# austinjeng/Shift-GCN

Hardware: AMD Instinct MI355X
Metric: skeleton clips/sec fwd+bwd, NTU (3,300,25,2) bs=64; 1/2/4/8 MI355X (higher is better)
Workload: dtype fp32; 1 GPU; NTU Shift-GCN training step (fwd+CE+bwd+SGD), x=(64,3,300,25,2) per GPU; global_batch=64, per_gpu_batch=64, parallelism=dp1, hipgraph=False, world_size=1, backend=none

## Files before the change

include/shiftgcn.h:

```cpp
#ifndef SHIFTGCN_H_
#define SHIFTGCN_H_

#include <stddef.h>

#ifdef __cplusplus
extern "C" {
#endif

#define SGCN_EINVAL (-22)
#define SGCN_ABI_VERSION 24
#define SGCN_ABI_DIAG_FLAG 0x10000

int sgcn_abi_version(void);


int sgcn_tshift_fwd(const float* in, float* out, const float* xpos, const float* ypos,
                    const float* in_scale, const float* in_shift, float* plane_stats,
                    int B, int C, int H, int W, int stride, int ypos_is_raw, void* stream);

int sgcn_tshift_fwd_pre(const float* z, float* out, const float* xpos, const float* ypos,
                        const float* pre_scale, const float* pre_shift, const float* r,
                        const float* r_scale, const float* r_shift, const float* in_scale,
                        const float* in_shift, int B, int C, int H, int W, int stride,
                        int ypos_is_raw, void* stream);

int sgcn_tshift_fwd_tail(const float* in, float* out, const float* xpos, const float* ypos,
                         const float* post_scale, const float* post_shift, const float* r,
                         const float* r_scale, const float* r_shift, const float* gather_m,
                         float* out_gathered, int B, int C, int H, int W, int stride,
                         int ypos_is_raw, void* stream);

int sgcn_tshift_bwd_bnin(const float* dy, const float* y, const float* s, const float* coef,
                         const float* in, const float* xpos, const float* ypos, float* gin,
                         float* gx, float* gy, void* ws, size_t ws_bytes, int B, int C, int H,
                         int W, int ypos_is_raw, int dy_plane, void* stream);
size_t sgcn_tshift_bwd_ws_bytes(int B, int C);

int sgcn_tshift_pos_finalize(const void* ws, int B, int C, float* gx, float* gy, void* stream);

int sgcn_tshift_bwd(const float* gout, const float* in, const float* xpos, const float* ypos,
                    const float* in_scale, const float* in_shift, int relu_mask,
                    const float* bn_mean, const float* bn_invstd, float* bn_part, float* gin,
                    float* gx, float* gy, void* ws, size_t ws_bytes, int B, int C, int H,
                    int W, int stride, int ypos_is_raw, void* stream);

int sgcn_tshift_fwd_f64(const double* in, double* out, const double* xpos, const double* ypos,
                        int B, int C, int H, int W, int stride, int ypos_is_raw, void* stream);
size_t sgcn_tshift_bwd_f64_ws_bytes(int B, int C);
int sgcn_tshift_bwd_f64(const double* gout, const double* in, const double* xpos,
                        const double* ypos, double* gin, double* gx, double* gy, void* ws,
                        size_t ws_bytes, int B, int C, int H, int W, int stride,
                        int ypos_is_raw, void* stream);

int sgcn_tshift_bwd_gbn(const float* gout, const float* in, const float* xpos,
                        const float* ypos, const float* in_scale, const float* in_shift,
                        const float* bn_mean, const float* bn_invstd, float* bn_part,
                        const float* z, const float* z_mean, const float* z_invstd,
                        float* z_part, const float* d, const float* d_mean,
                        const float* d_invstd, float* d_part, float* gin, float* gx, float* gy,
                        void* ws, size_t ws_bytes, int B, int C, int H, int W, void* stream);


int sgcn_pw_fwd(const float* w, int w_mcontig, const float* bias, const float* x,
                long long x_bstride, long long x_cstride, int x_tstride, int x_rsign,
                const float* mask, float* y, long long y_bstride, long long y_cstride,
                int y_tstride, int y_rsign, int relu, int accumulate, int B, int M, int K,
                int T, int V, void* stream);

size_t sgcn_pw_tshift_ws_bytes(int K);
int sgcn_pw_fwd_tshift(const float* w, const float* bias, const float* x, long long x_bstride,
                       long long x_cstride, const float* xpos, const float* ypos,
                       const float* in_scale, const float* in_shift, float* x_shifted,
                       void* ws, size_t ws_bytes, float* y, long long y_bstride,
                       long long y_cstride, int relu, int two_row, int B, int M, int K, int T,
                       int V, void* stream);

size_t sgcn_pw_dw_ws_bytes(int B, int M, int Nc, int T, int V);

int sgcn_pw_dw(const float* g, long long g_bstride, long long g_cstride, int g_tstride,
               int g_rsign, const float* x, long long x_bstride, long long x_cstride,
               int x_tstride, int x_rsign, const float* mask, float* dw, int dw_transpose,
               int dw_accumulate, float* dbias, int dbias_accumulate, void* ws,
               size_t ws_bytes, int B, int M, int Nc, int T, int V, void* stream);


size_t sgcn_moments_ws_bytes(int B, int C, int V, int per_joint);

int sgcn_moments(const float* x, float* part, int B, int C, int T, int V, int per_joint,
                 void* stream);


int sgcn_bn_finalize(const float* part, int B, int F, int n_part, int perm_V,
                     const float* gamma, const float* beta, float eps, float momentum,
                     float* running_mean, float* running_var, long long* num_batches,
                     float* mean, float* invstd, float* scale, float* shift, void* stream);

int sgcn_bn_eval_coef(int F, int perm_V, const float* gamma, const float* beta,
                      const float* running_mean, const float* running_var, float eps,
                      float* mean, float* invstd, float* scale, float* shift, void* stream);

int sgcn_bn_apply(const float* x, const float* scale, const float* shift, int per_joint,
                  const float* r, const float* rscale, const float* rshift, int relu,
                  float* y, float* y_stats, const float* gather_m, float* y_gathered, int B,
                  int C, int T, int V, void* stream);
int sgcn_bn_bwd_reduce(const float* dy, const float* y, int relu, const float* x,
                       const float* mean, const float* invstd, int per_joint, const float* r,
                       const float* rmean, const float* rinvstd, const float* dy_coef,
                       float* part, float* rpart, int B, int C, int T, int V, int dy_plane,
                       void* stream);

int sgcn_bn_bwd_finalize(const float* part, int B, int F, long long n_total, int perm_V,
                         const float* mean, const float* invstd, const float* gamma,
                         float* dgamma, float* dbeta, int accumulate, int batch_stats,
                         float* coef, void* stream);

int sgcn_bn_bwd_finalize_gbn(const float* part6, int B, int C, int V, long long n_total,
                             const float* dy_coef, const float* dy_mean, const float* mean,
                             const float* invstd, const float* gamma, float* dgamma,
                             float* dbeta, int accumulate, int batch_stats, float* coef,
                             void* stream);

int sgcn_bn_bwd_apply(const float* dy, const float* y, int relu, const float* x,
                      const float* coef, int per_joint, const float* r, const float* rcoef,
                      const float* dy_coef, float* dx, float* dr, int B, int C, int T, int V,
                      void* stream);

int sgcn_mask_prep(const float* mask, float* m, int n, void* stream);

int sgcn_gcn_gather(const float* x0, const float* m, float* xg, int B, int C, int T, int V,
                    void* stream);

#define SGCN_DXF_MASK_DX 1
#define SGCN_DXF_ADD2_PLANE 2
int sgcn_gcn_dx_finish(const float* dxt, const float* x0, const float* m, const float* add1,
                       const float* add2, const float* add2_mask, float* dx, float* dmask_part,
                       const float* prev_s, const float* prev_mean, const float* prev_invstd,
                       float* prev_part, int B, int C, int T, int V, int flags, void* stream);

int sgcn_mask_grad_finalize(const float* part, const float* mask, int B, int C, int V,
                            float* dmask, int accumulate, void* stream);

int sgcn_modalities(const float* joint, const int* parent, float* out_joint, float* out_bone,
                    float* out_joint_motion, float* out_bone_motion, const float* scale,
                    const float* shift, int planes, int N, int C, int T, int V, int M,
                    void* stream);


size_t sgcn_head_ws_bytes(int N, int C, int V, int M);

int sgcn_head_moments(const float* x, float* part, int N, int C, int T, int V, int M,
                      void* stream);

int sgcn_head_apply(const float* x, const float* scale, const float* shift, float* y, int N,
                    int C, int T, int V, int M, void* stream);

int sgcn_head_bwd_reduce(const float* g, const float* x, const float* mean, const float* invstd,
                         float* part, int N, int C, int T, int V, int M, void* stream);

int sgcn_head_bwd_apply(const float* g, const float* x, const float* coef, float* dx, int N,
                        int C, int T, int V, int M, void* stream);

int sgcn_pool(const float* x, float* out, int N, int M, int C, long long P, void* stream);

int sgcn_pool_bwd(const float* dout, float* dx, int N, int M, int C, long long P,
                  void* stream);

int sgcn_pool_bwd_planes(const float* dout, float* dplane, int N, int M, int C, long long P,
                         void* stream);


int sgcn_sgd_chunk_elems(void);

int sgcn_sgd_step(const void* table, const int* numel, const int* chunks, int n_chunks,
                  float momentum, int nesterov, void* stream);

#define SGCN_BATCH_MAX 32
int sgcn_tshift_pos_finalize_many(const void* const* partials, float* const* gx,
                                  float* const* gy, const int* B, const int* C, int n,
                                  void* stream);
int sgcn_mask_prep_many(const float* const* mask, float* const* m, const int* count, int n,
                        void* stream);
int sgcn_mask_grad_finalize_many(const float* const* part, const float* const* mask,
                                 float* const* dmask, const int* B, const int* C,
                                 const int* V, int n, void* stream);

#ifdef __cplusplus
}
#endif

#endif
```

shift-gcn_amd/csrc/bn.hip:

```cpp
#include "common.hpp"

namespace sgcn {
namespace {

constexpr int kThreads = 256;

constexpr int kU = 4;

constexpr int kUM = 8;

template <bool PER_JOINT, bool ZU = false>
__global__ __launch_bounds__(kThreads) void moments_kernel(const float* __restrict__ x,
                                                            float2* __restrict__ part, int T,
                                                            int V, int C) {
  SGCN_CRIT_PRIO();
  __shared__ float s1[kThreads], s2[kThreads], red[2 * kThreads / 64];
  const int plane = gridDim.x - 1 - blockIdx.x;
  const int P = T * V;
  const float* __restrict__ xp = x + (size_t)plane * P;
  const int i = threadIdx.x;
  if (PER_JOINT) {
    const int G = kThreads / V;
    float a = 0.f, q = 0.f;
    const int v = i % V, r = i / V;
// ... 595 lines not shown
  for (int q = 0; q < kGbnW - 1; ++q) {
#pragma unroll
    for (int j = 0; j < 6; ++j) s6[j] += red[q][j][lane];
  }
  const int c = f / V;
  const double k1 = dyc[c], k2 = dyc[C + c], c3 = (double)dyc[2 * C + c] + k2 * (double)dym[c];
  const double sg = k1 * s6[0] + k2 * s6[1] + c3 * s6[2];
  const double sgx = k1 * s6[3] + k2 * s6[4] + c3 * s6[5];
  const int rf = ref_feature(f, V, F);
  if (dgamma) dgamma[rf] = accumulate ? dgamma[rf] + (float)sgx : (float)sgx;
  if (dbeta) dbeta[rf] = accumulate ? dbeta[rf] + (float)sg : (float)sg;
  const float g = gamma ? gamma[rf] : 1.f;
  const float is = invstd[f];
  const float q1 = g * is;
  const float q2 = batch_stats ? (float)(-(double)q1 * (double)is * (sgx / n_total)) : 0.f;
  const float q3 = batch_stats ? (float)(-(double)q1 * (sg / n_total) - (double)q2 * (double)mean[f])
                               : 0.f;
  coef[f] = q1;
  coef[F + f] = q2;
  coef[2 * F + f] = q3;
}

template <int PJM, bool RELU, int RES, bool DYT>
__global__ __launch_bounds__(kThreads) void bn_bwd_apply_kernel(
    const float* __restrict__ dy, const float* __restrict__ y, const float* __restrict__ x,
    const float* __restrict__ coef, int F, const float* __restrict__ r,
    const float* __restrict__ rcoef, int RF, const float* __restrict__ dyc,
    float* __restrict__ dx, float* __restrict__ dr, int C, int T, int V) {
  SGCN_CRIT_PRIO();
  constexpr bool PER_JOINT = PJM != 0, GATH = PJM >= 2, XG = PJM == 3;
  const int plane = blockIdx.x, c = plane % C;
  const int P = T * V;
  const size_t off = (size_t)plane * P;
  const int rc = c % V;
  __shared__ float k_s[PER_JOINT ? 3 * kThreads : 1];
  if (PER_JOINT) {
    if ((int)threadIdx.x < V) {
      const int f = c * V + threadIdx.x;
      k_s[threadIdx.x] = coef[f];
      k_s[kThreads + threadIdx.x] = coef[F + f];
      k_s[2 * kThreads + threadIdx.x] = coef[2 * F + f];
    }
    __syncthreads();
  }
  float k1 = 0.f, k2 = 0.f, k3 = 0.f, q1 = 0.f, q2 = 0.f, q3 = 0.f;
  float d1 = 1.f, d2 = 0.f, d3 = 0.f;
  if (DYT) { d1 = dyc[c]; d2 = dyc[C + c]; d3 = dyc[2 * C + c]; }
  if (!PER_JOINT) { k1 = coef[c]; k2 = coef[F + c]; k3 = coef[2 * F + c]; }
  if (RES == 2) { q1 = rcoef[c]; q2 = rcoef[RF + c]; q3 = rcoef[2 * RF + c]; }
  const int dv = kThreads % V;
  int v = threadIdx.x % V;
  for (int base = 0; base < P; base += kThreads * kU) {
    float gv[kU], yv[kU], xv[kU], rv[kU];
#pragma unroll
    for (int u = 0; u < kU; ++u) {
      const int o = min(base + u * kThreads + (int)threadIdx.x, P - 1);
      gv[u] = dy[off + o];
      if (RELU) yv[u] = y[off + o];
      if (!XG) xv[u] = x[off + o];
      if (RES == 2) rv[u] = r[off + o];
    }
    if (XG) {
      int vq = v;
#pragma unroll
      for (int u = 0; u < kU; ++u) {
        const int o = min(base + u * kThreads + (int)threadIdx.x, P - 1);
        const int w = vq - rc;
        xv[u] = x[off + min(max(o - vq + (w < 0 ? w + V : w), 0), P - 1)];
        vq += dv;
        if (vq >= V) vq -= V;
      }
    }
#pragma unroll
    for (int u = 0; u < kU; ++u) {
      const int o = base + u * kThreads + threadIdx.x;
      float g = gv[u];
      if (DYT) g = d1 * g + d2 * yv[u] + d3;
      if (RELU) g = yv[u] > 0.f ? g : 0.f;
      if (PER_JOINT) { k1 = k_s[v]; k2 = k_s[kThreads + v]; k3 = k_s[2 * kThreads + v]; }
      if (o < P) {
        int od = o;
        if (GATH) {
          const int w = v - rc;
          od = o - v + (w < 0 ? w + V : w);
        }
        dx[off + od] = k1 * g + k2 * xv[u] + k3;
        if (RES == 1) dr[off + o] = g;
        if (RES == 2) dr[off + o] = q1 * g + q2 * rv[u] + q3;
      }
      v += dv;
      if (v >= V) v -= V;
    }
  }
}

template <int NT, int LPT, int PJM, bool RELU, int RES, bool DYT>
__global__ __launch_bounds__(NT) void bn_bwd_apply_ja_kernel(
    const float* __restrict__ dy, const float* __restrict__ y, const float* __restrict__ x,
    const float* __restrict__ coef, int F, const float* __restrict__ r,
    const float* __restrict__ rcoef, int RF, const float* __restrict__ dyc,
    float* __restrict__ dx, float* __restrict__ dr, int C, int T, int V) {
  SGCN_CRIT_PRIO();
  static_assert(PJM == 0 || PJM == 3, "per-channel, or per-joint gathered (ZU)");
  constexpr bool PER_JOINT = PJM == 3;
  const int plane = blockIdx.x, c = plane % C, rc = c % V;
  const int GR = NT / V, NTJ = GR * V, tid = threadIdx.x;
  const bool own = tid < NTJ;
  const int w = tid % V;
  const int P = T * V;
  const size_t off = (size_t)plane * P;
  const unsigned vo = own ? (unsigned)tid * 4u : 0x80000000u, vstep = (unsigned)NTJ * 4u;
  const unsigned pb = (unsigned)P * 4u;
  int wz = w - rc;
  wz = wz < 0 ? wz + V : wz;
  const unsigned go = vo + (unsigned)((PER_JOINT ? wz - w : 0) * 4);
  float gv[LPT], yv[RELU ? LPT : 1], xv[LPT], rv[RES == 2 ? LPT : 1];
  {
    const auto dyr = make_rsrc(dy + off, pb);
    const auto xr = make_rsrc(x + off, pb);
#pragma unroll
    for (int e = 0; e < LPT; ++e) {
      gv[e] = bload(dyr, vo + e * vstep, 0);
      xv[e] = bload(xr, go + e * vstep, 0);
    }
    if (RELU) {
      const auto yr = make_rsrc(y + off, pb);
#pragma unroll
      for (int e = 0; e < LPT; ++e) yv[e] = bload(yr, vo + e * vstep, 0);
    }
    if (RES == 2) {
      const auto rr = make_rsrc(r + off, pb);
#pragma unroll
      for (int e = 0; e < LPT; ++e) rv[e] = bload(rr, vo + e * vstep, 0);
    }
  }
  const int f = PER_JOINT ? c * V + w : c;
  const float k1 = coef[f], k2 = coef[F + f], k3 = coef[2 * F + f];
  float d1 = 1.f, d2 = 0.f, d3 = 0.f, q1 = 0.f, q2 = 0.f, q3 = 0.f;
  if (DYT) { d1 = dyc[c]; d2 = dyc[C + c]; d3 = dyc[2 * C + c]; }
  if (RES == 2) { q1 = rcoef[c]; q2 = rcoef[RF + c]; q3 = rcoef[2 * RF + c]; }
  const auto dxr = make_rsrc(dx + off, pb);
  const auto drr = make_rsrc(RES ? dr + off : dx + off, RES ? pb : 0u);
#pragma unroll
  for (int e = 0; e < LPT; ++e) {
    float g = gv[e];
    if (DYT) g = d1 * g + d2 * yv[e] + d3;
    if (RELU) g = yv[e] > 0.f ? g : 0.f;
    bstore(dxr, k1 * g + k2 * xv[e] + k3, go + e * vstep, 0);
    if (RES == 1) bstore(drr, g, vo + e * vstep, 0);
    if (RES == 2) bstore(drr, q1 * g + q2 * rv[e] + q3, vo + e * vstep, 0);
  }
}

template <int NT, int LPT, bool ADD1, bool ADD2, bool PART, int A2M>
__global__ __launch_bounds__(NT) void gcn_dx_finish_ja_kernel(
    const float* __restrict__ dxt, const float* __restrict__ x0, const float* __restrict__ m,
    const float* __restrict__ add1, const float* __restrict__ add2, float* __restrict__ dx,
    float* __restrict__ dmask_part, const float* __restrict__ ps,
    const float* __restrict__ pmean, const float* __restrict__ pinvstd,
    float2* __restrict__ bn_part, int C, int T, int V, const float* __restrict__ add2m,
    int flags) {
  SGCN_CRIT_PRIO();
#ifdef SGCN_DIAG_F1B_REAL
  return;
#endif
  __shared__ float s0[NT];
  __shared__ float red[2 * NT / 64];
  const int plane = blockIdx.x, c = plane % C, rc = c % V;
  const int GR = NT / V, NTJ = GR * V, tid = threadIdx.x;
  const bool own = tid < NTJ;
  const int vd = tid % V;
  int us = vd - rc;
  us = us < 0 ? us + V : us;
  const int P = T * V;
  const size_t off = (size_t)plane * P;
  const unsigned vo = own ? (unsigned)tid * 4u : 0x80000000u, vstep = (unsigned)NTJ * 4u;
  const unsigned pb = (unsigned)P * 4u;
  const unsigned uo = vo + (unsigned)((us - vd) * 4);
  const bool mdx = flags & SGCN_DXF_MASK_DX;
  constexpr bool A2P = A2M == 2;
  float gv[LPT], xq[LPT], a1[ADD1 ? LPT : 1], a2[ADD2 && !A2P ? LPT : 1], a2q[A2M ? LPT : 1];
  float sv[PART ? LPT : 1];
  {
#ifdef SGCN_DIAG_F1B_BOUND
    const auto gr = make_rsrc(dxt + off, 0u), xr = make_rsrc(x0 + off, pb);
#else
    const auto gr = make_rsrc(dxt + off, pb), xr = make_rsrc(x0 + off, pb);
#endif
#pragma unroll
    for (int e = 0; e < LPT; ++e) {
      gv[e] = bload(gr, uo + e * vstep, 0);
      xq[e] = bload(xr, vo + e * vstep, 0);
    }
    if (ADD1) {
      const auto ar = make_rsrc(add1 + off, pb);
#pragma unroll
      for (int e = 0; e < LPT; ++e) a1[e] = bload(ar, vo + e * vstep, 0);
    }
    if (ADD2 && !A2P) {
      const auto ar = make_rsrc(add2 + off, pb);
#pragma unroll
      for (int e = 0; e < LPT; ++e) a2[e] = bload(ar, vo + e * vstep, 0);
    }
    if (A2M) {
      const auto ar = make_rsrc(add2m + off, pb);
#pragma unroll
      for (int e = 0; e < LPT; ++e) a2q[e] = bload(ar, vo + e * vstep, 0);
    }
    if (PART) {
      const auto ar = make_rsrc(ps + off, pb);
#pragma unroll
      for (int e = 0; e < LPT; ++e) sv[e] = bload(ar, vo + e * vstep, 0);
    }
  }
  const float mu = m[us * C + c];
  float pm = 0.f, pi = 0.f, a2v = 0.f;
  if (PART) { pm = pmean[c]; pi = pinvstd[c]; }
  if (A2P) a2v = add2[plane];
  const auto dxr = make_rsrc(dx + off, pb);
  float acc = 0.f, b0 = 0.f, b1 = 0.f;
#pragma unroll
  for (int e = 0; e < LPT; ++e) {
    float val = gv[e] * mu;
    if (ADD1) val += a1[e];
    if (ADD2) val += A2M ? (a2q[e] > 0.f ? (A2P ? a2v : a2[e]) : 0.f) : a2[e];
    bstore(dxr, (xq[e] > 0.f || !mdx) ? val : 0.f, vo + e * vstep, 0);
    acc = fmaf(gv[e], xq[e], acc);
    if (PART) {
      const float g = xq[e] > 0.f ? val : 0.f;
      b0 += g;
      b1 = fmaf(g, (sv[e] - pm) * pi, b1);
    }
  }
  if (PART) {
    block_sum2(b0, b1, red);
    if (tid == 0) bn_part[plane] = make_float2(b0, b1);
  }
  s0[tid] = acc;
  __syncthreads();
  if (tid < V) {
    int vq = tid + rc;
    vq = vq >= V ? vq - V : vq;
    float sum = 0.f;
    for (int g = 0; g < GR; ++g) sum += s0[g * V + vq];
    dmask_part[(size_t)plane * V + tid] = sum;
  }
}

__global__ __launch_bounds__(kThreads) void gcn_gather_kernel(const float* __restrict__ x0,
                                                              const float* __restrict__ m,
                                                              float* __restrict__ xg, int C,
                                                              int T, int V) {
  SGCN_CRIT_PRIO();
  __shared__ float m_s[kThreads];
  const int plane = blockIdx.x, c = plane % C;
  const int P = T * V;
  const size_t off = (size_t)plane * P;
  const int rc = c % V;
  if ((int)threadIdx.x < V) m_s[threadIdx.x] = m[threadIdx.x * C + c];
  __syncthreads();
  const int dv = kThreads % V;
  int w = threadIdx.x % V;
  for (int base = 0; base < P; base += kThreads * kU) {
    float xv[kU], mv[kU];
    int ww = w;
#pragma unroll
    for (int u = 0; u < kU; ++u) {
      const int oraw = base + u * kThreads + (int)threadIdx.x;
      int src = ww + rc;
      src = src >= V ? src - V : src;
      xv[u] = x0[off + min(oraw - ww + src, P - 1)];
      mv[u] = m_s[ww];
      ww += dv;
      if (ww >= V) ww -= V;
    }
#pragma unroll
    for (int u = 0; u < kU; ++u) {
      const int o = base + u * kThreads + (int)threadIdx.x;
      if (o < P) xg[off + o] = xv[u] * mv[u];
    }
    w = ww;
  }
}

template <bool ADD1, bool ADD2, bool PART, bool A2M = false>
__global__ __launch_bounds__(kThreads) void gcn_dx_finish_kernel(
    const float* __restrict__ dxt, const float* __restrict__ x0, const float* __restrict__ m,
    const float* __restrict__ add1, const float* __restrict__ add2, float* __restrict__ dx,
    float* __restrict__ dmask_part, const float* __restrict__ ps,
    const float* __restrict__ pmean, const float* __restrict__ pinvstd,
    float2* __restrict__ bn_part, int C, int T, int V, const float* __restrict__ add2m,
    int flags) {
  SGCN_CRIT_PRIO();
  const bool mdx = flags & SGCN_DXF_MASK_DX, a2p = flags & SGCN_DXF_ADD2_PLANE;
  __shared__ float s0[kThreads];
  const int plane = blockIdx.x, c = plane % C;
  const size_t off = (size_t)plane * T * V;
  const int rc = c % V;
  const int i = threadIdx.x;
  const int G = kThreads / V;
  const int vd = i % V, rr = i / V;
  int us = vd - rc;
  us = us < 0 ? us + V : us;
  const float mu = m[us * C + c];
  float pm = 0.f, pi = 0.f;
  if (PART) { pm = pmean[c]; pi = pinvstd[c]; }
  float acc = 0.f, b0 = 0.f, b1 = 0.f;
  if (i < G * V) {
    for (int t0 = rr; t0 < T; t0 += G * kU) {
      float gv[kU], xq[kU], a1[kU], a2[kU], sv[kU], a2q[kU];
#pragma unroll
      for (int k = 0; k < kU; ++k) {
        const int row = min(t0 + k * G, T - 1) * V;
        gv[k] = dxt[off + row + us];
        xq[k] = x0[off + row + vd];
        if (ADD1) a1[k] = add1[off + row + vd];
        if (ADD2) a2[k] = a2p ? add2[plane] : add2[off + row + vd];
        if (A2M) a2q[k] = add2m[off + row + vd];
        if (PART) sv[k] = ps[off + row + vd];
      }
#pragma unroll
      for (int k = 0; k < kU; ++k) {
        const int t = t0 + k * G;
        float val = gv[k] * mu;
        if (ADD1) val += a1[k];
        if (ADD2) val += A2M ? (a2q[k] > 0.f ? a2[k] : 0.f) : a2[k];
        if (t < T) dx[off + t * V + vd] = (xq[k] > 0.f || !mdx) ? val : 0.f;
        acc += (t < T) ? gv[k] * xq[k] : 0.f;
        if (PART) {
          const float g = (t < T && xq[k] > 0.f) ? val : 0.f;
          b0 += g;
          b1 += g * ((sv[k] - pm) * pi);
        }
      }
    }
  }
  if (PART) {
    __shared__ float red[2 * kThreads / 64];
    block_sum2(b0, b1, red);
    if (i == 0) bn_part[plane] = make_float2(b0, b1);
  }
  s0[i] = acc;
  __syncthreads();
  if (i < V) {
    int vq = i + rc;
    vq = vq >= V ? vq - V : vq;
    float sum = 0.f;
    for (int g = 0; g < G; ++g) sum += s0[g * V + vq];
    dmask_part[(size_t)plane * V + i] = sum;
  }
}

__global__ void mask_prep_kernel(const float* __restrict__ mask, float* __restrict__ m, int n) {
  const int i = blockIdx.x * blockDim.x + threadIdx.x;
  if (i < n) m[i] = tanhf(mask[i]) + 1.f;
}

struct MaskPrepBatch {
  const float* mask[SGCN_BATCH_MAX];
  float* m[SGCN_BATCH_MAX];
  int n[SGCN_BATCH_MAX];
};
__global__ void mask_prep_many_kernel(const MaskPrepBatch t) {
  const int e = blockIdx.y;
  const int i = blockIdx.x * blockDim.x + threadIdx.x;
  if (i < t.n[e]) t.m[e][i] = tanhf(t.mask[e][i]) + 1.f;
}

__device__ __forceinline__ void mask_grad_body(const float* __restrict__ part,
                                               const float* __restrict__ mask, int B, int C,
                                               int V, float* __restrict__ dmask,
                                               int accumulate);
__global__ __launch_bounds__(64 * kFW) void mask_grad_finalize_kernel(
    const float* __restrict__ part, const float* __restrict__ mask, int B, int C, int V,
    float* __restrict__ dmask, int accumulate) {
  mask_grad_body(part, mask, B, C, V, dmask, accumulate);
}
struct MaskGradBatch {
  const float* part[SGCN_BATCH_MAX];
  const float* mask[SGCN_BATCH_MAX];
  float* dmask[SGCN_BATCH_MAX];
  int B[SGCN_BATCH_MAX];
  int C[SGCN_BATCH_MAX];
  int V[SGCN_BATCH_MAX];
};
__global__ __launch_bounds__(64 * kFW) void mask_grad_finalize_many_kernel(const MaskGradBatch t) {
  const int i = blockIdx.y;
  if ((int)blockIdx.x * kFW >= t.C[i] * t.V[i]) return;
  mask_grad_body(t.part[i], t.mask[i], t.B[i], t.C[i], t.V[i], t.dmask[i], 0);
}
__device__ __forceinline__ void mask_grad_body(const float* __restrict__ part,
                                               const float* __restrict__ mask, int B, int C,
                                               int V, float* __restrict__ dmask,
                                               int accumulate) {
  const int F = C * V;
  const int lane = threadIdx.x & 63;
  const int f = blockIdx.x * kFW + (int)(threadIdx.x >> 6);
  const int fc = min(f, F - 1);
  double a = 0.0;
  for (int b0 = lane; b0 < B; b0 += 64 * 4) {
    float pv[4];
#pragma unroll
    for (int u = 0; u < 4; ++u) {
      const int b = b0 + u * 64;
      pv[u] = b < B ? part[(size_t)b * F + fc] : 0.f;
    }
#pragma unroll
    for (int u = 0; u < 4; ++u) a += pv[u];
  }
  const double s = wave_dsum(a);
  if (f >= F || lane != 0) return;
  const int c = f / V, u = f - c * V;
  const int i = u * C + c;
  const float t = tanhf(mask[i]);
  const float g = (float)s * (1.f - t * t);
  dmask[i] = accumulate ? dmask[i] + g : g;
}

}
}

using namespace sgcn;

constexpr int kJaSplit = 8192;

int ja_lpt(int T, int V, int nt) {
  if (V > 64) return 0;
  const int ntj = (nt / V) * V, per = (T * V + ntj - 1) / ntj;
  return per <= 8 ? 8 : (per <= 16 ? 16 : (per <= 24 ? 24 : (per <= 32 ? 32 : 0)));
}

#define SGCN_PLANE_CHECK() \
  SGCN_REQUIRE(B >= 0 && C > 0 && T >= 0 && V > 0 && V <= kThreads)

extern "C" {

size_t sgcn_moments_ws_bytes(int B, int C, int V, int per_joint) {
  return (size_t)B * C * (per_joint ? V : 1) * sizeof(float2);
}

int sgcn_moments(const float* x, float* part, int B, int C, int T, int V, int per_joint,
                 void* stream) {
  SGCN_PLANE_CHECK();
  if (B == 0) return 0;
  SGCN_REQUIRE(x && part && T > 0);
  hipStream_t st = (hipStream_t)stream;
  SGCN_REQUIRE(per_joint == 0 || per_joint == 3);
  {
    const int nt = T * V <= kJaSplit ? kThreads : 512;
    const int lpt = ja_lpt(T, V, nt);
    if (lpt) {
#define SGCN_MJ(NT, L, PJ)                                                                     \
  moments_ja_kernel<NT, L, PJ, PJ><<<B * C, NT, 0, st>>>(x, (float2*)part, T, V, C)
#define SGCN_MJ_L(NT, PJ)                                                                      \
  do {                                                                                         \
    if (lpt == 8) SGCN_MJ(NT, 8, PJ); else if (lpt == 16) SGCN_MJ(NT, 16, PJ);                 \
    else if (lpt == 24) SGCN_MJ(NT, 24, PJ);                                                   \
    else SGCN_MJ(NT, 32, PJ);                                                                  \
  } while (0)
      if (nt == kThreads) { if (per_joint) SGCN_MJ_L(kThreads, true); else SGCN_MJ_L(kThreads, false); }
      else { if (per_joint) SGCN_MJ_L(512, true); else SGCN_MJ_L(512, false); }
#undef SGCN_MJ_L
#undef SGCN_MJ
      SGCN_LAUNCH_CHECK();
      return 0;
    }
  }
  if (per_joint == 3)
    moments_kernel<true, true><<<B * C, kThreads, 0, st>>>(x, (float2*)part, T, V, C);
  else moments_kernel<false><<<B * C, kThreads, 0, st>>>(x, (float2*)part, T, V, C);
  SGCN_LAUNCH_CHECK();
  return 0;
}

int sgcn_bn_finalize(const float* part, int B, int F, int n_part, int perm_V,
                     const float* gamma, const float* beta, float eps, float momentum,
                     float* running_mean, float* running_var, long long* num_batches,
                     float* mean, float* invstd, float* scale, float* shift, void* stream) {
  SGCN_REQUIRE(part && B > 0 && F > 0 && n_part > 0 && mean && invstd && scale && shift);
// ... 181 lines not shown
  SGCN_REQUIRE(part && B > 0 && F > 0 && n_total > 0 && mean && invstd && coef);
  SGCN_REQUIRE(perm_V <= 0 || F % perm_V == 0);
  bn_bwd_finalize_kernel<<<(F + 63) / 64, 64 * kFSW, 0, (hipStream_t)stream>>>(
      (const float2*)part, B, F, (double)n_total, perm_V, mean, invstd, gamma, dgamma, dbeta,
      accumulate, batch_stats, coef);
  SGCN_LAUNCH_CHECK();
  return 0;
}

int sgcn_bn_bwd_finalize_gbn(const float* part6, int B, int C, int V, long long n_total,
                             const float* dy_coef, const float* dy_mean, const float* mean,
                             const float* invstd, const float* gamma, float* dgamma,
                             float* dbeta, int accumulate, int batch_stats, float* coef,
                             void* stream) {
  SGCN_REQUIRE(part6 && B > 0 && C > 0 && V > 0 && n_total > 0 && dy_coef && dy_mean && mean &&
               invstd && coef);
  const int F = C * V;
  bn_bwd_finalize_gbn_kernel<<<(F + 63) / 64, 64 * kGbnW, 0, (hipStream_t)stream>>>(
      part6, B, F, V, (double)n_total, dy_coef, dy_mean, C, mean, invstd, gamma, dgamma, dbeta,
      accumulate, batch_stats, coef);
  SGCN_LAUNCH_CHECK();
  return 0;
}

int sgcn_bn_bwd_apply(const float* dy, const float* y, int relu, const float* x,
                      const float* coef, int per_joint, const float* r, const float* rcoef,
                      const float* dy_coef, float* dx, float* dr, int B, int C, int T, int V,
                      void* stream) {
  SGCN_PLANE_CHECK();
  if (B == 0 || T == 0) return 0;
  SGCN_REQUIRE(dy && x && coef && dx && (y || !relu));
  SGCN_REQUIRE(!dy_coef || (y && relu));
  SGCN_REQUIRE(!rcoef || (r && dr));
  SGCN_REQUIRE(per_joint == 0 || per_joint == 3);
  hipStream_t st = (hipStream_t)stream;
  const int res = dr == nullptr ? 0 : (rcoef ? 2 : 1);
  const int F = per_joint ? C * V : C;
  dim3 g(B * C);
  if (per_joint == 3) SGCN_REQUIRE(relu);
  {
    const int nt = T * V <= kJaSplit ? kThreads : 512;
    const int lpt = ja_lpt(T, V, nt);
    if (lpt) {
#define SGCN_BJ(NT, L, PJ, RL, RS)                                                             \
  (dy_coef ? bn_bwd_apply_ja_kernel<NT, L, PJ, RL, RS, true><<<g, NT, 0, st>>>(                 \
                 dy, y, x, coef, F, r, rcoef, C, dy_coef, dx, dr, C, T, V)             \
           : bn_bwd_apply_ja_kernel<NT, L, PJ, RL, RS, false><<<g, NT, 0, st>>>(                \
                 dy, y, x, coef, F, r, rcoef, C, dy_coef, dx, dr, C, T, V))
#define SGCN_BJ_L(NT, PJ, RL, RS)                                                              \
  do {                                                                                         \
    if (lpt == 8) SGCN_BJ(NT, 8, PJ, RL, RS);                                                  \
    else if (lpt == 16) SGCN_BJ(NT, 16, PJ, RL, RS);                                           \
    else if (lpt == 24) SGCN_BJ(NT, 24, PJ, RL, RS);                                           \
    else SGCN_BJ(NT, 32, PJ, RL, RS);                                                          \
  } while (0)
#define SGCN_BJ_T(PJ, RL, RS)                                                                  \
  do { if (nt == kThreads) SGCN_BJ_L(kThreads, PJ, RL, RS); else SGCN_BJ_L(512, PJ, RL, RS); } while (0)
#define SGCN_BJ_R(PJ, RL)                                                                      \
  do {                                                                                         \
    if (res == 0) SGCN_BJ_T(PJ, RL, 0);                                                        \
    else if (res == 1) SGCN_BJ_T(PJ, RL, 1);                                                   \
    else SGCN_BJ_T(PJ, RL, 2);                                                                 \
  } while (0)
      if (per_joint == 3) SGCN_BJ_R(3, true);
      else if (relu) SGCN_BJ_R(0, true);
      else SGCN_BJ_R(0, false);
#undef SGCN_BJ_R
#undef SGCN_BJ_T
#undef SGCN_BJ_L
#undef SGCN_BJ
      SGCN_LAUNCH_CHECK();
      return 0;
    }
  }
#define SGCN_BA(PJ, RL, RS)                                                                   \
  (dy_coef ? bn_bwd_apply_kernel<PJ, RL, RS, true><<<g, kThreads, 0, st>>>(                      \
                 dy, y, x, coef, F, r, rcoef, C, dy_coef, dx, dr, C, T, V)                      \
           : bn_bwd_apply_kernel<PJ, RL, RS, false><<<g, kThreads, 0, st>>>(                     \
                 dy, y, x, coef, F, r, rcoef, C, dy_coef, dx, dr, C, T, V))
#define SGCN_BA_R(PJ, RL) \
  if (res == 0) SGCN_BA(PJ, RL, 0); else if (res == 1) SGCN_BA(PJ, RL, 1); else SGCN_BA(PJ, RL, 2)
  if (per_joint == 3) { SGCN_BA_R(3, true); }
  else if (relu) { SGCN_BA_R(0, true); } else { SGCN_BA_R(0, false); }
#undef SGCN_BA_R
#undef SGCN_BA
  SGCN_LAUNCH_CHECK();
  return 0;
}

int sgcn_mask_prep(const float* mask, float* m, int n, void* stream) {
  SGCN_REQUIRE(mask && m && n > 0);
  mask_prep_kernel<<<(n + 255) / 256, 256, 0, (hipStream_t)stream>>>(mask, m, n);
  SGCN_LAUNCH_CHECK();
  return 0;
}

int sgcn_mask_prep_many(const float* const* mask, float* const* m, const int* count, int n,
                        void* stream) {
  SGCN_REQUIRE(n >= 0 && n <= SGCN_BATCH_MAX);
  if (n == 0) return 0;
  SGCN_REQUIRE(mask && m && count);
  MaskPrepBatch t{};
  int mx = 0;
  for (int i = 0; i < n; ++i) {
    SGCN_REQUIRE(mask[i] && m[i] && count[i] > 0);
    t.mask[i] = mask[i];
    t.m[i] = m[i];
    t.n[i] = count[i];
    mx = max(mx, count[i]);
  }
  mask_prep_many_kernel<<<dim3((mx + 255) / 256, n), 256, 0, (hipStream_t)stream>>>(t);
  SGCN_LAUNCH_CHECK();
  return 0;
}

int sgcn_mask_grad_finalize_many(const float* const* part, const float* const* mask,
                                 float* const* dmask, const int* B, const int* C,
                                 const int* V, int n, void* stream) {
  SGCN_REQUIRE(n >= 0 && n <= SGCN_BATCH_MAX);
  if (n == 0) return 0;
  SGCN_REQUIRE(part && mask && dmask && B && C && V);
  MaskGradBatch t{};
  int mf = 0;
  for (int i = 0; i < n; ++i) {
    SGCN_REQUIRE(part[i] && mask[i] && dmask[i] && B[i] > 0 && C[i] > 0 && V[i] > 0);
    t.part[i] = part[i];
    t.mask[i] = mask[i];
    t.dmask[i] = dmask[i];
    t.B[i] = B[i];
    t.C[i] = C[i];
    t.V[i] = V[i];
    mf = max(mf, C[i] * V[i]);
  }
  mask_grad_finalize_many_kernel<<<dim3((mf + kFW - 1) / kFW, n), 64 * kFW, 0,
                                   (hipStream_t)stream>>>(t);
  SGCN_LAUNCH_CHECK();
  return 0;
}

int sgcn_gcn_gather(const float* x0, const float* m, float* xg, int B, int C, int T, int V,
                    void* stream) {
  SGCN_PLANE_CHECK();
  if (B == 0 || T == 0) return 0;
  SGCN_REQUIRE(x0 && m && xg && x0 != xg);
  gcn_gather_kernel<<<B * C, kThreads, 0, (hipStream_t)stream>>>(x0, m, xg, C, T, V);
  SGCN_LAUNCH_CHECK();
  return 0;
}

int sgcn_gcn_dx_finish(const float* dxt, const float* x0, const float* m, const float* add1,
                       const float* add2, const float* add2_mask, float* dx, float* dmask_part,
                       const float* prev_s, const float* prev_mean, const float* prev_invstd,
                       float* prev_part, int B,
                       int C, int T, int V, int flags, void* stream) {
  SGCN_PLANE_CHECK();
  if (B == 0 || T == 0) return 0;
  SGCN_REQUIRE(dxt && x0 && m && dx && dmask_part);
  SGCN_REQUIRE((flags & ~(SGCN_DXF_MASK_DX | SGCN_DXF_ADD2_PLANE)) == 0);
  SGCN_REQUIRE(!(flags & SGCN_DXF_ADD2_PLANE) || add2_mask);
  SGCN_REQUIRE(!prev_part || (prev_s && prev_mean && prev_invstd));
  SGCN_REQUIRE(!add2_mask || add2);
  hipStream_t st = (hipStream_t)stream;
  float2* pp = (float2*)prev_part;
  if (add2_mask) SGCN_REQUIRE(add1);
  {
    const int nt = T * V <= kJaSplit ? kThreads : 512;
    const int lpt = ja_lpt(T, V, nt);
    if (lpt) {
#define SGCN_FJ(NT, L, A1, A2, PT, AM)                                                         \
  gcn_dx_finish_ja_kernel<NT, L, A1, A2, PT, AM><<<B * C, NT, 0, st>>>(                        \
      dxt, x0, m, add1, add2, dx, dmask_part, prev_s, prev_mean, prev_invstd, pp, C, T, V,     \
      add2_mask, flags)
#define SGCN_FJ_L(NT, A1, A2, PT, AM)                                                          \
  do {                                                                                         \
    if (lpt == 8) SGCN_FJ(NT, 8, A1, A2, PT, AM);                                              \
    else if (lpt == 16) SGCN_FJ(NT, 16, A1, A2, PT, AM);                                       \
    else if (lpt == 24) SGCN_FJ(NT, 24, A1, A2, PT, AM);                                       \
    else SGCN_FJ(NT, 32, A1, A2, PT, AM);                                                      \
  } while (0)
#define SGCN_FJ_T(A1, A2, PT, AM)                                                              \
  do { if (nt == kThreads) SGCN_FJ_L(kThreads, A1, A2, PT, AM); else SGCN_FJ_L(512, A1, A2, PT, AM); } while (0)
#define SGCN_FJ_P(A1, A2, AM)                                                                  \
  do { if (pp) SGCN_FJ_T(A1, A2, true, AM); else SGCN_FJ_T(A1, A2, false, AM); } while (0)
      if (add2_mask) { if (flags & SGCN_DXF_ADD2_PLANE) SGCN_FJ_P(true, true, 2); else SGCN_FJ_P(true, true, 1); }
      else if (add1) { if (add2) SGCN_FJ_P(true, true, 0); else SGCN_FJ_P(true, false, 0); }
      else { if (add2) SGCN_FJ_P(false, true, 0); else SGCN_FJ_P(false, false, 0); }
#undef SGCN_FJ_P
#undef SGCN_FJ_T
#undef SGCN_FJ_L
#undef SGCN_FJ
      SGCN_LAUNCH_CHECK();
      return 0;
    }
  }
  if (add2_mask) {
    if (pp)
      gcn_dx_finish_kernel<true, true, true, true><<<B * C, kThreads, 0, st>>>(
          dxt, x0, m, add1, add2, dx, dmask_part, prev_s, prev_mean, prev_invstd, pp, C, T, V,
          add2_mask, flags);
    else
      gcn_dx_finish_kernel<true, true, false, true><<<B * C, kThreads, 0, st>>>(
          dxt, x0, m, add1, add2, dx, dmask_part, prev_s, prev_mean, prev_invstd, pp, C, T, V,
          add2_mask, flags);
    SGCN_LAUNCH_CHECK();
    return 0;
  }
#define SGCN_FIN(A1, A2, PT)                                                                \
  gcn_dx_finish_kernel<A1, A2, PT><<<B * C, kThreads, 0, st>>>(                           \
      dxt, x0, m, add1, add2, dx, dmask_part, prev_s, prev_mean, prev_invstd, pp, C, T, V,  \
      nullptr, flags)
#define SGCN_FIN_P(A1, A2)                                                                  \
  do {                                                                                      \
    if (pp) SGCN_FIN(A1, A2, true);                                                         \
    else SGCN_FIN(A1, A2, false);                                                           \
  } while (0)
  if (add1) { if (add2) SGCN_FIN_P(true, true); else SGCN_FIN_P(true, false); }
  else { if (add2) SGCN_FIN_P(false, true); else SGCN_FIN_P(false, false); }
#undef SGCN_FIN_P
#undef SGCN_FIN
  SGCN_LAUNCH_CHECK();
  return 0;
}

int sgcn_mask_grad_finalize(const float* part, const float* mask, int B, int C, int V,
                            float* dmask, int accumulate, void* stream) {
  SGCN_REQUIRE(part && mask && dmask && B > 0 && C > 0 && V > 0);
  mask_grad_finalize_kernel<<<(C * V + kFW - 1) / kFW, 64 * kFW, 0,
                              (hipStream_t)stream>>>(part, mask, B, C, V, dmask, accumulate);
  SGCN_LAUNCH_CHECK();
  return 0;
}

}
```

shift-gcn_amd/csrc/tshift.hip:

```cpp
#include "common.hpp"

#pragma clang fp contract(off)

namespace sgcn {
namespace {

constexpr int kThreads = 256;


struct Geom {
  int x1, y1;
  float dx, dy;
};

__device__ __forceinline__ Geom make_geom(float x, float y) {
  Geom g;
  g.x1 = (int)floorf(x);
  g.y1 = (int)floorf(y);
  g.dx = x - (float)g.x1;
  g.dy = y - (float)g.y1;
  return g;
}

__device__ __forceinline__ float blend(float q11, float q21, float q12, float q22, float dx,
// ... 429 lines not shown
    const int lstep = GR * stride * WP;
#pragma unroll
    for (int e = 0; e < LPT; ++e) {
      const int la = min(la0 + e * lstep, lmax);
      emit(e, blend(pl[la], pl[la + 1], pl[la + WP], pl[la + WP + 1], g.dx, g.dy));
    }
  } else {
    const bool c0 = (unsigned)(w + g.x1) < (unsigned)W, c1 = (unsigned)(w + g.x1 + 1) < (unsigned)W;
    const int cc0 = min(max(w + g.x1, 0), W - 1) + 1, cc1 = min(max(w + g.x1 + 1, 0), W - 1) + 1;
#pragma unroll
    for (int e = 0; e < LPT; ++e) {
      const int rr = (h0 + e * GR) * stride + g.y1;
      const bool r0 = (unsigned)rr < (unsigned)Hb, r1 = (unsigned)(rr + 1) < (unsigned)Hb;
      const int p0 = (min(max(rr, 0), Hb - 1) + kPadRows) * WP;
      const int p1 = (min(max(rr + 1, 0), Hb - 1) + kPadRows) * WP;
      const float q11 = (r0 && c0) ? pl[p0 + cc0] : 0.f, q21 = (r0 && c1) ? pl[p0 + cc1] : 0.f;
      const float q12 = (r1 && c0) ? pl[p1 + cc0] : 0.f, q22 = (r1 && c1) ? pl[p1 + cc1] : 0.f;
      emit(e, blend(q11, q21, q12, q22, g.dx, g.dy));
    }
  }
  if (STATS) {
    float s1 = 0.f;
#pragma unroll
    for (int e = 0; e < LPT; ++e) s1 += v[e];
    s1 = block_sum(s1, red);
    const float mean = s1 / (float)n;
    float m2 = 0.f;
#pragma unroll
    for (int e = 0; e < LPT; ++e) {
      const float d = v[e] - mean;
      m2 += e < nval ? d * d : 0.f;
    }
    m2 = block_sum(m2, red);
    if (tid == 0) pstats[plane] = make_float2(mean, m2);
  }
}

template <int NT, int LPT, int RES>
__global__ __launch_bounds__(NT) void tshift_fwd_pre_kernel(
    const float* __restrict__ z, float* __restrict__ out, const float* __restrict__ xpos,
    const float* __restrict__ ypos, const float* __restrict__ zs, const float* __restrict__ zt,
    const float* __restrict__ r, const float* __restrict__ rs, const float* __restrict__ rt,
    const float* __restrict__ scale, const float* __restrict__ shift, int C, int Hb, int W,
    int Ho, int stride, int add_half) {
  SGCN_CRIT_PRIO();
  extern __shared__ float pl[];
  __shared__ float zs_s[1024], zt_s[1024];
  const int plane = gridDim.x - 1 - blockIdx.x;
  const int c = plane % C;
  const int nb = Hb * W;
  const size_t ioff = (size_t)plane * nb;
  float* __restrict__ dst = out + (size_t)plane * Ho * W;
  const float y = add_half ? ypos[c] + 0.5f : ypos[c];
  const Geom g = make_geom(xpos[c], y);
  const float a = scale[c], b = shift[c];
  float q1 = 1.f, q2 = 0.f;
  if (RES == 2) { q1 = rs[c]; q2 = rt[c]; }
  for (int i = threadIdx.x; i < W; i += NT) {
    zs_s[i] = zs[c * W + i];
    zt_s[i] = zt[c * W + i];
  }
  __syncthreads();
  {
    float t[LPT], u[LPT];
#pragma unroll
    for (int e = 0; e < LPT; ++e) {
      const int i = min(e * NT + (int)threadIdx.x, nb - 1);
      t[e] = z[ioff + i];
      u[e] = r[ioff + i];
    }
    Walker pos(threadIdx.x, NT, W);
#pragma unroll
    for (int e = 0; e < LPT; ++e) {
      const int i = e * NT + threadIdx.x;
      float h = t[e] * zs_s[pos.w] + zt_s[pos.w];
      h += RES == 2 ? u[e] * q1 + q2 : u[e];
      h = fmaxf(h, 0.f);
      if (i < nb) pl[i] = h * a + b;
      pos.next();
    }
  }
  __syncthreads();
  const int n = Ho * W;
  for (int base = 0; base < n; base += LPT * NT) {
    Walker pos(base + threadIdx.x, NT, W);
#pragma unroll
    for (int e = 0; e < LPT; ++e) {
      TapIdx ti;
      tap_idx(pos.h * stride + g.y1, pos.w + g.x1, Hb, W, ti);
      const float q11 = sel(pl[ti.o00], ti.m00), q21 = sel(pl[ti.o01], ti.m01);
      const float q12 = sel(pl[ti.o10], ti.m10), q22 = sel(pl[ti.o11], ti.m11);
      const int o = base + e * NT + threadIdx.x;
      if (o < n) dst[o] = blend(q11, q21, q12, q22, g.dx, g.dy);
      pos.next();
    }
  }
}

template <int NT, int LPT, int RES, bool GOUT>
__global__ __launch_bounds__(NT) void tshift_fwd_tail_kernel(
    const float* __restrict__ in, float* __restrict__ out, const float* __restrict__ xpos,
    const float* __restrict__ ypos, const float* __restrict__ ps, const float* __restrict__ pt,
    const float* __restrict__ r, const float* __restrict__ rs, const float* __restrict__ rt,
    const float* __restrict__ gm, float* __restrict__ og, int C, int Hb, int W, int Ho,
    int stride, int add_half) {
  SGCN_CRIT_PRIO();
  extern __shared__ float pl[];
  __shared__ float gm_s[GOUT ? 1024 : 1];
  const int plane = gridDim.x - 1 - blockIdx.x;
  const int c = plane % C;
  const size_t ooff = (size_t)plane * Ho * W;
  const float y = add_half ? ypos[c] + 0.5f : ypos[c];
  const Geom g = make_geom(xpos[c], y);
  const float sc = ps[c], sh = pt[c];
  float q1 = 1.f, q2 = 0.f;
  if (RES == 2) { q1 = rs[c]; q2 = rt[c]; }
  const int rc = c % W;
  if (GOUT)
    for (int i = threadIdx.x; i < W; i += NT) gm_s[i] = gm[i * C + c];
  stage_plane<NT, LPT, false>(in + (size_t)plane * Hb * W, pl, Hb * W, 1.f, 0.f);
  __syncthreads();
  const int n = Ho * W;
  for (int base = 0; base < n; base += LPT * NT) {
    Walker pos(base + threadIdx.x, NT, W);
    float rv[LPT];
    if (RES) {
#pragma unroll
      for (int e = 0; e < LPT; ++e) rv[e] = r[ooff + min(base + e * NT + (int)threadIdx.x, n - 1)];
    }
#pragma unroll
    for (int e = 0; e < LPT; ++e) {
      TapIdx ti;
      tap_idx(pos.h * stride + g.y1, pos.w + g.x1, Hb, W, ti);
      const float q11 = sel(pl[ti.o00], ti.m00), q21 = sel(pl[ti.o01], ti.m01);
      const float q12 = sel(pl[ti.o10], ti.m10), q22 = sel(pl[ti.o11], ti.m11);
      const int o = base + e * NT + threadIdx.x;
      float a = blend(q11, q21, q12, q22, g.dx, g.dy) * sc + sh;
      if (RES == 1) a += rv[e];
      if (RES == 2) a += rv[e] * q1 + q2;
      a = fmaxf(a, 0.f);
      if (o < n) {
        out[ooff + o] = a;
        if (GOUT) {
          int u = pos.w - rc;
          u = u < 0 ? u + W : u;
          og[ooff + o - pos.w + u] = a * gm_s[u];
        }
      }
      pos.next();
    }
  }
}

template <int NT, int LPT, bool AFFINE, bool RELU_MASK, bool BNP, bool JA>
__global__ __launch_bounds__(NT) void tshift_bwd_s2_kernel(
    const float* __restrict__ gout, const float* __restrict__ in,
    const float* __restrict__ xpos, const float* __restrict__ ypos,
    const float* __restrict__ scale, const float* __restrict__ shift,
    const float* __restrict__ bn_mean, const float* __restrict__ bn_invstd,
    float* __restrict__ gin, float2* __restrict__ pgrad, float2* __restrict__ bn_part, int C,
    int Hb, int W, int Ho, int add_half) {
  SGCN_CRIT_PRIO();
  constexpr int STRIDE = 2;
  extern __shared__ float lds[];
  __shared__ float red[4 * NT / 64];
  const int plane = gridDim.x - 1 - blockIdx.x;
  const int c = plane % C;
  const int nb = Hb * W, nt = Ho * W;
  float* gs = lds;
  float* xs = lds + nt;
  float bmu = 0.f, bis = 0.f;
  if (BNP) { bmu = bn_mean[c]; bis = bn_invstd[c]; }
  const float x = xpos[c];
  const float y = add_half ? ypos[c] + 0.5f : ypos[c];
  float a = 1.f, b = 0.f;
  if (AFFINE) { a = scale[c]; b = shift[c]; }
  {
    const float* __restrict__ go = gout + (size_t)plane * nt;
    const float* __restrict__ src = in + (size_t)plane * nb;
    const int ntot = nt + nb;
    float t[LPT];
#pragma unroll
    for (int e = 0; e < LPT; ++e) {
      const int i = min(e * NT + (int)threadIdx.x, ntot - 1);
      t[e] = i < nt ? go[i] : src[i - nt];
    }
#pragma unroll
    for (int e = 0; e < LPT; ++e) {
      const int i = e * NT + threadIdx.x;
      if (i < ntot) lds[i] = t[e];
    }
  }
  __syncthreads();
  float* __restrict__ gi = gin + (size_t)plane * nb;

  float bs0 = 0.f, bs1 = 0.f;
  float ax = 0.f, ay = 0.f;
  if (JA) {
    const Geom r = make_geom(-x, -y);
    const int NTJ = (NT / W) * W, GR = NT / W;
    if ((int)threadIdx.x < NTJ && nt > 0) {
      const int w = (int)threadIdx.x % W, w1 = w + r.x1;
      const bool c0 = (unsigned)w1 < (unsigned)W, c1 = (unsigned)(w1 + 1) < (unsigned)W;
      const int cc0 = min(max(w1, 0), W - 1), cc1 = min(max(w1 + 1, 0), W - 1);
      int h = (int)threadIdx.x / W;
      for (int o = threadIdx.x; o < nb; o += NTJ, h += GR) {
        const int h1 = h + r.y1, hq = (h1 + 1) >> 1;
        const bool ev = (h1 & 1) == 0, rok = (unsigned)hq < (unsigned)Ho;
        const int ro = min(max(hq, 0), Ho - 1) * W;
        const float t0 = (rok && c0) ? gs[ro + cc0] : 0.f;
        const float t1 = (rok && c1) ? gs[ro + cc1] : 0.f;
        float val = blend(ev ? t0 : 0.f, ev ? t1 : 0.f, ev ? 0.f : t0, ev ? 0.f : t1, r.dx, r.dy);
        const float rin = xs[o];
        if (RELU_MASK) val = rin > 0.f ? val : 0.f;
        gi[o] = val;
        if (BNP) {
          bs0 += val;
          bs1 += val * ((rin - bmu) * bis);
        }
      }
    } else if ((int)threadIdx.x < NTJ) {
      for (int o = threadIdx.x; o < nb; o += NTJ) gi[o] = 0.f;
    }
  } else {
    const Geom r = make_geom(-x, -y);
    Walker pos(threadIdx.x, NT, W);
    for (int o = threadIdx.x; o < nb; o += NT) {
      const int h1 = pos.h + r.y1;
      const int w1 = pos.w + r.x1;
      TapIdx ti;
      {
        const int h2 = h1 + 1;
        const int hq1 = (h1 % 2 == 0) ? h1 / 2 : -1;
        const int hq2 = (h2 % 2 == 0) ? h2 / 2 : -1;
        TapIdx t1, t2;
        tap_idx(hq1, w1, Ho, W, t1);
        tap_idx(hq2, w1, Ho, W, t2);
        ti.o00 = t1.o00; ti.o01 = t1.o01; ti.m00 = t1.m00; ti.m01 = t1.m01;
        ti.o10 = t2.o00; ti.o11 = t2.o01; ti.m10 = t2.m00; ti.m11 = t2.m01;
      }
      float val = 0.f;
      if (nt > 0) {
        const float q11 = sel(gs[ti.o00], ti.m00), q21 = sel(gs[ti.o01], ti.m01);
        const float q12 = sel(gs[ti.o10], ti.m10), q22 = sel(gs[ti.o11], ti.m11);
        val = blend(q11, q21, q12, q22, r.dx, r.dy);
      }
      const float rin = xs[o];
      if (RELU_MASK) val = rin > 0.f ? val : 0.f;
      gi[o] = val;
      if (BNP) {
        bs0 += val;
        bs1 += val * ((rin - bmu) * bis);
      }
      pos.next();
    }
  }

  if (JA) {
    const Geom g = make_geom(x, y);
    const int NTJ = (NT / W) * W, GR = NT / W;
    if ((int)threadIdx.x < NTJ) {
      const int w = (int)threadIdx.x % W, wc = w + g.x1;
      const bool c0 = (unsigned)wc < (unsigned)W, c1 = (unsigned)(wc + 1) < (unsigned)W;
      const int cc0 = min(max(wc, 0), W - 1), cc1 = min(max(wc + 1, 0), W - 1);
      int h = (int)threadIdx.x / W;
      for (int o = threadIdx.x; o < nt; o += NTJ, h += GR) {
        const int rr = h * STRIDE + g.y1;
        const bool r0 = (unsigned)rr < (unsigned)Hb, r1 = (unsigned)(rr + 1) < (unsigned)Hb;
        const int p0 = min(max(rr, 0), Hb - 1) * W, p1 = min(max(rr + 1, 0), Hb - 1) * W;
        float q11 = xs[p0 + cc0], q21 = xs[p0 + cc1], q12 = xs[p1 + cc0], q22 = xs[p1 + cc1];
        if (AFFINE) { q11 = q11 * a + b; q21 = q21 * a + b; q12 = q12 * a + b; q22 = q22 * a + b; }
        q11 = (r0 && c0) ? q11 : 0.f;
        q21 = (r0 && c1) ? q21 : 0.f;
        q12 = (r1 && c0) ? q12 : 0.f;
        q22 = (r1 && c1) ? q22 : 0.f;
        const float vx = (1.f - g.dy) * (q21 - q11) + g.dy * (q22 - q12);
        const float vy = (1.f - g.dx) * (q12 - q11) + g.dx * (q22 - q21);
        const float gg = gs[o];
        ax += vx * gg;
        ay += vy * gg;
      }
    }
  } else {
    const Geom g = make_geom(x, y);
    Walker pos(threadIdx.x, NT, W);
    for (int o = threadIdx.x; o < nt; o += NT) {
      TapIdx ti;
      tap_idx(pos.h * STRIDE + g.y1, pos.w + g.x1, Hb, W, ti);
      float q11 = xs[ti.o00], q21 = xs[ti.o01], q12 = xs[ti.o10], q22 = xs[ti.o11];
      if (AFFINE) { q11 = q11 * a + b; q21 = q21 * a + b; q12 = q12 * a + b; q22 = q22 * a + b; }
      q11 = sel(q11, ti.m00);
      q21 = sel(q21, ti.m01);
      q12 = sel(q12, ti.m10);
      q22 = sel(q22, ti.m11);
      const float vx = (1.f - g.dy) * (q21 - q11) + g.dy * (q22 - q12);
      const float vy = (1.f - g.dx) * (q12 - q11) + g.dx * (q22 - q21);
      const float gg = gs[o];
      ax += vx * gg;
      ay += vy * gg;
      pos.next();
    }
  }
  if (BNP) {
    block_sum4(ax, ay, bs0, bs1, red);
    if (threadIdx.x == 0) {
      pgrad[plane] = make_float2(ax, ay);
      bn_part[plane] = make_float2(bs0, bs1);
    }
  } else {
    block_sum2(ax, ay, red);
    if (threadIdx.x == 0) pgrad[plane] = make_float2(ax, ay);
  }
}

template <int NT, int LPT, bool AFFINE, bool RELU_MASK, bool BNP, int GP, bool GBN,
          bool GBD = false>
__global__ __launch_bounds__(NT) void tshift_bwd_ra_kernel(
    const float* __restrict__ gout, const float* __restrict__ in,
    const float* __restrict__ xpos, const float* __restrict__ ypos,
    const float* __restrict__ scale, const float* __restrict__ shift,
    const float* __restrict__ bn_mean, const float* __restrict__ bn_invstd,
    float* __restrict__ gin, float2* __restrict__ pgrad, float2* __restrict__ bn_part, int C,
    int H, int W, const float* __restrict__ gdy, const float* __restrict__ gy,
    const float* __restrict__ gx, const float* __restrict__ gcoef,
    const float* __restrict__ gz, const float* __restrict__ gzm,
    const float* __restrict__ gzi, float* __restrict__ gzpart, const float* __restrict__ gd = nullptr,
    const float* __restrict__ gdm = nullptr, const float* __restrict__ gdi = nullptr,
    float* __restrict__ gdpart = nullptr, int gdyp = 0) {
  SGCN_CRIT_PRIO();
  static_assert(!GBN || (AFFINE && BNP && !GP), "GBN: shift_in with BNP");
// ... 274 lines not shown
      const int b = b0 + u * 64;
      pv[u] = b < B ? pgrad[(size_t)b * C + cc] : make_float2(0.f, 0.f);
    }
#pragma unroll
    for (int u = 0; u < 4; ++u) {
      ax += (double)pv[u].x;
      ay += (double)pv[u].y;
    }
  }
#pragma unroll
  for (int o = 32; o > 0; o >>= 1) {
    ax += __shfl_xor(ax, o, 64);
    ay += __shfl_xor(ay, o, 64);
  }
  if (c >= C || lane != 0) return;
  const double sx = ax, sy = ay;
  const float Gx = (float)(sx / (double)B);
  const float Gy = (float)(sy / (double)B);
  const float gy2 = Gy * Gy;
  const float dr = (float)sqrt((double)gy2);
  if (dr != 0.f) {
    const float qx = (float)((double)Gx / (double)dr);
    const float qy = (float)((double)Gy / (double)dr);
    gx[c] = (float)((double)qx * 0.0);
    gy[c] = (float)((double)qy * 0.01);
  } else {
    gx[c] = 0.0f;
    gy[c] = (float)0.0001;
  }
}

template <int EPT>
void launch_fwd(bool affine, bool stats, const float* in, float* out, const float* xpos,
                const float* ypos, const float* scale, const float* shift, float2* ps, int B,
                int C, int H, int W, int Ho, int stride, int add_half, hipStream_t st) {
  dim3 grid(B * C), block(kThreads);
#define SGCN_FWD(A, S)                                                                     \
  tshift_fwd_kernel<EPT, A, S><<<grid, block, 0, st>>>(in, out, xpos, ypos, scale, shift, \
                                                      ps, C, H, W, Ho, stride, add_half)
  if (affine) {
    if (stats) SGCN_FWD(true, true); else SGCN_FWD(true, false);
  } else {
    if (stats) SGCN_FWD(false, true); else SGCN_FWD(false, false);
  }
#undef SGCN_FWD
}

template <int LPT, int NT = kThreads>
void launch_fwd_lds(bool affine, bool stats, const float* in, float* out, const float* xpos,
                    const float* ypos, const float* scale, const float* shift, float2* ps,
                    int B, int C, int H, int W, int Ho, int stride, int add_half,
                    hipStream_t st) {
  dim3 grid(B * C), block(NT);
  const size_t lds = (size_t)H * W * sizeof(float);
#define SGCN_FWDL(A, S)                                                                  \
  tshift_fwd_lds_kernel<NT, LPT, LPT, A, S><<<grid, block, lds, st>>>(                    \
      in, out, xpos, ypos, scale, shift, ps, C, H, W, Ho, stride, add_half)
  if (affine) {
    if (stats) SGCN_FWDL(true, true); else SGCN_FWDL(true, false);
  } else {
    if (stats) SGCN_FWDL(false, true); else SGCN_FWDL(false, false);
  }
#undef SGCN_FWDL
}

int pad_fwd_lpt(int H, int W, int nt) {
  if (W > 64) return 0;
  const int ntj = (nt / W) * W, per = (H * W + ntj - 1) / ntj;
  int lpt = per <= 8 ? 8 : (per <= 16 ? 16 : (per <= 24 ? 24 : (per <= 32 ? 32 : 0)));
  if (nt == 512 && per > 8 && per <= 12) lpt = 12;
  if (nt == 512 && per > 16 && per <= 20) lpt = 20;
  return (size_t)(ra_pad_floats(H, W) + 1) * sizeof(float) > 65536 ? 0 : lpt;
}

template <int NT>
bool launch_fwd_pad(bool affine, bool stats, const float* in, float* out, const float* xpos,
                    const float* ypos, const float* scale, const float* shift, float2* ps,
                    int B, int C, int H, int W, int Ho, int stride, int add_half,
                    hipStream_t st) {
  const int lpt = pad_fwd_lpt(H, W, NT);
  const size_t lds = (size_t)(ra_pad_floats(H, W) + 1) * sizeof(float);
  if (lpt == 0) return false;
#define SGCN_FWDP(L, A, S)                                                                   \
  tshift_fwd_pad_kernel<NT, L, 0, A, S><<<B * C, NT, lds, st>>>(                             \
      in, out, xpos, ypos, scale, shift, ps, C, H, W, Ho, stride, add_half, nullptr, nullptr, \
      nullptr, nullptr, nullptr, nullptr, nullptr)
#define SGCN_FWDP_AS(L)                                                                      \
  do {                                                                                       \
    if (affine) { if (stats) SGCN_FWDP(L, true, true); else SGCN_FWDP(L, true, false); }     \
    else { if (stats) SGCN_FWDP(L, false, true); else SGCN_FWDP(L, false, false); }          \
  } while (0)
  if (lpt == 8) SGCN_FWDP_AS(8); else if (lpt == 12) SGCN_FWDP_AS(12); else if (lpt == 16) SGCN_FWDP_AS(16);
  else if (lpt == 20) SGCN_FWDP_AS(20); else if (lpt == 24) SGCN_FWDP_AS(24); else SGCN_FWDP_AS(32);
#undef SGCN_FWDP_AS
#undef SGCN_FWDP
  return true;
}

template <int EPT, int STRIDE>
void launch_bwd(bool affine, bool relu, const float* gout, const float* in, const float* xpos,
                const float* ypos, const float* scale, const float* shift, const float* bmu,
                const float* bis, float* gin, float2* pg, float2* bp, int B, int C, int H,
                int W, int Ho, int add_half, hipStream_t st) {
  dim3 grid(B * C), block(kThreads);
#define SGCN_BWD(A, R, P)                                                                    \
  tshift_bwd_kernel<EPT, A, R, STRIDE, P><<<grid, block, 0, st>>>(                            \
      gout, in, xpos, ypos, scale, shift, bmu, bis, gin, pg, bp, C, H, W, Ho, add_half)
  if (bp) {
    if (affine) {
      if (relu) SGCN_BWD(true, true, true); else SGCN_BWD(true, false, true);
    } else {
      if (relu) SGCN_BWD(false, true, true); else SGCN_BWD(false, false, true);
    }
  } else {
    if (affine) {
      if (relu) SGCN_BWD(true, true, false); else SGCN_BWD(true, false, false);
    } else {
      if (relu) SGCN_BWD(false, true, false); else SGCN_BWD(false, false, false);
    }
  }
#undef SGCN_BWD
}

constexpr int kBwdThreads = 512;

template <int LPT, bool JA>
void launch_bwd_s2(bool affine, bool relu, const float* gout, const float* in,
                   const float* xpos, const float* ypos, const float* scale,
                   const float* shift, const float* bmu, const float* bis, float* gin,
                   float2* pg, float2* bp, int B, int C, int H, int W, int Ho, int add_half,
                   hipStream_t st) {
  constexpr int NT = kBwdThreads;
  dim3 grid(B * C), block(NT);
  const size_t lds = (size_t)(H + Ho) * W * sizeof(float);
#define SGCN_BWDL(A, R, P)                                                                  \
  tshift_bwd_s2_kernel<NT, LPT, A, R, P, JA><<<grid, block, lds, st>>>(                      \
      gout, in, xpos, ypos, scale, shift, bmu, bis, gin, pg, bp, C, H, W, Ho, add_half)
  if (bp) {
    if (affine) {
      if (relu) SGCN_BWDL(true, true, true); else SGCN_BWDL(true, false, true);
    } else {
      if (relu) SGCN_BWDL(false, true, true); else SGCN_BWDL(false, false, true);
    }
  } else {
    if (affine) {
      if (relu) SGCN_BWDL(true, true, false); else SGCN_BWDL(true, false, false);
    } else {
      if (relu) SGCN_BWDL(false, true, false); else SGCN_BWDL(false, false, false);
    }
  }
#undef SGCN_BWDL
}

int pick_lpt(int n, int nt) {
  const int per = (n + nt - 1) / nt;
  return per <= 8 ? 8 : (per <= 16 ? 16 : 32);
}

int ra_lpt(int n, int nt, int W) {
  const int nte = (nt / W) * W;
  if (nte <= 0 || W > 64) return 0;
  const int per = (n + nte - 1) / nte;
  if (nt == 512 && per > 8 && per <= 12) return 12;
  if (nt == 512 && per > 16 && per <= 20) return 20;
  return per <= 8 ? 8 : (per <= 16 ? 16 : (per <= 24 ? 24 : (per <= 32 ? 32 : 0)));
}

constexpr int kRaSplit256 = 8192;
#ifndef SGCN_GBD_SPLIT
#define SGCN_GBD_SPLIT 1
#endif

size_t ra_lds_bytes(int H, int W, int nt, bool gbn) {
  const int f = ra_pad_floats(H, W);
  return (size_t)(gbn ? max(f + 1, 6 * nt) : f + 1) * sizeof(float);
}
constexpr size_t kRaLdsMax = 65536;

template <bool AFFINE, bool RELU, bool BNP, int GP, bool GBN, bool GBD = false>
bool launch_ra(int nt, const float* gout, const float* in, const float* xpos,
               const float* ypos, const float* scale, const float* shift, const float* bmu,
               const float* bis, float* gin, float2* pg, float2* bp, int B, int C, int H,
               int W, const float* gdy, const float* gy, const float* gx, const float* gcoef,
               const float* gz, const float* gzm, const float* gzi, float* gzpart,
               hipStream_t st, const float* gd = nullptr, const float* gdm = nullptr,
               const float* gdi = nullptr, float* gdpart = nullptr, int gdyp = 0) {
  const int lpt = ra_lpt(H * W, nt, W);
  const size_t lds = ra_lds_bytes(H, W, nt, GBN);
  if (lpt == 0 || lds > kRaLdsMax) return false;
#define SGCN_RA(NT, L)                                                                         \
  tshift_bwd_ra_kernel<NT, L, AFFINE, RELU, BNP, GP, GBN, GBD><<<B * C, NT, lds, st>>>(        \
      gout, in, xpos, ypos, scale, shift, bmu, bis, gin, pg, bp, C, H, W, gdy, gy, gx, gcoef,  \
      gz, gzm, gzi, gzpart, gd, gdm, gdi, gdpart, gdyp)
  if (nt == 256) {
    if (lpt == 8) SGCN_RA(256, 8); else if (lpt == 16) SGCN_RA(256, 16); else if (lpt == 24) SGCN_RA(256, 24); else SGCN_RA(256, 32);
  } else {
    if (lpt == 8) SGCN_RA(512, 8); else if (lpt == 12) SGCN_RA(512, 12); else if (lpt == 16) SGCN_RA(512, 16);
    else if (lpt == 20) SGCN_RA(512, 20); else if (lpt == 24) SGCN_RA(512, 24); else SGCN_RA(512, 32);
  }
#undef SGCN_RA
  return true;
}

int pick_ept(int n) {
  const int per = (n + kThreads - 1) / kThreads;
  return per <= 8 ? 8 : (per <= 16 ? 16 : 32);
}

}
}

using namespace sgcn;

extern "C" {

int sgcn_tshift_fwd(const float* in, float* out, const float* xpos, const float* ypos,
                    const float* in_scale, const float* in_shift, float* plane_stats, int B,
                    int C, int H, int W, int stride, int ypos_is_raw, void* stream) {
  SGCN_REQUIRE(B >= 0 && C > 0 && H >= 0 && W > 0 && stride >= 1);
  SGCN_REQUIRE((in_scale == nullptr) == (in_shift == nullptr));
  const int Ho = H / stride;
  if (B == 0 || Ho == 0) return 0;
  SGCN_REQUIRE(in && out && xpos && ypos);
  SGCN_REQUIRE((long long)H * W < (1LL << 30) && (long long)B * C < (1LL << 31));
  hipStream_t st = (hipStream_t)stream;
  const bool aff = in_scale != nullptr, stats = plane_stats != nullptr;
  float2* ps = (float2*)plane_stats;
  const int ah = (ypos_is_raw && stride != 1) ? 1 : 0;
  if (H * W <= kFwdLdsMax2 &&
      (H * W <= kFwdLdsMax
           ? launch_fwd_pad<kThreads>(aff, stats, in, out, xpos, ypos, in_scale, in_shift, ps, B, C, H, W, Ho, stride, ah, st)
           : launch_fwd_pad<512>(aff, stats, in, out, xpos, ypos, in_scale, in_shift, ps, B, C, H, W, Ho, stride, ah, st))) {
    SGCN_LAUNCH_CHECK();
    return 0;
  }
  if (H * W <= kFwdLdsMax) {
    switch (pick_lpt(H * W, kThreads)) {
      case 8: launch_fwd_lds<8>(aff, stats, in, out, xpos, ypos, in_scale, in_shift, ps, B, C, H, W, Ho, stride, ah, st); break;
      case 16: launch_fwd_lds<16>(aff, stats, in, out, xpos, ypos, in_scale, in_shift, ps, B, C, H, W, Ho, stride, ah, st); break;
      default: launch_fwd_lds<32>(aff, stats, in, out, xpos, ypos, in_scale, in_shift, ps, B, C, H, W, Ho, stride, ah, st); break;
    }
    SGCN_LAUNCH_CHECK();
    return 0;
  }
  if (H * W <= kFwdLdsMax2) {
    launch_fwd_lds<32, 512>(aff, stats, in, out, xpos, ypos, in_scale, in_shift, ps, B, C, H, W, Ho, stride, ah, st);
    SGCN_LAUNCH_CHECK();
    return 0;
  }
  switch (pick_ept(Ho * W)) {
    case 8: launch_fwd<8>(aff, stats, in, out, xpos, ypos, in_scale, in_shift, ps, B, C, H, W, Ho, stride, ah, st); break;
    case 16: launch_fwd<16>(aff, stats, in, out, xpos, ypos, in_scale, in_shift, ps, B, C, H, W, Ho, stride, ah, st); break;
    default: launch_fwd<32>(aff, stats, in, out, xpos, ypos, in_scale, in_shift, ps, B, C, H, W, Ho, stride, ah, st); break;
  }
  SGCN_LAUNCH_CHECK();
  return 0;
}

int sgcn_tshift_fwd_pre(const float* z, float* out, const float* xpos, const float* ypos,
                        const float* pre_scale, const float* pre_shift, const float* r,
                        const float* r_scale, const float* r_shift, const float* in_scale,
                        const float* in_shift, int B, int C, int H, int W, int stride,
                        int ypos_is_raw, void* stream) {
  SGCN_REQUIRE(B >= 0 && C > 0 && H >= 0 && W > 0 && W <= 1024 && stride >= 1);
  SGCN_REQUIRE((r_scale == nullptr) == (r_shift == nullptr));
  SGCN_REQUIRE(H * W <= kFwdLdsMax2);
  const int Ho = H / stride;
  if (B == 0 || Ho == 0) return 0;
  SGCN_REQUIRE(z && out && xpos && ypos && pre_scale && pre_shift && r && in_scale &&
               in_shift && out != z);
  SGCN_REQUIRE((long long)B * C < (1LL << 31));
  hipStream_t st = (hipStream_t)stream;
  const int ah = (ypos_is_raw && stride != 1) ? 1 : 0;
  {
    const int nt = H * W <= kFwdLdsMax ? kThreads : 512;
    const int lpt = pad_fwd_lpt(H, W, nt);
    if (lpt) {
      const size_t plds = (size_t)(ra_pad_floats(H, W) + 1) * sizeof(float);
#define SGCN_PREP(NT, L, R)                                                                    \
  tshift_fwd_pad_kernel<NT, L, 1, true, false, R><<<B * C, NT, plds, st>>>(                    \
      z, out, xpos, ypos, in_scale, in_shift, nullptr, C, H, W, Ho, stride, ah, pre_scale,      \
      pre_shift, r, r_scale, r_shift)
#define SGCN_PREP_R(NT, L) \
  do { if (r_scale) SGCN_PREP(NT, L, 2); else SGCN_PREP(NT, L, 1); } while (0)
      if (nt == kThreads) {
        if (lpt == 8) SGCN_PREP_R(kThreads, 8); else if (lpt == 16) SGCN_PREP_R(kThreads, 16); else if (lpt == 24) SGCN_PREP_R(kThreads, 24); else SGCN_PREP_R(kThreads, 32);
      } else {
        if (lpt == 8) SGCN_PREP_R(512, 8); else if (lpt == 12) SGCN_PREP_R(512, 12); else if (lpt == 16) SGCN_PREP_R(512, 16);
        else if (lpt == 20) SGCN_PREP_R(512, 20); else if (lpt == 24) SGCN_PREP_R(512, 24); else SGCN_PREP_R(512, 32);
      }
#undef SGCN_PREP_R
#undef SGCN_PREP
      SGCN_LAUNCH_CHECK();
      return 0;
    }
  }
  const size_t lds = (size_t)H * W * sizeof(float);
#define SGCN_PRE(NT, L, R)                                                                     \
  tshift_fwd_pre_kernel<NT, L, R><<<B * C, NT, lds, st>>>(z, out, xpos, ypos, pre_scale,       \
                                                           pre_shift, r, r_scale, r_shift,     \
                                                           in_scale, in_shift, C, H, W, Ho,    \
                                                           stride, ah)
#define SGCN_PRE_R(NT, L) \
  do { if (r_scale) SGCN_PRE(NT, L, 2); else SGCN_PRE(NT, L, 1); } while (0)
  if (H * W <= kFwdLdsMax) {
    switch (pick_lpt(H * W, kThreads)) {
      case 8: SGCN_PRE_R(kThreads, 8); break;
      case 16: SGCN_PRE_R(kThreads, 16); break;
      default: SGCN_PRE_R(kThreads, 32); break;
    }
  } else {
    SGCN_PRE_R(512, 32);
  }
#undef SGCN_PRE_R
#undef SGCN_PRE
  SGCN_LAUNCH_CHECK();
  return 0;
}

int sgcn_tshift_fwd_tail(const float* in, float* out, const float* xpos, const float* ypos,
                         const float* post_scale, const float* post_shift, const float* r,
                         const float* r_scale, const float* r_shift, const float* gather_m,
                         float* out_gathered, int B, int C, int H, int W, int stride,
                         int ypos_is_raw, void* stream) {
  SGCN_REQUIRE(B >= 0 && C > 0 && H >= 0 && W > 0 && W <= 1024 && stride >= 1);
  SGCN_REQUIRE((r_scale == nullptr) == (r_shift == nullptr) && (r || !r_scale));
  SGCN_REQUIRE((gather_m == nullptr) == (out_gathered == nullptr));
  SGCN_REQUIRE(H * W <= kFwdLdsMax2);
  const int Ho = H / stride;
  if (B == 0 || Ho == 0) return 0;
  SGCN_REQUIRE(in && out && xpos && ypos && post_scale && post_shift && out != in);
  SGCN_REQUIRE((long long)B * C < (1LL << 31));
  hipStream_t st = (hipStream_t)stream;
  const int ah = (ypos_is_raw && stride != 1) ? 1 : 0;
  const int res = r == nullptr ? 0 : (r_scale ? 2 : 1);
  const bool go = out_gathered != nullptr;
  {
    const int nt = H * W <= kFwdLdsMax ? kThreads : 512;
    const int lpt = pad_fwd_lpt(H, W, nt);
    if (lpt) {
      const size_t plds = (size_t)(ra_pad_floats(H, W) + 1) * sizeof(float);
#define SGCN_TAILP(NT, L, R, G)                                                                \
  tshift_fwd_pad_kernel<NT, L, 2, false, false, R, G><<<B * C, NT, plds, st>>>(                \
      in, out, xpos, ypos, post_scale, post_shift, nullptr, C, H, W, Ho, stride, ah, nullptr,  \
      nullptr, r, r_scale, r_shift, gather_m, out_gathered)
#define SGCN_TAILP_RG(NT, L)                                                                   \
  do {                                                                                         \
    if (res == 0) { if (go) SGCN_TAILP(NT, L, 0, true); else SGCN_TAILP(NT, L, 0, false); }    \
    else if (res == 1) { if (go) SGCN_TAILP(NT, L, 1, true); else SGCN_TAILP(NT, L, 1, false); } \
    else { if (go) SGCN_TAILP(NT, L, 2, true); else SGCN_TAILP(NT, L, 2, false); }             \
  } while (0)
      if (nt == kThreads) {
        if (lpt == 8) SGCN_TAILP_RG(kThreads, 8); else if (lpt == 16) SGCN_TAILP_RG(kThreads, 16); else if (lpt == 24) SGCN_TAILP_RG(kThreads, 24); else SGCN_TAILP_RG(kThreads, 32);
      } else {
        if (lpt == 8) SGCN_TAILP_RG(512, 8); else if (lpt == 12) SGCN_TAILP_RG(512, 12); else if (lpt == 16) SGCN_TAILP_RG(512, 16);
        else if (lpt == 20) SGCN_TAILP_RG(512, 20); else if (lpt == 24) SGCN_TAILP_RG(512, 24); else SGCN_TAILP_RG(512, 32);
      }
#undef SGCN_TAILP_RG
#undef SGCN_TAILP
      SGCN_LAUNCH_CHECK();
      return 0;
    }
  }
  const size_t lds = (size_t)H * W * sizeof(float);
#define SGCN_TAIL(NT, L, R, G)                                                                \
  tshift_fwd_tail_kernel<NT, L, R, G><<<B * C, NT, lds, st>>>(                                \
      in, out, xpos, ypos, post_scale, post_shift, r, r_scale, r_shift, gather_m,            \
      out_gathered, C, H, W, Ho, stride, ah)
#define SGCN_TAIL_RG(NT, L)                                                                   \
  do {                                                                                        \
    if (res == 0) { if (go) SGCN_TAIL(NT, L, 0, true); else SGCN_TAIL(NT, L, 0, false); }     \
    else if (res == 1) { if (go) SGCN_TAIL(NT, L, 1, true); else SGCN_TAIL(NT, L, 1, false); } \
    else { if (go) SGCN_TAIL(NT, L, 2, true); else SGCN_TAIL(NT, L, 2, false); }              \
  } while (0)
  if (H * W <= kFwdLdsMax) {
    switch (pick_lpt(H * W, kThreads)) {
      case 8: SGCN_TAIL_RG(kThreads, 8); break;
      case 16: SGCN_TAIL_RG(kThreads, 16); break;
      default: SGCN_TAIL_RG(kThreads, 32); break;
    }
  } else {
    SGCN_TAIL_RG(512, 32);
  }
#undef SGCN_TAIL_RG
#undef SGCN_TAIL
  SGCN_LAUNCH_CHECK();
  return 0;
}

int sgcn_tshift_bwd_bnin(const float* dy, const float* y, const float* s, const float* coef,
                         const float* in, const float* xpos, const float* ypos, float* gin,
                         float* gx, float* gy, void* ws, size_t ws_bytes, int B, int C, int H,
                         int W, int ypos_is_raw, int dy_plane, void* stream) {
  SGCN_REQUIRE(B > 0 && C > 0 && H > 0 && W > 0);
  SGCN_REQUIRE(H * W <= kBwdLdsMax);
  SGCN_REQUIRE(dy && s && coef && in && xpos && ypos && gin && ws);
  SGCN_REQUIRE((gx == nullptr) == (gy == nullptr));
  SGCN_REQUIRE(ws_bytes >= sgcn_tshift_bwd_ws_bytes(B, C));
  SGCN_REQUIRE((long long)B * C < (1LL << 31));
  (void)ypos_is_raw;
  hipStream_t st = (hipStream_t)stream;
  float2* pg = (float2*)ws;
  const int ntb = H * W <= 4096 ? 256 : 512;
  const int dyp = dy_plane != 0;
  const bool ok =
      y ? launch_ra<false, true, false, 1, false>(
              ntb, nullptr, in, xpos, ypos, nullptr, nullptr, nullptr, nullptr, gin, pg, nullptr,
              B, C, H, W, dy, y, s, coef, nullptr, nullptr, nullptr, nullptr, st, nullptr,
              nullptr, nullptr, nullptr, dyp)
        : launch_ra<false, true, false, 2, false>(
              ntb, nullptr, in, xpos, ypos, nullptr, nullptr, nullptr, nullptr, gin, pg, nullptr,
              B, C, H, W, dy, nullptr, s, coef, nullptr, nullptr, nullptr, nullptr, st, nullptr,
              nullptr, nullptr, nullptr, dyp);
  SGCN_REQUIRE(ok);
  SGCN_LAUNCH_CHECK();
  if (gx) tshift_pos_finalize_kernel<<<(C + 3) / 4, 256, 0, st>>>(pg, B, C, gx, gy);
  SGCN_LAUNCH_CHECK();
  return 0;
}

size_t sgcn_tshift_bwd_ws_bytes(int B, int C) { return (size_t)B * C * sizeof(float2); }

int sgcn_tshift_pos_finalize_many(const void* const* partials, float* const* gx,
                                  float* const* gy, const int* B, const int* C, int n,
                                  void* stream) {
  SGCN_REQUIRE(n >= 0 && n <= SGCN_BATCH_MAX);
  if (n == 0) return 0;
  SGCN_REQUIRE(partials && gx && gy && B && C);
  PosBatch t{};
  int max_c = 0;
  for (int i = 0; i < n; ++i) {
    SGCN_REQUIRE(partials[i] && gx[i] && gy[i] && B[i] > 0 && C[i] > 0);
    t.p[i] = (const float2*)partials[i];
    t.gx[i] = gx[i];
    t.gy[i] = gy[i];
    t.B[i] = B[i];
    t.C[i] = C[i];
    max_c = max(max_c, C[i]);
  }
  tshift_pos_finalize_many_kernel<<<dim3((max_c + 3) / 4, n), 256, 0, (hipStream_t)stream>>>(t);
  SGCN_LAUNCH_CHECK();
  return 0;
}

int sgcn_tshift_pos_finalize(const void* ws, int B, int C, float* gx, float* gy, void* stream) {
  SGCN_REQUIRE(B > 0 && C > 0 && ws && gx && gy);
  tshift_pos_finalize_kernel<<<(C + 3) / 4, 256, 0, (hipStream_t)stream>>>((const float2*)ws, B,
                                                                           C, gx, gy);
  SGCN_LAUNCH_CHECK();
  return 0;
}

int sgcn_tshift_bwd_gbn(const float* gout, const float* in, const float* xpos,
                        const float* ypos, const float* in_scale, const float* in_shift,
                        const float* bn_mean, const float* bn_invstd, float* bn_part,
                        const float* z, const float* z_mean, const float* z_invstd,
                        float* z_part, const float* d, const float* d_mean,
                        const float* d_invstd, float* d_part, float* gin, float* gx, float* gy,
                        void* ws, size_t ws_bytes, int B, int C, int H, int W, void* stream) {
  SGCN_REQUIRE(B > 0 && C > 0 && H > 0 && W > 0 && W <= 64);
  SGCN_REQUIRE((d == nullptr) == (d_part == nullptr) && (!d || (d_mean && d_invstd)));
  SGCN_REQUIRE(H * W <= kBwdLdsMax);
  SGCN_REQUIRE(gout && in && xpos && ypos && in_scale && in_shift && bn_mean && bn_invstd &&
               bn_part && z && z_mean && z_invstd && z_part && gin && ws);
  SGCN_REQUIRE((gx == nullptr) == (gy == nullptr));
  SGCN_REQUIRE(ws_bytes >= sgcn_tshift_bwd_ws_bytes(B, C));
  SGCN_REQUIRE((long long)B * C < (1LL << 31));
  hipStream_t st = (hipStream_t)stream;
  float2* pg = (float2*)ws;
  float2* bp = (float2*)bn_part;
  const int n = H * W;
  const int l256 = n <= kRaSplit256 ? ra_lpt(n, 256, W) : 0;
  const int ntg = l256 && !(SGCN_GBD_SPLIT && d && l256 > 24) ? 256 : kBwdThreads;
  const bool ok =
      d ? launch_ra<true, false, true, false, true, true>(
              ntg, gout, in, xpos, ypos, in_scale, in_shift, bn_mean, bn_invstd, gin, pg, bp, B,
              C, H, W, nullptr, nullptr, nullptr, nullptr, z, z_mean, z_invstd, z_part, st, d,
              d_mean, d_invstd, d_part)
        : launch_ra<true, false, true, false, true>(
              ntg, gout, in, xpos, ypos, in_scale, in_shift, bn_mean, bn_invstd, gin, pg, bp, B,
              C, H, W, nullptr, nullptr, nullptr, nullptr, z, z_mean, z_invstd, z_part, st);
  SGCN_REQUIRE(ok);
  SGCN_LAUNCH_CHECK();
  if (gx) tshift_pos_finalize_kernel<<<(C + 3) / 4, 256, 0, st>>>(pg, B, C, gx, gy);
  SGCN_LAUNCH_CHECK();
  return 0;
}

int sgcn_tshift_bwd(const float* gout, const float* in, const float* xpos, const float* ypos,
                    const float* in_scale, const float* in_shift, int relu_mask,
                    const float* bn_mean, const float* bn_invstd, float* bn_part, float* gin,
                    float* gx, float* gy, void* ws, size_t ws_bytes, int B, int C, int H,
                    int W, int stride, int ypos_is_raw, void* stream) {
  SGCN_REQUIRE(B > 0 && C > 0 && H >= 0 && W > 0 && (stride == 1 || stride == 2));
  SGCN_REQUIRE((in_scale == nullptr) == (in_shift == nullptr));
  const int Ho = H / stride;
  SGCN_REQUIRE((gout || Ho == 0) && (in || H == 0) && (gin || H == 0));
  SGCN_REQUIRE(xpos && ypos && ws && (gx == nullptr) == (gy == nullptr));
  SGCN_REQUIRE(!bn_part || (bn_mean && bn_invstd));
  SGCN_REQUIRE(ws_bytes >= sgcn_tshift_bwd_ws_bytes(B, C));
  SGCN_REQUIRE((long long)H * W < (1LL << 30) && (long long)B * C < (1LL << 31));
  hipStream_t st = (hipStream_t)stream;
  const bool aff = in_scale != nullptr, relu = relu_mask != 0;
  float2* pg = (float2*)ws;
  float2* bp = (float2*)bn_part;
  const int ah = (ypos_is_raw && stride != 1) ? 1 : 0;
  if (stride == 1 && H > 0) {
    const int nt1 = H * W <= kRaSplit256 && ra_lpt(H * W, 256, W) ? 256 : kBwdThreads;
    bool done;
#define SGCN_RA1(A, R, P)                                                                       done = launch_ra<A, R, P, false, false>(nt1, gout, in, xpos, ypos, in_scale, in_shift,                                                 bn_mean, bn_invstd, gin, pg, bp, B, C, H, W, nullptr,                                           nullptr, nullptr, nullptr, nullptr, nullptr, nullptr,                                           nullptr, st)
    if (bp) {
      if (aff) { if (relu) SGCN_RA1(true, true, true); else SGCN_RA1(true, false, true); }
      else { if (relu) SGCN_RA1(false, true, true); else SGCN_RA1(false, false, true); }
    } else {
      if (aff) { if (relu) SGCN_RA1(true, true, false); else SGCN_RA1(true, false, false); }
      else { if (relu) SGCN_RA1(false, true, false); else SGCN_RA1(false, false, false); }
    }
#undef SGCN_RA1
    if (done) {
      SGCN_LAUNCH_CHECK();
      if (gx) tshift_pos_finalize_kernel<<<(C + 3) / 4, 256, 0, st>>>(pg, B, C, gx, gy);
      SGCN_LAUNCH_CHECK();
      return 0;
    }
  }
  if (stride == 2 && (H + Ho) * W <= kBwdLdsMax && H > 0) {
    const int lpt = pick_lpt((H + Ho) * W, kBwdThreads);
#define SGCN_BWDL_LPT(L, J)                                                                   \
  launch_bwd_s2<L, J>(aff, relu, gout, in, xpos, ypos, in_scale, in_shift, bn_mean, bn_invstd, \
                      gin, pg, bp, B, C, H, W, Ho, ah, st)
    if (W <= 64) {
      if (lpt == 8) SGCN_BWDL_LPT(8, true); else if (lpt == 16) SGCN_BWDL_LPT(16, true);
      else SGCN_BWDL_LPT(32, true);
    } else {
      if (lpt == 8) SGCN_BWDL_LPT(8, false); else if (lpt == 16) SGCN_BWDL_LPT(16, false);
      else SGCN_BWDL_LPT(32, false);
    }
#undef SGCN_BWDL_LPT
  } else {
  const int ept = pick_ept(H * W);
#define SGCN_BWD_EPT(E)                                                                     \
  (stride == 1 ? launch_bwd<E, 1>(aff, relu, gout, in, xpos, ypos, in_scale, in_shift, \
                                  bn_mean, bn_invstd, gin, pg, bp, B, C, H, W, Ho, ah, st)                                   \
               : launch_bwd<E, 2>(aff, relu, gout, in, xpos, ypos, in_scale, in_shift, \
                                  bn_mean, bn_invstd, gin, pg, bp, B, C, H, W, Ho, ah, st))
  if (ept == 8) SGCN_BWD_EPT(8); else if (ept == 16) SGCN_BWD_EPT(16); else SGCN_BWD_EPT(32);
#undef SGCN_BWD_EPT
  }
  SGCN_LAUNCH_CHECK();
  if (gx) tshift_pos_finalize_kernel<<<(C + 3) / 4, 256, 0, st>>>(pg, B, C, gx, gy);
  SGCN_LAUNCH_CHECK();
  return 0;
}

}
```

shift-gcn_amd/shiftgcn/_lib.py:

```python
from __future__ import annotations

import ctypes
import os

import torch

LIB_NAME = "libshiftgcn_hip.so"
LIB_PATH = os.path.join(os.path.dirname(os.path.abspath(__file__)), LIB_NAME)
LIB_PATH = os.environ.get("SGCN_LIB_PATH", LIB_PATH)
ABI_VERSION = 24
BATCH_MAX = 32
ABI_DIAG_FLAG = 0x10000
EINVAL = -22

_lib = None

_P = ctypes.c_void_p
_I = ctypes.c_int
_F = ctypes.c_float
_Z = ctypes.c_size_t
_L = ctypes.c_longlong

SIGNATURES = {
    "sgcn_abi_version": (_I, []),
    "sgcn_sgd_chunk_elems": (_I, []),
    "sgcn_sgd_step": (_I, [_P, _P, _P, _I, _F, _I, _P]),
    "sgcn_tshift_fwd": (_I, [_P, _P, _P, _P, _P, _P, _P, _I, _I, _I, _I, _I, _I, _P]),
    "sgcn_tshift_fwd_pre": (_I, [_P, _P, _P, _P, _P, _P, _P, _P, _P, _P, _P, _I, _I, _I, _I,
                                 _I, _I, _P]),
    "sgcn_tshift_fwd_tail": (_I, [_P, _P, _P, _P, _P, _P, _P, _P, _P, _P, _P, _I, _I, _I, _I,
                                  _I, _I, _P]),
    "sgcn_tshift_bwd_ws_bytes": (_Z, [_I, _I]),
    "sgcn_tshift_pos_finalize": (_I, [_P, _I, _I, _P, _P, _P]),
    "sgcn_tshift_bwd": (_I, [_P, _P, _P, _P, _P, _P, _I, _P, _P, _P, _P, _P, _P, _P, _Z, _I,
                             _I, _I, _I, _I, _I, _P]),
    "sgcn_tshift_fwd_f64": (_I, [_P, _P, _P, _P, _I, _I, _I, _I, _I, _I, _P]),
    "sgcn_tshift_bwd_f64_ws_bytes": (_Z, [_I, _I]),
    "sgcn_tshift_bwd_f64": (_I, [_P, _P, _P, _P, _P, _P, _P, _P, _Z, _I, _I, _I, _I, _I, _I,
                                 _P]),
    "sgcn_pw_fwd": (_I, [_P, _I, _P, _P, _L, _L, _I, _I, _P, _P, _L, _L, _I, _I, _I, _I, _I,
                         _I, _I, _I, _I, _P]),
    "sgcn_pw_tshift_ws_bytes": (_Z, [_I]),
    "sgcn_pw_fwd_tshift": (_I, [_P, _P, _P, _L, _L, _P, _P, _P, _P, _P, _P, _Z, _P, _L, _L, _I,
                                _I, _I, _I, _I, _I, _I, _P]),
    "sgcn_pw_dw_ws_bytes": (_Z, [_I, _I, _I, _I, _I]),
    "sgcn_pw_dw": (_I, [_P, _L, _L, _I, _I, _P, _L, _L, _I, _I, _P, _P, _I, _I, _P, _I, _P, _Z,
                        _I, _I, _I, _I, _I, _P]),
    "sgcn_moments_ws_bytes": (_Z, [_I, _I, _I, _I]),
    "sgcn_moments": (_I, [_P, _P, _I, _I, _I, _I, _I, _P]),
    "sgcn_bn_finalize": (_I, [_P, _I, _I, _I, _I, _P, _P, _F, _F, _P, _P, _P, _P, _P, _P, _P,
                              _P]),
    "sgcn_bn_eval_coef": (_I, [_I, _I, _P, _P, _P, _P, _F, _P, _P, _P, _P, _P]),
    "sgcn_bn_apply": (_I, [_P, _P, _P, _I, _P, _P, _P, _I, _P, _P, _P, _P, _I, _I, _I, _I,
                           _P]),
    "sgcn_bn_bwd_reduce": (_I, [_P, _P, _I, _P, _P, _P, _I, _P, _P, _P, _P, _P, _P, _I, _I, _I,
                                _I, _I, _P]),
    "sgcn_bn_bwd_finalize": (_I, [_P, _I, _I, _L, _I, _P, _P, _P, _P, _P, _I, _I, _P, _P]),
    "sgcn_bn_bwd_apply": (_I, [_P, _P, _I, _P, _P, _I, _P, _P, _P, _P, _P, _I, _I, _I, _I,
                               _P]),
    "sgcn_mask_prep": (_I, [_P, _P, _I, _P]),
    "sgcn_gcn_gather": (_I, [_P, _P, _P, _I, _I, _I, _I, _P]),
    "sgcn_gcn_dx_finish": (_I, [_P, _P, _P, _P, _P, _P, _P, _P, _P, _P, _P, _P, _I, _I, _I, _I,
                                _I, _P]),
    "sgcn_tshift_bwd_bnin": (_I, [_P, _P, _P, _P, _P, _P, _P, _P, _P, _P, _P, _Z, _I, _I, _I,
                                  _I, _I, _I, _P]),
    "sgcn_mask_grad_finalize": (_I, [_P, _P, _I, _I, _I, _P, _I, _P]),
    "sgcn_modalities": (_I, [_P, _P, _P, _P, _P, _P, _P, _P, _I, _I, _I, _I, _I, _I, _P]),
    "sgcn_tshift_bwd_gbn": (_I, [_P, _P, _P, _P, _P, _P, _P, _P, _P, _P, _P, _P, _P, _P, _P, _P,
                                 _P, _P, _P, _P, _P, _Z, _I, _I, _I, _I, _P]),
    "sgcn_bn_bwd_finalize_gbn": (_I, [_P, _I, _I, _I, _L, _P, _P, _P, _P, _P, _P, _P, _I, _I,
                                      _P, _P]),
    "sgcn_head_ws_bytes": (_Z, [_I, _I, _I, _I]),
    "sgcn_head_moments": (_I, [_P, _P, _I, _I, _I, _I, _I, _P]),
    "sgcn_head_apply": (_I, [_P, _P, _P, _P, _I, _I, _I, _I, _I, _P]),
    "sgcn_head_bwd_reduce": (_I, [_P, _P, _P, _P, _P, _I, _I, _I, _I, _I, _P]),
    "sgcn_head_bwd_apply": (_I, [_P, _P, _P, _P, _I, _I, _I, _I, _I, _P]),
    "sgcn_pool": (_I, [_P, _P, _I, _I, _I, _L, _P]),
    "sgcn_pool_bwd": (_I, [_P, _P, _I, _I, _I, _L, _P]),
    "sgcn_pool_bwd_planes": (_I, [_P, _P, _I, _I, _I, _L, _P]),
    "sgcn_tshift_pos_finalize_many": (_I, [_P, _P, _P, _P, _P, _I, _P]),
    "sgcn_mask_prep_many": (_I, [_P, _P, _P, _I, _P]),
    "sgcn_mask_grad_finalize_many": (_I, [_P, _P, _P, _P, _P, _P, _I, _P]),
}


class NativeLibraryError(RuntimeError):
    pass


def _open(path):
    lib = ctypes.CDLL(path, mode=ctypes.RTLD_LOCAL)
    lib.sgcn_abi_version.restype = _I
    lib.sgcn_abi_version.argtypes = []
    abi = lib.sgcn_abi_version()
    if abi & ABI_DIAG_FLAG:
        if os.environ.get("SGCN_ALLOW_DIAG_LIB") != "1" or os.path.basename(path) == LIB_NAME:
            raise NativeLibraryError(
                f"{path} is a DIAGNOSTIC build (SGCN_PW_DIAG / SGCN_PW_STAMPS / SGCN_DIAG_*: "
                "its results are wrong); rebuild with `make -C shift-gcn_amd/csrc`")
        abi &= ~ABI_DIAG_FLAG
    if abi != ABI_VERSION:
        raise NativeLibraryError(f"{path}: ABI version {abi} != {ABI_VERSION}; rebuild it")
    for name, (res, args) in SIGNATURES.items():
        fn = getattr(lib, name)
        fn.restype = res
        fn.argtypes = args
    return lib


def load():
    global _lib
    if _lib is not None:
        return _lib
    if not os.path.exists(LIB_PATH):
        raise NativeLibraryError(
            f"{LIB_PATH} not found: build it with `python -c 'import __graft_entry__ as g; "
            f"g.build()'` (or `make -C shift-gcn_amd/csrc`). There is no CPU fallback.")
    _lib = _open(LIB_PATH)
    return _lib


def check(rc: int, name: str) -> None:
    if rc == 0:
        return
    if rc == EINVAL:
        raise ValueError(f"{name}: invalid argument (shape/pointer/stride)")
    raise RuntimeError(f"{name}: HIP error {rc}")
```

shift-gcn_amd/shiftgcn/fused.py:

```python
from __future__ import annotations

import collections
import os
import threading

import torch

from . import ops
from .ops import PlaneView as PV


def _empty(*shape, like):
    return torch.empty(shape, device=like.device, dtype=torch.float32)


_SIDE = {}


def _side_stream(device):
    s = _SIDE.get(device)
    if s is None:
        s = _SIDE[device] = torch.cuda.Stream(device=device)
    return s

# ... 42 lines not shown

    def __init__(self, t):
        self.t = t


def _late(t, off):
    return _Later(t) if off else t


class _Task:

    __slots__ = ("pos", "mask", "grads", "side")

    def __init__(self):
        self.pos, self.mask, self.grads, self.side = [], [], [], False


_TASKS = {}


def _task(device):
    key = (device, torch._C._current_graph_task_id())
    t = _TASKS.get(key)
    if t is None:
        t = _TASKS[key] = _Task()
        torch.autograd.Variable._execution_engine.queue_callback(lambda: _finish(key))
    return t


def _defer_ok(params):
    if torch.is_grad_enabled():
        return False
    for p in params:
        if (getattr(p, "_backward_hooks", None) or
                getattr(p, "_post_accumulate_grad_hooks", None)):
            return False
        try:
            if not torch._C._will_engine_execute_node(
                    torch.autograd.graph.get_gradient_edge(p).node):
                return False
        except RuntimeError:
            return False
    return True


def _accumulate(p, g):
    cur = p.grad
    if cur is None:
        p.grad = g
    elif ops.is_grad_slot(p, g) and not ops.is_grad_slot(p, cur):
        g.add_(cur)
        p.grad = g
    else:
        cur.add_(g)


def _finish(key):
    t = _TASKS.pop(key, None)
    if t is None:
        return
    dev = key[0]
    if t.pos or t.mask:
        keep = [e[0].ws for e in t.pos] + [e[0] for e in t.mask]
        with _OffPath(t.side and not (TAIL_MAIN & 1), *keep):
            ops.pos_finalize_many(t.pos)
            ops.mask_grad_finalize_many(t.mask)
    s = _SIDE.get(dev)
    if t.side and s is not None:
        torch.cuda.current_stream(dev).wait_stream(s)
    for p, g in t.grads:
        _accumulate(p, g)


def _pos_grads(gx, gy, shift):
    if not isinstance(gx, ops.PosPartials):
        return gx, gy
    ox, oy = ops.grad_like(shift.xpos), ops.grad_like(shift.ypos)
    if BATCH_SIDE:
        _task(gx.ws.device).pos.append((gx, ox, oy))
    else:
        with _OffPath(True, gx.ws):
            gx.finalize(ox, oy)
    return _Later(ox), _Later(oy)


def _pos_alloc(shift, off):
    return None if off else (ops.grad_like(shift.xpos), ops.grad_like(shift.ypos))


TAIL_MAIN = int(os.environ.get("SGCN_TAIL_MAIN", "3"))


class GcnSaved:
    __slots__ = ("x0", "xg", "Z", "zst", "D0", "dst", "H", "m", "h_moments")


def gcn_forward(mod, x0, training, off=False, gathered=None, prepared=None):
    B, Cin, T, V = x0.shape
    Cout = mod.out_channels
    D0 = dst = None
    if mod.has_down:
        conv, bn = mod.down[0], mod.down[1]
        D0 = _empty(B, Cout, T, V, like=x0)
        down = _OffPath(off, x0)
        with down:
            ops.pw_fwd(conv.weight, False, conv.bias, PV(x0), PV(D0), Cout, Cin, T, V)
            if training:
                dst = ops.bn_finalize(ops.moments(D0, False), B, Cout, T * V, bn)
            else:
                dst = ops.bn_eval_coef(bn, Cout)
    if gathered is not None:
        xg, m = gathered
    else:
        m = _mask_of(mod, prepared)
        xg = ops.gcn_gather(x0, m)
    Z = _empty(B, Cout, T, V, like=x0)
    ops.pw_fwd(mod.Linear_weight, True, mod.Linear_bias, PV(xg), PV(Z), Cout, Cin, T, V)
    if training:
        zst = ops.bn_finalize(ops.moments(Z, 3), B, Cout * V, T, mod.bn, perm_V=V)
    else:
        zst = ops.bn_eval_coef(mod.bn, Cout * V, perm_V=V)
    if mod.has_down:
        down.wait()
        H, hm = ops.bn_apply(Z, zst, 3, r=D0, rst=dst, relu=True, out_stats=training)
    else:
        H, hm = ops.bn_apply(Z, zst, 3, r=x0, relu=True, out_stats=training)
    s = GcnSaved()
    s.x0, s.xg, s.Z, s.zst, s.D0, s.dst, s.H, s.m = x0, xg, Z, zst, D0, dst, H, m
    s.h_moments = hm
    return H, s


def _mask_of(gcn, prepared=None):
    fm = gcn.Feature_Mask
    if prepared is not None and prepared[0] is fm and prepared[1] == fm._version:
        return prepared[2]
    if gcn.training:
        return ops.mask_prep(fm)
    return ops.cached(gcn, "_sgcn_mask", ops._src_key((fm,)), lambda: ops.mask_prep(fm),
                      fm.device)


def prepare_masks(gcns):
    fms = [g.Feature_Mask for g in gcns]
    if any(g.training for g in gcns):
        ms = ops.mask_prep_many(fms)
    else:
        ms = ops.cached(gcns[0], "_sgcn_masks", ops._src_key(fms) + tuple(map(id, gcns)),
                        lambda: ops.mask_prep_many(fms), fms[0].device)
    return [(fm, fm._version, m) for fm, m in zip(fms, ms)]


def gcn_backward(mod, s: GcnSaved, dH, extra_dx=None, dy_coef=None, prev=None, pre6=None,
                 off=False, mask_dx=False):
    x0 = s.x0
    assert not (mask_dx and mod.has_down)
    B, Cin, T, V = x0.shape
    Cout = mod.out_channels
    g = {}
    rpart = None
    if pre6 is not None:
        assert dy_coef is not None and (pre6[2] is not None) == mod.has_down
        coefZ, g["bn.weight"], g["bn.bias"] = ops.bn_bwd_finalize_gbn(
            pre6[0], B, Cout, V, B * T, dy_coef, pre6[1], s.zst, mod.bn)
    else:
        if mod.has_down:
            conv, bnd = mod.down[0], mod.down[1]
            part, rpart = ops.bn_bwd_reduce(dH, s.H, True, s.Z, s.zst, 3, r=s.D0,
                                            rst=s.dst, dy_coef=dy_coef)
        else:
            part, rpart = ops.bn_bwd_reduce(dH, s.H, True, s.Z, s.zst, 3, dy_coef=dy_coef)
        coefZ, g["bn.weight"], g["bn.bias"] = ops.bn_bwd_finalize(part, B, Cout * V, B * T,
                                                                   s.zst, mod.bn, perm_V=V)
    dZ = _empty(B, Cout, T, V, like=x0)
    g_id = dD0 = None
    if mod.has_down:
        conv, bnd = mod.down[0], mod.down[1]
        if pre6 is not None:
            coefD, g["down.1.weight"], g["down.1.bias"] = ops.bn_bwd_finalize_gbn(
                pre6[2], B, Cout, 1, B * T * V, dy_coef, pre6[1], s.dst, bnd)
        else:
            coefD, g["down.1.weight"], g["down.1.bias"] = ops.bn_bwd_finalize(
                rpart, B, Cout, B * T * V, s.dst, bnd)
        dD0 = _empty(B, Cout, T, V, like=x0)
        ops.bn_bwd_apply(dH, s.H, True, s.Z, coefZ, 3, r=s.D0, rcoef=coefD, dr=dD0, dx=dZ,
                         dy_coef=dy_coef)
    else:
        g_id = _empty(B, Cin, T, V, like=x0)
        ops.bn_bwd_apply(dH, s.H, True, s.Z, coefZ, 3, dr=g_id, dx=dZ, dy_coef=dy_coef)
    dLW = ops.grad_like(mod.Linear_weight)
    dLb = ops.grad_like(mod.Linear_bias)
    dXt = _empty(B, Cin, T, V, like=x0)
    ops.pw_fwd(mod.Linear_weight, False, None, PV(dZ), PV(dXt), Cin, Cout, T, V)
    with _OffPath(off, dZ, s.xg):
        ops.pw_dw(PV(dZ), PV(s.xg), dLW, Cout, Cin, T, V, transpose=True, dbias=dLb)
    g["Linear_weight"], g["Linear_bias"] = _late(dLW, off), _late(dLb, off)
    a2, a2m = extra_dx or (None, None)
    res = ops.gcn_dx_finish(dXt, x0, s.m, add1=g_id, add2=a2, prev=prev, add2_mask=a2m,
                            mask_dx=mask_dx)
    dx, mpart, prev_part = res if prev is not None else (*res, None)
    dmask = ops.grad_like(mod.Feature_Mask)
    fm = mod.Feature_Mask
    if BATCH_SIDE and (off or _defer_ok((fm,))):
        _task(mpart.device).mask.append((mpart, fm, B, Cin, V, dmask))
        g["Feature_Mask"] = _Later(dmask)
    else:
        with _OffPath(off, mpart):
            ops.mask_grad_finalize(mpart, fm, B, Cin, V, out=dmask)
        g["Feature_Mask"] = _late(dmask, off)
    if mod.has_down:
        dWd = ops.grad_like(conv.weight)
        dbd = ops.grad_like(conv.bias)
        ops.pw_fwd(conv.weight, True, None, PV(dD0), PV(dx), Cin, Cout, T, V, accumulate=True)
        with _OffPath(off, dD0, x0):
            ops.pw_dw(PV(dD0), PV(x0), dWd, Cout, Cin, T, V, dbias=dbd)
        g["down.0.weight"], g["down.0.bias"] = _late(dWd, off), _late(dbd, off)
    return dx, g, prev_part


class TcnSaved:
    __slots__ = ("H", "ast", "As", "R", "S", "sst")


def tshift_fused(C):
    return C >= TSHIFT_FUSION_MIN_C


def folded_conv_bn(conv, bn):
    srcs = (conv.weight, conv.bias, bn.weight, bn.bias, bn.running_mean, bn.running_var)
    key = ops._src_key(srcs) + (float(bn.eps),)

    def make():
        st = ops.bn_eval_coef(bn, conv.out_channels)
        with torch.no_grad():
            w = (conv.weight.detach() *
                 st.scale.view(-1, *([1] * (conv.weight.dim() - 1)))).contiguous()
            b = (conv.bias.detach() * st.scale + st.shift if conv.bias is not None
                 else st.shift.clone())
        return w, b
    return ops.cached(conv, "_sgcn_fold", key, make, conv.weight.device)


def convbn_infer_folded(mod, x):
    B, Cin, T, V = x.shape
    conv = mod.conv
    Cout = conv.out_channels
    To = (T - 1) // mod.stride + 1
    w, b = folded_conv_bn(conv, mod.bn)
    R = _empty(B, Cout, To, V, like=x)
    ops.pw_fwd(w, False, b, PV(x, mod.stride), PV(R), Cout, Cin, To, V)
    return R


def gcn_infer_z(mod, x0, gathered=None, prepared=None):
    B, Cin, T, V = x0.shape
    Cout = mod.out_channels
    if gathered is not None:
        xg = gathered[0]
    else:
        xg = ops.gcn_gather(x0, _mask_of(mod, prepared))
    Z = _empty(B, Cout, T, V, like=x0)
    ops.pw_fwd(mod.Linear_weight, True, mod.Linear_bias, PV(xg), PV(Z, 1, +1), Cout, Cin, T, V)
    zst = ops.bn_eval_coef(mod.bn, Cout * V, perm_V=V)
    if mod.has_down:
        conv, bn = mod.down[0], mod.down[1]
        D0 = _empty(B, Cout, T, V, like=x0)
        if EVAL_FOLD:
            w, b = folded_conv_bn(conv, bn)
            ops.pw_fwd(w, False, b, PV(x0), PV(D0), Cout, Cin, T, V)
            return Z, zst, D0, None
        ops.pw_fwd(conv.weight, False, conv.bias, PV(x0), PV(D0), Cout, Cin, T, V)
        return Z, zst, D0, ops.bn_eval_coef(bn, Cout)
    return Z, zst, x0, None


def tcn_core_forward(mod, H, training, h_moments=None, tail=None, pre=None):
    src = H if H is not None else pre[0]
    B, C, T, V = src.shape
    Cout = mod.out_channels
    si, so = mod.shift_in, mod.shift_out
    stride = so.stride
    if training:
        if h_moments is None:
            h_moments = ops.moments(H, False)
        ast = ops.bn_finalize(h_moments, B, C, T * V, mod.bn)
    else:
        ast = ops.bn_eval_coef(mod.bn, C)
    R = _empty(B, Cout, T, V, like=src)
    tl = mod.temporal_linear
    As = None
    if pre is not None:
        As = ops.tshift_fwd_pre(pre[0], si.xpos.detach(), si.ypos.detach(), si.stride, pre[1],
                                pre[2], pre[3], ast)
        ops.pw_fwd(tl.weight, False, tl.bias, PV(As), PV(R), Cout, C, T, V, relu=True)
    elif tshift_fused(C) and tail is None:
        As = torch.empty_like(H)
        ops.pw_fwd_tshift(tl.weight, tl.bias, PV(H), si.xpos.detach(), si.ypos.detach(), ast,
                          PV(R), Cout, C, T, V, relu=True, x_shifted=As, two_row=TSHIFT_TWO_ROW)
    else:
        As = ops.tshift_fwd(H, si.xpos.detach(), si.ypos.detach(), si.stride, affine=ast)
        ops.pw_fwd(tl.weight, False, tl.bias, PV(As), PV(R), Cout, C, T, V, relu=True)
    To = T // stride
    if tail is not None:
        sst = ops.bn_eval_coef(mod.bn2, Cout)
        return ops.tshift_fwd_tail(R, so.xpos.detach(), so.ypos.detach(), stride, sst,
                                   r=tail[0], rst=tail[1], gather_m=tail[2])
    stats = _empty(B * Cout * 2, like=src) if training else None
    S = ops.tshift_fwd(R, so.xpos.detach(), so.ypos.detach(), stride, stats=stats)
    if training:
        sst = ops.bn_finalize(stats, B, Cout, To * V, mod.bn2)
    else:
        sst = ops.bn_eval_coef(mod.bn2, Cout)
    s = TcnSaved()
    s.H, s.ast, s.As, s.R, s.S, s.sst = H, ast, As, R, S, sst
    return S, sst, s


def tcn_core_backward(mod, s: TcnSaved, dS, materialize_dx=True, gpre=None, gcn_z=None,
                      off=False):
    H = s.H
    B, C, T, V = H.shape
    Cout = mod.out_channels
    si, so = mod.shift_in, mod.shift_out
    g, pre6 = {}, None
    if gpre is not None:
        dRp, gx, gy = ops.tshift_bwd_bnin(gpre[0], gpre[1], s.S, gpre[2], s.R,
                                          so.xpos.detach(), so.ypos.detach(), defer_pos=off,
                                          pos_out=_pos_alloc(so, off))
    else:
        dRp, gx, gy = ops.tshift_bwd(dS, s.R, so.xpos.detach(), so.ypos.detach(), so.stride,
                                     relu_mask=True, defer_pos=off,
                                     pos_out=_pos_alloc(so, off))
    g["shift_out.xpos"], g["shift_out.ypos"] = _pos_grads(gx, gy, so)
    tl = mod.temporal_linear
    dWt = ops.grad_like(tl.weight)
    dbt = ops.grad_like(tl.bias)

    dAs = _empty(B, C, T, V, like=H)
    ops.pw_fwd(tl.weight, True, None, PV(dRp), PV(dAs), C, Cout, T, V)
    with _OffPath(off, dRp, s.As):
        ops.pw_dw(PV(dRp), PV(s.As), dWt, Cout, C, T, V, dbias=dbt)
    g["temporal_linear.weight"], g["temporal_linear.bias"] = _late(dWt, off), _late(dbt, off)
    if gcn_z is not None and GBN_FUSION and si.stride == 1 and ops.ra_fits(T * V, V):
        down = gcn_z[2] if len(gcn_z) > 2 else None
        res = ops.tshift_bwd_gbn(dAs, H, si.xpos.detach(), si.ypos.detach(), s.ast, gcn_z[0],
                                 gcn_z[1], defer_pos=off, down=down,
                                 pos_out=_pos_alloc(si, off))
        dA, gx, gy, part, zpart = res[:5]
        pre6 = (zpart, s.ast, res[5] if down is not None else None)
    else:
        dA, gx, gy, part = ops.tshift_bwd(
            dAs, H, si.xpos.detach(), si.ypos.detach(), si.stride, scale=s.ast.scale,
            shift=s.ast.shift, bn_stats=s.ast, defer_pos=off, pos_out=_pos_alloc(si, off))
    g["shift_in.xpos"], g["shift_in.ypos"] = _pos_grads(gx, gy, si)
    coef, g["bn.weight"], g["bn.bias"] = ops.bn_bwd_finalize(part, B, C, B * T * V, s.ast,
                                                             mod.bn)
    if not materialize_dx:
        return (dA, coef), g, pre6
    dH = ops.bn_bwd_apply(dA, None, False, H, coef, False)
    return dH, g, pre6


class ConvBnSaved:
    __slots__ = ("x", "Rc", "rst", "To")


def convbn_core_forward(mod, x, training):
    B, Cin, T, V = x.shape
    conv, bn = mod.conv, mod.bn
    Cout = conv.out_channels
    s_t = mod.stride
    To = (T - 1) // s_t + 1
    Rc = _empty(B, Cout, To, V, like=x)
    ops.pw_fwd(conv.weight, False, conv.bias, PV(x, s_t), PV(Rc), Cout, Cin, To, V)
    if training:
        rst = ops.bn_finalize(ops.moments(Rc, False), B, Cout, To * V, bn)
    else:
        rst = ops.bn_eval_coef(bn, Cout)
    s = ConvBnSaved()
    s.x, s.Rc, s.rst, s.To = x, Rc, rst, To
    return Rc, rst, s


def convbn_dx_and_dw(mod, s: ConvBnSaved, dRc, dx, accumulate, off=False):
    B, Cin, T, V = s.x.shape
    conv = mod.conv
    Cout = conv.out_channels
    dW = ops.grad_like(conv.weight)
    db = ops.grad_like(conv.bias)
    ops.pw_fwd(conv.weight, True, None, PV(dRc), PV(dx, mod.stride), Cin, Cout, s.To, V,
               accumulate=accumulate)
    with _OffPath(off, dRc, s.x):
        ops.pw_dw(PV(dRc), PV(s.x, mod.stride), dW, Cout, Cin, s.To, V, dbias=db)
    return {"conv.weight": _late(dW, off), "conv.bias": _late(db, off)}


class _Link:

    __slots__ = ("out", "xg", "gm", "tail", "full", "dx", "prev_part", "masked")

    def __init__(self):
        self.out = self.xg = self.gm = self.tail = self.dx = self.prev_part = None
        self.full = self.masked = False

    def take(self, x):
        r = ((self.xg, self.gm), self.tail, self.full) if self.out is x else (None, None, False)
        self.out = self.xg = self.gm = self.tail = None
        self.full = False
        return r


_Pos = collections.namedtuple("_Pos", "link_in link_out nxt off mask nxt_mask",
                              defaults=(None, None, None, False, None, None))


def chain_positions(units):
    masks = prepare_masks([u.gcn1 for u in units])
    links = [None] + [_Link() for _ in units[1:]] + [None]
    nxt, masks = list(units[1:]) + [None], masks + [None]
    return [_Pos(links[i], links[i + 1], nxt[i], bool(i or not TAIL_MAIN & 2), masks[i],
                 masks[i + 1]) for i in range(len(units))]


class UnitSaved:
    __slots__ = ("x", "gs", "ts", "rs", "out", "link_in", "link_out", "prev", "full", "off")


def unit_forward(unit, x, training):
    pos = unit.__dict__.get("_link_pos") or _Pos()
    li, lo, nxt = pos.link_in, pos.link_out, pos.nxt
    gathered, prev, full = li.take(x) if li is not None else (None, None, False)
    li = li if gathered is not None else None
    if (not training and _INFER.active and
            x.shape[2] * x.shape[3] <= ops.TAIL_MAX_PLANE):
        pre = gcn_infer_z(unit.gcn1, x, gathered, pos.mask)
        r = rst = None
        if unit.residual_kind == "conv":
            if EVAL_FOLD:
                r = convbn_infer_folded(unit.residual, x)
            else:
                r, rst, _ = convbn_core_forward(unit.residual, x, training)
        elif unit.residual_kind == "identity":
            r = x
        gm = _mask_of(nxt.gcn1, pos.nxt_mask) if lo is not None else None
        out, xg_next = tcn_core_forward(unit.tcn1, None, training, tail=(r, rst, gm),
                                        pre=pre)
        if lo is not None:
            lo.out, lo.xg, lo.gm, lo.tail, lo.full = out, xg_next, gm, None, False
        return out, None
    off = ASYNC_DW and pos.off and not torch.cuda.is_current_stream_capturing()
    gm = _mask_of(nxt.gcn1, pos.nxt_mask) if lo is not None else None
    H, gs = gcn_forward(unit.gcn1, x, training, off=off, gathered=gathered,
                        prepared=pos.mask)
    rs = None
    if unit.residual_kind == "conv":
        res = _OffPath(off, x)
        with res:
            Rc, rst, rs = convbn_core_forward(unit.residual, x, training)
    S, sst, ts = tcn_core_forward(unit.tcn1, H, training, h_moments=gs.h_moments)
    if unit.residual_kind == "conv":
        res.wait()
        out = ops.bn_apply(S, sst, False, r=Rc, rst=rst, relu=True, gather_m=gm)
    elif unit.residual_kind == "identity":
        out = ops.bn_apply(S, sst, False, r=x, relu=True, gather_m=gm)
    else:
        out = ops.bn_apply(S, sst, False, relu=True, gather_m=gm)
    if lo is not None:
        out, lo.xg = out
        lo.out, lo.gm = out, gm
        lo.full = nxt.residual_kind != "conv" and not nxt.gcn1.has_down
        lo.tail = (S, sst) if lo.full and unit.residual_kind != "conv" else None
    s = UnitSaved()
    s.x, s.gs, s.ts, s.rs, s.out, s.off = x, gs, ts, rs, out, off
    s.link_in, s.link_out, s.prev, s.full = li, lo, prev, full
    return out, s


def _gcn_z(unit, s: UnitSaved):
    if unit.gcn1.has_down:
        return (s.gs.Z, s.gs.zst, (s.gs.D0, s.gs.dst)) if GBN_FUSION >= 2 else None
    return (s.gs.Z, s.gs.zst)


def _off_path_ok(unit, s: UnitSaved):
    if not s.off or torch.cuda.is_current_stream_capturing():
        return False
    if not _defer_ok([p for p in unit.parameters() if p.requires_grad]):
        return False
    _task(s.x.device).side = True
    return True


def unit_backward(unit, s: UnitSaved, dout):
    return _unit_backward(unit, s, dout, _off_path_ok(unit, s))


def _premask_ok(unit, x, off):
    if not PREMASK or torch.cuda.is_current_stream_capturing():
        return False
    if getattr(x, "_backward_hooks", None) or x.retains_grad or x.grad_fn is None:
        return False
    if not off:
        params = [p for p in unit.parameters() if p.requires_grad]
        if not params or not _defer_ok(params):
            return False
    try:
        return bool(torch._C._will_engine_execute_node(x.grad_fn))
    except RuntimeError:
        return False


def _fused_tail(unit, To, V):
    return (unit.residual_kind != "conv" and unit.tcn1.shift_out.stride == 1 and
            ops.ra_fits(To * V, V))


def premasked(s: UnitSaved, dout):
    lo = s.link_out
    return lo is not None and lo.masked and lo.dx is dout


def _unit_backward(unit, s: UnitSaved, dout, off):
    ts = s.ts
    S = ts.S
    B, Cout, To, V = S.shape
    kind = unit.residual_kind
    li, lo = s.link_in, s.link_out
    g = {}
    y, relu = (None, False) if premasked(s, dout) else (s.out, True)
    mask_dx = s.full and _premask_ok(unit, s.x, off)
    part = rpart = None
    if lo is not None:
        if lo.dx is dout:
            part = lo.prev_part
        lo.dx, lo.prev_part, lo.masked = None, None, False
    if part is None:
        r, rst = (s.rs.Rc, s.rs.rst) if kind == "conv" else (None, None)
        part, rpart = ops.bn_bwd_reduce(dout, y, relu, S, ts.sst, False, r=r, rst=rst)
    coef2, g["tcn1.bn2.weight"], g["tcn1.bn2.bias"] = ops.bn_bwd_finalize(
        part, B, Cout, B * To * V, ts.sst, unit.tcn1.bn2)
    dS = gpre = dres = extra = None
    if _fused_tail(unit, To, V):
        gpre = (dout, y, coef2)
        if kind == "identity":
            extra = (dout, y)
    else:
        dS = torch.empty_like(S)
        if kind == "conv":
            coefR, g["residual.bn.weight"], g["residual.bn.bias"] = ops.bn_bwd_finalize(
                rpart, B, Cout, B * To * V, s.rs.rst, unit.residual.bn)
            dres = torch.empty_like(s.rs.Rc)
            ops.bn_bwd_apply(dout, y, relu, S, coef2, False, r=s.rs.Rc, rcoef=coefR, dr=dres,
                             dx=dS)
        else:
            if kind == "identity":
                dres = torch.empty_like(s.x)
                extra = (dres, None)
            ops.bn_bwd_apply(dout, y, relu, S, coef2, False, dr=dres, dx=dS)
    (dA, coefA), gt, pre6 = tcn_core_backward(unit.tcn1, ts, dS, materialize_dx=False,
                                              gpre=gpre, gcn_z=_gcn_z(unit, s), off=off)
    dx, gg, prev_part = gcn_backward(unit.gcn1, s.gs, dA, extra_dx=extra, dy_coef=coefA,
                                     prev=s.prev, pre6=pre6, off=off, mask_dx=mask_dx)
    if s.prev is not None or mask_dx:
        li.dx, li.prev_part, li.masked = dx, prev_part, mask_dx
    g.update({"tcn1." + k: v for k, v in gt.items()})
    g.update({"gcn1." + k: v for k, v in gg.items()})
    if kind == "conv":
        gr = convbn_dx_and_dw(unit.residual, s.rs, dres, dx, accumulate=True, off=off)
        g.update({"residual." + k: v for k, v in gr.items()})
    return dx, g


TSHIFT_FUSION_MIN_C = int(os.environ.get("SGCN_TSHIFT_FUSION_MIN_C", "512"))
TSHIFT_TWO_ROW = int(os.environ.get("SGCN_TSHIFT_TWO_ROW", "2"))
EVAL_FOLD = int(os.environ.get("SGCN_EVAL_FOLD", "1"))
GBN_FUSION = int(os.environ.get("SGCN_GBN_FUSION", "2"))
ASYNC_DW = int(os.environ.get("SGCN_ASYNC_DW", "1"))
PREMASK = int(os.environ.get("SGCN_PREMASK", "1"))


def trainable(module):
    return [(n, p) for n, p in module.named_parameters() if p.requires_grad]


class _BlockFunction(torch.autograd.Function):

    @staticmethod
    def forward(ctx, impl, module, x, *params):
        fwd, bwd = impl
        training = module.training
        y, saved = fwd(module, x.contiguous(), training)
        ctx.impl, ctx.module, ctx.saved, ctx.training = impl, module, saved, training
        tr = trainable(module)
        ctx.names, ctx.params = [n for n, _ in tr], [p for _, p in tr]
        ctx.save_for_backward(x, y)
        return y

    @staticmethod
    def backward(ctx, dy):
        ctx.saved_tensors
        if ctx.saved is None:
            raise RuntimeError(
                f"{type(ctx.module).__name__}: backward through the fused HIP block was "
                "called a second time; its saved activations are released after the first "
                "backward (retain_graph=True / double backward is not supported)")
        _, bwd = ctx.impl
        dyp = _unit_dy_planes(ctx, dy)
        dx, grads = bwd(ctx.module, ctx.saved, dy.contiguous() if dyp is None else dyp)
        ctx.saved = None
        out = []
        for n, p in zip(ctx.names, ctx.params):
            g = grads.get(n)
            if isinstance(g, _Later):
                _task(g.t.device).grads.append((p, g.t))
                g = None
            out.append(g)
        return (None, None, dx) + tuple(out)


def _unit_dy_planes(ctx, dy):
    if not (PREMASK and ctx.impl is UNIT_IMPL and dy.dim() == 4 and dy.stride(2) == 0 and
            dy.stride(3) == 0 and isinstance(ctx.saved, UnitSaved) and
            _fused_tail(ctx.module, dy.shape[2], dy.shape[3])):
        return None
    return dy[:, :, 0, 0].contiguous()


class _InferFlag(threading.local):
    active = False


_INFER = _InferFlag()


def run_block(impl, module, x):
    params = [p for _, p in trainable(module)]
    prev = _INFER.active
    _INFER.active = not (torch.is_grad_enabled() and
                         (x.requires_grad or any(p.requires_grad for p in params)))
    try:
        return _BlockFunction.apply(impl, module, x, *params)
    finally:
        _INFER.active = prev


def _tcn_standalone_fwd(mod, H, training):
    S, sst, ts = tcn_core_forward(mod, H, training)
    y = ops.bn_apply(S, sst, False)
    return y, ts


def _tcn_standalone_bwd(mod, ts, dy):
    S = ts.S
    B, C, To, V = S.shape
    part, _ = ops.bn_bwd_reduce(dy, None, False, S, ts.sst, False)
    coef, dg, db = ops.bn_bwd_finalize(part, B, C, B * To * V, ts.sst, mod.bn2)
    dS = ops.bn_bwd_apply(dy, None, False, S, coef, False)
    dH, g, _ = tcn_core_backward(mod, ts, dS)
    g["bn2.weight"], g["bn2.bias"] = dg, db
    return dH, g


def _convbn_standalone_fwd(mod, x, training):
    Rc, rst, s = convbn_core_forward(mod, x, training)
    return ops.bn_apply(Rc, rst, False), s


def _convbn_standalone_bwd(mod, s, dy):
    B, C, To, V = s.Rc.shape
    part, _ = ops.bn_bwd_reduce(dy, None, False, s.Rc, s.rst, False)
    coef, dg, db = ops.bn_bwd_finalize(part, B, C, B * To * V, s.rst, mod.bn)
    dRc = ops.bn_bwd_apply(dy, None, False, s.Rc, coef, False)
    dx = torch.zeros_like(s.x)
    g = convbn_dx_and_dw(mod, s, dRc, dx, accumulate=True)
    g["bn.weight"], g["bn.bias"] = dg, db
    return dx, g


GCN_IMPL = (gcn_forward, lambda mod, s, dy: gcn_backward(mod, s, dy)[:2])
TCN_IMPL = (_tcn_standalone_fwd, _tcn_standalone_bwd)
CONVBN_IMPL = (_convbn_standalone_fwd, _convbn_standalone_bwd)
UNIT_IMPL = (unit_forward, unit_backward)
```

shift-gcn_amd/shiftgcn/ops.py:

```python
from __future__ import annotations

import ctypes

import torch

from . import _lib

_F32 = torch.float32


def _ptr(t):
    if t is None:
        return None
    return t.data_ptr()


class LaunchTimer:

    def __init__(self, ops_filter=None, detail=False):
        self.ops_filter = ops_filter
        self.detail = detail
        self.records = []

    def begin(self, op, flops, nbytes, device):
# ... 264 lines not shown
            _ptr(inp), _ptr(out), _ptr(xpos), _ptr(ypos), _ptr(st.scale), _ptr(st.shift),
            _ptr(r), _ptr(rst.scale) if rst else None, _ptr(rst.shift) if rst else None,
            _ptr(gather_m), _ptr(og), B, C, H, W, stride, 1, _stream(inp))
    _lib.check(rc, "sgcn_tshift_fwd_tail")
    return out, og


class PosPartials:

    __slots__ = ("ws", "B", "C")

    def __init__(self, ws, B, C):
        self.ws, self.B, self.C = ws, B, C

    def finalize(self, gx, gy):
        check_input(gx, "gx")
        check_input(gy, "gy")
        with _timed("finalize", 0, self.ws.numel() * 4, self.ws):
            rc = _lib.load().sgcn_tshift_pos_finalize(_ptr(self.ws), self.B, self.C, _ptr(gx),
                                                      _ptr(gy), _stream(self.ws))
        _lib.check(rc, "sgcn_tshift_pos_finalize")
        return gx, gy


def _pos_out(defer_pos, ws, B, C, dev, pos_out=None):
    if defer_pos:
        return None, None, PosPartials(ws, B, C)
    if pos_out is not None:
        for t, n in zip(pos_out, ("grad_xpos", "grad_ypos")):
            check_input(t, n)
            if t.numel() != C:
                raise ValueError(f"{n} must hold {C} elements")
        return pos_out[0], pos_out[1], None
    return (torch.empty((C,), device=dev, dtype=_F32), torch.empty((C,), device=dev, dtype=_F32),
            None)


def tshift_bwd(gout, inp, xpos, ypos, stride, scale=None, shift=None, relu_mask=False,
               ypos_is_raw=True, bn_stats=None, defer_pos=False, pos_out=None):
    if inp.dtype == torch.float64:
        if (scale is not None or shift is not None or relu_mask or bn_stats is not None):
            raise RuntimeError("the fused shift options are float32-only")
        return _tshift_bwd_f64(gout, inp, xpos, ypos, stride, ypos_is_raw)
    check_input(gout, "grad_output")
    check_input(inp, "input")
    check_input(xpos, "xpos")
    check_input(ypos, "ypos")
    _opt(scale, "scale"), _opt(shift, "shift")
    B, C, H, W = inp.shape
    lib = _lib.load()
    dev = inp.device
    gin = torch.empty_like(inp)
    nbytes = lib.sgcn_tshift_bwd_ws_bytes(B, C)
    ws = torch.empty((max(nbytes, 4) + 3) // 4, device=dev, dtype=_F32)
    gx, gy, pp = _pos_out(defer_pos, ws, B, C, dev, pos_out)
    bpart = torch.empty((B * C * 2,), device=dev, dtype=_F32) if bn_stats is not None else None
    nb = 4 * (gout.numel() + 2 * inp.numel())
    with _timed("tshift_bwd", 0, nb, inp, _shp(inp)):
        rc = lib.sgcn_tshift_bwd(_ptr(gout), _ptr(inp), _ptr(xpos), _ptr(ypos), _ptr(scale),
                                 _ptr(shift), int(bool(relu_mask)),
                                 _ptr(bn_stats.mean) if bn_stats is not None else None,
                                 _ptr(bn_stats.invstd) if bn_stats is not None else None,
                                 _ptr(bpart), _ptr(gin), _ptr(gx), _ptr(gy), _ptr(ws), nbytes,
                                 B, C, H, W, stride, int(ypos_is_raw), _stream(inp))
    _lib.check(rc, "sgcn_tshift_bwd")
    if pp is not None:
        gx = pp
    if bn_stats is not None:
        return gin, gx, gy, bpart
    return gin, gx, gy


GBN_MAX_PLANE = 16384


def ra_fits(n, V):
    if V > 64 or n > GBN_MAX_PLANE:
        return False
    if (n // V + 2 * 4) * (V + 2) + 1 > 16384:
        return False
    nt = 256 if n <= 4096 else 512
    return -(-n // ((nt // V) * V)) <= 32


def tshift_bwd_gbn(gout, inp, xpos, ypos, st: "BnStats", z, zst: "BnStats", defer_pos=False,
                   down=None, pos_out=None):
    check_input(gout, "grad_output")
    check_input(inp, "input")
    check_input(z, "z")
    if down is not None:
        check_input(down[0], "d")
    B, C, H, W = inp.shape
    lib = _lib.load()
    dev = inp.device
    gin = torch.empty_like(inp)
    nbytes = lib.sgcn_tshift_bwd_ws_bytes(B, C)
    ws = torch.empty((max(nbytes, 4) + 3) // 4, device=dev, dtype=_F32)
    gx, gy, pp = _pos_out(defer_pos, ws, B, C, dev, pos_out)
    bpart = torch.empty((B * C * 2,), device=dev, dtype=_F32)
    zpart = torch.empty((6 * B * C * W,), device=dev, dtype=_F32)
    d, dst, dpart = None, None, None
    if down is not None:
        d, dst = down
        dpart = torch.empty((6 * B * C,), device=dev, dtype=_F32)
    nb = 4 * (gout.numel() + (3 if down is None else 4) * inp.numel())
    with _timed("tshift_bwd", 0, nb, inp, ("GBND " if down is not None else "GBN ") + _shp(inp)):
        rc = lib.sgcn_tshift_bwd_gbn(_ptr(gout), _ptr(inp), _ptr(xpos), _ptr(ypos),
                                     _ptr(st.scale), _ptr(st.shift), _ptr(st.mean),
                                     _ptr(st.invstd), _ptr(bpart), _ptr(z), _ptr(zst.mean),
                                     _ptr(zst.invstd), _ptr(zpart), _ptr(d),
                                     _ptr(dst.mean if dst is not None else None),
                                     _ptr(dst.invstd if dst is not None else None),
                                     _ptr(dpart), _ptr(gin), _ptr(gx), _ptr(gy), _ptr(ws),
                                     nbytes, B, C, H, W, _stream(inp))
    _lib.check(rc, "sgcn_tshift_bwd_gbn")
    if down is not None:
        return gin, (pp if pp is not None else gx), gy, bpart, zpart, dpart
    return gin, (pp if pp is not None else gx), gy, bpart, zpart


BNIN_MAX_PLANE = 16384


def _plane_dy(dy, x):
    if dy.dim() == 2:
        if tuple(dy.shape) != tuple(x.shape[:2]):
            raise ValueError(f"per-plane gradient {tuple(dy.shape)} of planes {tuple(x.shape)}")
        return True
    return False


def tshift_bwd_bnin(dy, y, s, coef, inp, xpos, ypos, defer_pos=False, pos_out=None):
    for t, n in ((dy, "dy"), (y, "y"), (s, "s"), (inp, "input"), (coef, "coef")):
        if t is not None:
            check_input(t, n)
    B, C, H, W = inp.shape
    dyp = _plane_dy(dy, inp)
    lib = _lib.load()
    dev = inp.device
    gin = torch.empty_like(inp)
    nbytes = lib.sgcn_tshift_bwd_ws_bytes(B, C)
    ws = torch.empty((max(nbytes, 4) + 3) // 4, device=dev, dtype=_F32)
    gx, gy, pp = _pos_out(defer_pos, ws, B, C, dev, pos_out)
    nb = 4 * (dy.numel() + (2 + (y is not None)) * s.numel() + inp.numel())
    with _timed("tshift_bwd", 0, nb, inp, _shp(inp)):
        rc = lib.sgcn_tshift_bwd_bnin(
            _ptr(dy), _ptr(y), _ptr(s), _ptr(coef), _ptr(inp), _ptr(xpos), _ptr(ypos),
            _ptr(gin), _ptr(gx), _ptr(gy), _ptr(ws), nbytes, B, C, H, W, 1, int(dyp),
            _stream(inp))
    _lib.check(rc, "sgcn_tshift_bwd_bnin")
    return gin, (pp if pp is not None else gx), gy


class PlaneView:

    __slots__ = ("t", "bstride", "cstride", "tstride", "rsign")

    def __init__(self, t, tstride=1, rsign=0):
        check_input(t, "plane operand")
        self.t = t
        self.bstride = t.stride(0)
        self.cstride = t.stride(1)
        self.tstride = tstride
        self.rsign = rsign


PW_MAX_ELEMS = 1 << 29


def _plane_extent(v: PlaneView, B, C, T, V):
    return (B - 1) * v.bstride + C * v.cstride + T * v.tstride * V


def _batch_chunk(views, B, T, V):
    bc = B
    for v, C in views:
        per = v.bstride
        fixed = C * v.cstride + T * v.tstride * V
        if fixed >= PW_MAX_ELEMS:
            raise ValueError("pointwise operand plane too large for one sample")
        if (B - 1) * per + fixed >= PW_MAX_ELEMS:
            bc = min(bc, max(1, (PW_MAX_ELEMS - 1 - fixed) // max(per, 1) + 1))
    return bc


def pw_fwd(w, w_mcontig, bias, x: PlaneView, out: PlaneView, M, K, T, V, mask=None,
           relu=False, accumulate=False):
    check_input(w, "weight")
    _opt(bias, "bias"), _opt(mask, "mask")
    B = x.t.shape[0]
    lib = _lib.load()
    P = B * T * V
    bc = _batch_chunk([(x, K), (out, M)], B, T, V)
    det = (f"M{M} K{K} T{T} V{V} xrot{x.rsign} yrot{out.rsign} mask{int(mask is not None)} "
           f"ts{x.tstride}{out.tstride} acc{int(accumulate)} mc{int(w_mcontig)}")
    with _timed("pw_fwd", 2.0 * P * M * K, 4.0 * P * (M * (2 if accumulate else 1) + K), x.t,
                det):
        for b0 in range(0, B, bc):
            nb = min(bc, B - b0)
            rc = lib.sgcn_pw_fwd(_ptr(w), int(w_mcontig), _ptr(bias),
                                 x.t.data_ptr() + 4 * b0 * x.bstride, x.bstride,
                                 x.cstride, x.tstride, x.rsign, _ptr(mask),
                                 out.t.data_ptr() + 4 * b0 * out.bstride,
                                 out.bstride, out.cstride, out.tstride, out.rsign, int(relu),
                                 int(accumulate), nb, M, K, T, V, _stream(x.t))
            _lib.check(rc, "sgcn_pw_fwd")
    return out.t


def pw_dw(g: PlaneView, x: PlaneView, dw, M, Nc, T, V, mask=None, transpose=False,
          accumulate=False, dbias=None, dbias_accumulate=False):
    check_input(dw, "dw")
    _opt(dbias, "dbias"), _opt(mask, "mask")
    B = g.t.shape[0]
    lib = _lib.load()
    bc = _batch_chunk([(g, M), (x, Nc)], B, T, V)
    nbytes = lib.sgcn_pw_dw_ws_bytes(bc, M, Nc, T, V)
    ws = torch.empty((nbytes + 3) // 4, device=g.t.device, dtype=_F32)
    P = B * T * V
    det = (f"M{M} N{Nc} T{T} V{V} grot{g.rsign} xrot{x.rsign} mask{int(mask is not None)} "
           f"ts{g.tstride}{x.tstride}")
    with _timed("pw_dw", 2.0 * P * M * Nc, 4.0 * P * (M + Nc), g.t, det):
        for b0 in range(0, B, bc):
            nb = min(bc, B - b0)
            first = b0 == 0
            rc = lib.sgcn_pw_dw(g.t.data_ptr() + 4 * b0 * g.bstride, g.bstride, g.cstride,
                                g.tstride, g.rsign, x.t.data_ptr() + 4 * b0 * x.bstride,
                                x.bstride, x.cstride, x.tstride, x.rsign, _ptr(mask),
                                _ptr(dw), int(transpose), int(accumulate or not first),
                                _ptr(dbias), int(dbias_accumulate or not first), _ptr(ws),
                                nbytes, nb, M, Nc, T, V, _stream(g.t))
            _lib.check(rc, "sgcn_pw_dw")
    return dw


def pw_fwd_tshift(w, bias, x: PlaneView, xpos, ypos, st, out: PlaneView, M, K, T, V,
                  relu=False, x_shifted=None, two_row=2):
    check_input(w, "weight")
    _opt(bias, "bias")
    if x.tstride != 1 or x.rsign != 0 or out.tstride != 1 or out.rsign != 0:
        raise ValueError("pw_fwd_tshift: plain planes only")
    B = x.t.shape[0]
    lib = _lib.load()
    P = B * T * V
    nbytes = lib.sgcn_pw_tshift_ws_bytes(K)
    ws = torch.empty((nbytes + 3) // 4, device=x.t.device, dtype=_F32)
    bc = _batch_chunk([(x, K), (out, M)], B, T, V)
    sc = st.scale if st is not None else None
    sh = st.shift if st is not None else None
    if x_shifted is not None:
        check_input(x_shifted, "x_shifted")
        if x_shifted.shape != x.t.shape or x_shifted.stride() != x.t.stride():
            raise ValueError("x_shifted must have the layout of x")
    nbx = 4.0 * P * (M + K * (2 if x_shifted is not None else 1))
    with _timed("pw_fwd", 2.0 * P * M * K, nbx, x.t,
                f"TSH M{M} K{K} T{T} V{V} side{int(x_shifted is not None)}"):
        for b0 in range(0, B, bc):
            nb = min(bc, B - b0)
            xs = None if x_shifted is None else x_shifted.data_ptr() + 4 * b0 * x.bstride
            rc = lib.sgcn_pw_fwd_tshift(_ptr(w), _ptr(bias), x.t.data_ptr() + 4 * b0 * x.bstride,
                                        x.bstride, x.cstride, _ptr(xpos), _ptr(ypos), _ptr(sc),
                                        _ptr(sh), xs, _ptr(ws), nbytes,
                                        out.t.data_ptr() + 4 * b0 * out.bstride, out.bstride,
                                        out.cstride, int(relu), int(two_row), nb, M, K, T, V,
                                        _stream(x.t))
            _lib.check(rc, "sgcn_pw_fwd_tshift")
    return out.t


def moments(x, per_joint):
    check_input(x, "input")
    B, C, T, V = x.shape
    part = torch.empty((B * C * (V if per_joint else 1) * 2,), device=x.device, dtype=_F32)
    with _timed("bn_stats", 0, 4 * x.numel(), x, _shp(x)):
        rc = _lib.load().sgcn_moments(_ptr(x), _ptr(part), B, C, T, V, int(per_joint),
                                      _stream(x))
    _lib.check(rc, "sgcn_moments")
    return part


class BnStats:

    __slots__ = ("mean", "invstd", "scale", "shift", "buf", "batch")

    def __init__(self, F, device, batch=True):
        buf = torch.empty((4, F), device=device, dtype=_F32)
        self.buf = buf
        self.mean, self.invstd, self.scale, self.shift = buf[0], buf[1], buf[2], buf[3]
        self.batch = batch


def bn_finalize(part, B, F, n_part, bn, perm_V=0, training=True):
    st = BnStats(F, part.device)
    lib = _lib.load()
    track = training and bn.track_running_stats and bn.running_mean is not None
    if track and bn.momentum is None:
        raise NotImplementedError("BatchNorm momentum=None is not supported on the HIP path")
    momentum = bn.momentum if bn.momentum is not None else 0.0
    with _timed("finalize", 0, 4 * part.numel(), part):
        rc = lib.sgcn_bn_finalize(
            _ptr(part), B, F, n_part, perm_V, _ptr(bn.weight), _ptr(bn.bias), float(bn.eps),
            float(momentum), _ptr(bn.running_mean) if track else None,
            _ptr(bn.running_var) if track else None,
            _ptr(bn.num_batches_tracked) if track else None, _ptr(st.mean),
            _ptr(st.invstd), _ptr(st.scale), _ptr(st.shift), _stream(part))
    _lib.check(rc, "sgcn_bn_finalize")
# ... 32 lines not shown
    y = torch.empty_like(x) if out is None else out
    ys = torch.empty((B * C * 2,), device=x.device, dtype=_F32) if out_stats else None
    yg = torch.empty_like(y) if gather_m is not None else None
    nb = 4 * x.numel() * (2 + (r is not None) + (yg is not None))
    with _timed("bn_apply", 0, nb, x, _shp(x)):
        rc = _lib.load().sgcn_bn_apply(
            _ptr(x), _ptr(st.scale), _ptr(st.shift), int(per_joint), _ptr(r),
            _ptr(rst.scale) if rst is not None else None,
            _ptr(rst.shift) if rst is not None else None, int(relu), _ptr(y), _ptr(ys),
            _ptr(gather_m), _ptr(yg), B, C, T, V, _stream(x))
    _lib.check(rc, "sgcn_bn_apply")
    if gather_m is not None:
        return y, yg
    return y if out_stats is None else (y, ys)


def bn_bwd_reduce(dy, y, relu, x, st: BnStats, per_joint, r=None, rst: BnStats = None,
                  dy_coef=None):
    check_input(dy, "grad_output")
    B, C, T, V = x.shape
    dyp = _plane_dy(dy, x)
    dev = x.device
    part = torch.empty((B * C * (V if per_joint else 1) * 2,), device=dev, dtype=_F32)
    rpart = torch.empty((B * C * 2,), device=dev, dtype=_F32) if r is not None else None
    nb = 4 * (dy.numel() + x.numel() * (1 + (y is not None) + (r is not None)))
    with _timed("bn_bwd_reduce", 0, nb, x, _shp(x)):
        rc = _lib.load().sgcn_bn_bwd_reduce(_ptr(dy), _ptr(y), int(relu), _ptr(x),
                                            _ptr(st.mean), _ptr(st.invstd), int(per_joint),
                                            _ptr(r), _ptr(rst.mean) if rst else None,
                                            _ptr(rst.invstd) if rst else None, _ptr(dy_coef),
                                            _ptr(part), _ptr(rpart), B, C, T, V, int(dyp),
                                            _stream(x))
    _lib.check(rc, "sgcn_bn_bwd_reduce")
    return part, rpart


def bn_bwd_finalize(part, B, F, n_total, st: BnStats, bn, perm_V=0):
    dev = part.device
    coef = torch.empty((3, F), device=dev, dtype=_F32)
    dgamma = grad_like(bn.weight) if bn.weight is not None else None
    dbeta = grad_like(bn.bias) if bn.bias is not None else None
    with _timed("finalize", 0, 4 * part.numel(), part):
        rc = _lib.load().sgcn_bn_bwd_finalize(_ptr(part), B, F, int(n_total), perm_V,
                                              _ptr(st.mean), _ptr(st.invstd), _ptr(bn.weight),
                                              _ptr(dgamma), _ptr(dbeta), 0, int(st.batch),
                                              _ptr(coef), _stream(part))
    _lib.check(rc, "sgcn_bn_bwd_finalize")
    return coef, dgamma, dbeta


def bn_bwd_finalize_gbn(part6, B, C, V, n_total, dy_coef, dy_st: BnStats, st: BnStats, bn):
    dev = part6.device
    F = C * V
    coef = torch.empty((3, F), device=dev, dtype=_F32)
    dgamma = grad_like(bn.weight) if bn.weight is not None else None
    dbeta = grad_like(bn.bias) if bn.bias is not None else None
    with _timed("finalize", 0, 4 * part6.numel(), part6):
        rc = _lib.load().sgcn_bn_bwd_finalize_gbn(_ptr(part6), B, C, V, int(n_total),
                                                  _ptr(dy_coef), _ptr(dy_st.mean),
                                                  _ptr(st.mean), _ptr(st.invstd),
                                                  _ptr(bn.weight), _ptr(dgamma), _ptr(dbeta), 0,
                                                  int(st.batch), _ptr(coef), _stream(part6))
    _lib.check(rc, "sgcn_bn_bwd_finalize_gbn")
    return coef, dgamma, dbeta


def bn_bwd_apply(dy, y, relu, x, coef, per_joint, r=None, rcoef=None, dr=None, dx=None,
                 dy_coef=None):
    B, C, T, V = x.shape
    dx = torch.empty_like(x) if dx is None else dx
    nb = 4 * x.numel() * (3 + (y is not None) + (r is not None) + (dr is not None))
    with _timed("bn_bwd_apply", 0, nb, x, _shp(x)):
        rc = _lib.load().sgcn_bn_bwd_apply(
            _ptr(dy), _ptr(y), int(relu), _ptr(x), _ptr(coef), int(per_joint), _ptr(r),
            _ptr(rcoef), _ptr(dy_coef), _ptr(dx), _ptr(dr), B, C, T, V, _stream(x))
    _lib.check(rc, "sgcn_bn_bwd_apply")
    return dx


def mask_prep(mask):
    check_input(mask, "Feature_Mask")
    m = torch.empty_like(mask)
    with _timed("finalize", 0, 8 * mask.numel(), mask):
        rc = _lib.load().sgcn_mask_prep(_ptr(mask), _ptr(m), mask.numel(), _stream(mask))
    _lib.check(rc, "sgcn_mask_prep")
    return m


def _arr(ctype, vals):
    return (ctype * len(vals))(*vals)


def _chunks(xs):
    for i in range(0, len(xs), _lib.BATCH_MAX):
        yield xs[i:i + _lib.BATCH_MAX]


def mask_prep_many(masks):
    outs = []
    for ch in _chunks(list(masks)):
        for mk in ch:
            check_input(mk, "Feature_Mask")
        o = [torch.empty_like(mk) for mk in ch]
        with _timed("finalize", 0, 8 * sum(m.numel() for m in ch), ch[0]):
            rc = _lib.load().sgcn_mask_prep_many(
                _arr(ctypes.c_void_p, [m.data_ptr() for m in ch]),
                _arr(ctypes.c_void_p, [t.data_ptr() for t in o]),
                _arr(ctypes.c_int, [m.numel() for m in ch]), len(ch), _stream(ch[0]))
        _lib.check(rc, "sgcn_mask_prep_many")
        outs += o
    return outs


def pos_finalize_many(entries):
    for ch in _chunks(list(entries)):
        for _, gx, gy in ch:
            check_input(gx, "gx")
            check_input(gy, "gy")
        with _timed("finalize", 0, sum(pp.ws.numel() * 4 for pp, _, _ in ch), ch[0][1]):
            rc = _lib.load().sgcn_tshift_pos_finalize_many(
                _arr(ctypes.c_void_p, [pp.ws.data_ptr() for pp, _, _ in ch]),
                _arr(ctypes.c_void_p, [gx.data_ptr() for _, gx, _ in ch]),
                _arr(ctypes.c_void_p, [gy.data_ptr() for _, _, gy in ch]),
                _arr(ctypes.c_int, [pp.B for pp, _, _ in ch]),
                _arr(ctypes.c_int, [pp.C for pp, _, _ in ch]), len(ch), _stream(ch[0][1]))
        _lib.check(rc, "sgcn_tshift_pos_finalize_many")


def mask_grad_finalize_many(entries):
    for ch in _chunks(list(entries)):
        for e in ch:
            check_input(e[5], "dmask")
        with _timed("finalize", 0, sum(e[0].numel() * 4 for e in ch), ch[0][0]):
            rc = _lib.load().sgcn_mask_grad_finalize_many(
                _arr(ctypes.c_void_p, [e[0].data_ptr() for e in ch]),
                _arr(ctypes.c_void_p, [e[1].data_ptr() for e in ch]),
                _arr(ctypes.c_void_p, [e[5].data_ptr() for e in ch]),
                _arr(ctypes.c_int, [e[2] for e in ch]), _arr(ctypes.c_int, [e[3] for e in ch]),
                _arr(ctypes.c_int, [e[4] for e in ch]), len(ch), _stream(ch[0][0]))
        _lib.check(rc, "sgcn_mask_grad_finalize_many")


def gcn_gather(x0, m):
    B, C, T, V = x0.shape
    xg = torch.empty_like(x0)
    with _timed("gcn_gather", 0, 8 * x0.numel(), x0, _shp(x0)):
        rc = _lib.load().sgcn_gcn_gather(_ptr(x0), _ptr(m), _ptr(xg), B, C, T, V,
                                         _stream(x0))
    _lib.check(rc, "sgcn_gcn_gather")
    return xg


def gcn_dx_finish(dxt, x0, m, add1=None, add2=None, prev=None, add2_mask=None,
                  mask_dx=False):
    B, C, T, V = dxt.shape
    flags = int(bool(mask_dx)) | (2 if add2 is not None and _plane_dy(add2, dxt) else 0)
    dx = torch.empty_like(dxt)
    part = torch.empty((B * C * V,), device=dxt.device, dtype=_F32)
    pp = torch.empty((B * C * 2,), device=dxt.device, dtype=_F32) if prev is not None else None
    ps, pst = prev if prev is not None else (None, None)
    nb = 4 * (dxt.numel() * (3 + sum(t is not None for t in (add1, add2_mask, ps))) +
              (add2.numel() if add2 is not None else 0))
    with _timed("gcn_dx_finish", 0, nb, dxt, _shp(dxt)):
        rc = _lib.load().sgcn_gcn_dx_finish(_ptr(dxt), _ptr(x0), _ptr(m), _ptr(add1),
                                            _ptr(add2), _ptr(add2_mask), _ptr(dx), _ptr(part),
                                            _ptr(ps), _ptr(pst.mean) if pst else None,
                                            _ptr(pst.invstd) if pst else None, _ptr(pp), B, C,
                                            T, V, flags, _stream(dxt))
    _lib.check(rc, "sgcn_gcn_dx_finish")
    return (dx, part) if prev is None else (dx, part, pp)


def mask_grad_finalize(part, mask, B, C, V, out=None):
    dmask = torch.empty_like(mask) if out is None else out
    with _timed("finalize", 0, 4 * part.numel(), mask):
        rc = _lib.load().sgcn_mask_grad_finalize(_ptr(part), _ptr(mask), B, C, V, _ptr(dmask),
                                                 0, _stream(mask))
    _lib.check(rc, "sgcn_mask_grad_finalize")
    return dmask


def head_moments(x):
    check_input(x, "input")
    N, C, T, V, M = x.shape
    part = torch.empty((N * M * V * C * 2,), device=x.device, dtype=_F32)
    with _timed("head", 0, 4 * x.numel(), x):
        rc = _lib.load().sgcn_head_moments(_ptr(x), _ptr(part), N, C, T, V, M, _stream(x))
    _lib.check(rc, "sgcn_head_moments")
    return part


def head_apply(x, st: BnStats):
    N, C, T, V, M = x.shape
    y = torch.empty((N * M, C, T, V), device=x.device, dtype=_F32)
    with _timed("head", 0, 8 * x.numel(), x):
        rc = _lib.load().sgcn_head_apply(_ptr(x), _ptr(st.scale), _ptr(st.shift), _ptr(y), N, C,
                                         T, V, M, _stream(x))
    _lib.check(rc, "sgcn_head_apply")
    return y


def head_bwd_reduce(g, x, st: BnStats):
    check_input(g, "grad_output")
    N, C, T, V, M = x.shape
    part = torch.empty((N * M * V * C * 2,), device=x.device, dtype=_F32)
    with _timed("head", 0, 8 * x.numel(), x):
        rc = _lib.load().sgcn_head_bwd_reduce(_ptr(g), _ptr(x), _ptr(st.mean), _ptr(st.invstd),
                                              _ptr(part), N, C, T, V, M, _stream(x))
    _lib.check(rc, "sgcn_head_bwd_reduce")
    return part


def head_bwd_apply(g, x, coef):
    N, C, T, V, M = x.shape
    dx = torch.empty_like(x)
    with _timed("head", 0, 12 * x.numel(), x):
        rc = _lib.load().sgcn_head_bwd_apply(_ptr(g), _ptr(x), _ptr(coef), _ptr(dx), N, C, T, V,
                                             M, _stream(x))
    _lib.check(rc, "sgcn_head_bwd_apply")
    return dx


def pool(x, N, M):
    check_input(x, "input")
    C = x.shape[1]
    P = x.numel() // max(1, N * M * C)
    out = torch.empty((N, C), device=x.device, dtype=_F32)
    with _timed("pool", 0, 4 * x.numel(), x):
        rc = _lib.load().sgcn_pool(_ptr(x), _ptr(out), N, M, C, P, _stream(x))
    _lib.check(rc, "sgcn_pool")
    return out


def pool_bwd(dout, shape, N, M, planes=False):
    check_input(dout, "grad_output")
    C = shape[1]
    P = 1
    for d in shape[2:]:
        P *= d
    if planes:
        dp = torch.empty((N * M, C), device=dout.device, dtype=_F32)
        with _timed("pool", 0, 4 * (dout.numel() + dp.numel()), dout):
            rc = _lib.load().sgcn_pool_bwd_planes(_ptr(dout), _ptr(dp), N, M, C, P,
                                                  _stream(dout))
        _lib.check(rc, "sgcn_pool_bwd_planes")
        return dp
    dx = torch.empty(shape, device=dout.device, dtype=_F32)
    with _timed("pool", 0, 4 * dx.numel(), dout):
        rc = _lib.load().sgcn_pool_bwd(_ptr(dout), _ptr(dx), N, M, C, P, _stream(dout))
    _lib.check(rc, "sgcn_pool_bwd")
    return dx
```

Measured before the change: 2053 clips/s.

## Fuse stride-2 tshift backward with BN-apply and residual gradient in conv units

Adds a stride-2 variant of the BN-input temporal-shift backward kernel. It computes the BN/ReLU gradient from dy, y and s in-register and also emits the residual-branch BN gradient in the same pass. The residual conv's dx is now written compactly at the strided length and added as a stride-2 plane inside gcn_dx_finish. This replaces an accumulate-into-full-dx pass, removing separate bn_bwd_apply launches and extra full-size traffic for downsampling units. It adds template variants and bookkeeping, and uses contract-off adds to keep rounding the same as before.

```diff
diff --git a/include/shiftgcn.h b/include/shiftgcn.h
--- a/include/shiftgcn.h
+++ b/include/shiftgcn.h
@@ -8,7 +8,7 @@
 #endif
 
 #define SGCN_EINVAL (-22)
-#define SGCN_ABI_VERSION 24
+#define SGCN_ABI_VERSION 25
 #define SGCN_ABI_DIAG_FLAG 0x10000
 
 int sgcn_abi_version(void);
@@ -34,6 +34,11 @@
                          const float* in, const float* xpos, const float* ypos, float* gin,
                          float* gx, float* gy, void* ws, size_t ws_bytes, int B, int C, int H,
                          int W, int ypos_is_raw, int dy_plane, void* stream);
+int sgcn_tshift_bwd_s2_bnin(const float* dy, const float* y, const float* s, const float* coef,
+                            const float* r, const float* rcoef, float* dres, const float* in,
+                            const float* xpos, const float* ypos, float* gin, float* gx,
+                            float* gy, void* ws, size_t ws_bytes, int B, int C, int H, int W,
+                            int ypos_is_raw, void* stream);
 size_t sgcn_tshift_bwd_ws_bytes(int B, int C);
 
 int sgcn_tshift_pos_finalize(const void* ws, int B, int C, float* gx, float* gy, void* stream);
@@ -132,10 +137,12 @@
 
 #define SGCN_DXF_MASK_DX 1
 #define SGCN_DXF_ADD2_PLANE 2
+#define SGCN_DXF_ADD1_PLAIN 4
 int sgcn_gcn_dx_finish(const float* dxt, const float* x0, const float* m, const float* add1,
                        const float* add2, const float* add2_mask, float* dx, float* dmask_part,
                        const float* prev_s, const float* prev_mean, const float* prev_invstd,
-                       float* prev_part, int B, int C, int T, int V, int flags, void* stream);
+                       float* prev_part, int B, int C, int T, int V, int flags,
+                       int add2_stride, void* stream);
 
 int sgcn_mask_grad_finalize(const float* part, const float* mask, int B, int C, int V,
                             float* dmask, int accumulate, void* stream);
diff --git a/shift-gcn_amd/csrc/bn.hip b/shift-gcn_amd/csrc/bn.hip
--- a/shift-gcn_amd/csrc/bn.hip
+++ b/shift-gcn_amd/csrc/bn.hip
@@ -771,14 +771,19 @@
   }
 }
 
-template <int NT, int LPT, bool ADD1, bool ADD2, bool PART, int A2M>
+__device__ __forceinline__ float plain_add(float a, float b) {
+#pragma clang fp contract(off)
+  return a + b;
+}
+
+template <int NT, int LPT, int ADD1, bool ADD2, bool PART, int A2M>
 __global__ __launch_bounds__(NT) void gcn_dx_finish_ja_kernel(
     const float* __restrict__ dxt, const float* __restrict__ x0, const float* __restrict__ m,
     const float* __restrict__ add1, const float* __restrict__ add2, float* __restrict__ dx,
     float* __restrict__ dmask_part, const float* __restrict__ ps,
     const float* __restrict__ pmean, const float* __restrict__ pinvstd,
     float2* __restrict__ bn_part, int C, int T, int V, const float* __restrict__ add2m,
-    int flags) {
+    int flags, int T2) {
   SGCN_CRIT_PRIO();
 #ifdef SGCN_DIAG_F1B_REAL
   return;
@@ -798,7 +803,9 @@
   const unsigned uo = vo + (unsigned)((us - vd) * 4);
   const bool mdx = flags & SGCN_DXF_MASK_DX;
   constexpr bool A2P = A2M == 2;
-  float gv[LPT], xq[LPT], a1[ADD1 ? LPT : 1], a2[ADD2 && !A2P ? LPT : 1], a2q[A2M ? LPT : 1];
+  constexpr bool A2S = A2M == 3;
+  constexpr bool A2Q = A2M == 1 || A2M == 2;
+  float gv[LPT], xq[LPT], a1[ADD1 ? LPT : 1], a2[ADD2 && !A2P ? LPT : 1], a2q[A2Q ? LPT : 1];
   float sv[PART ? LPT : 1];
   {
 #ifdef SGCN_DIAG_F1B_BOUND
@@ -816,12 +823,19 @@
 #pragma unroll
       for (int e = 0; e < LPT; ++e) a1[e] = bload(ar, vo + e * vstep, 0);
     }
-    if (ADD2 && !A2P) {
+    if (ADD2 && A2S) {
+      const auto ar = make_rsrc(add2 + (size_t)plane * T2 * V, (unsigned)(T2 * V) * 4u);
+#pragma unroll
+      for (int e = 0; e < LPT; ++e) {
+        const int t = tid / V + e * GR;
+        a2[e] = bload(ar, own && !(t & 1) ? (unsigned)((t >> 1) * V + vd) * 4u : 0x80000000u, 0);
+      }
+    } else if (ADD2 && !A2P) {
       const auto ar = make_rsrc(add2 + off, pb);
 #pragma unroll
       for (int e = 0; e < LPT; ++e) a2[e] = bload(ar, vo + e * vstep, 0);
     }
-    if (A2M) {
+    if (A2Q) {
       const auto ar = make_rsrc(add2m + off, pb);
 #pragma unroll
       for (int e = 0; e < LPT; ++e) a2q[e] = bload(ar, vo + e * vstep, 0);
@@ -841,8 +855,13 @@
 #pragma unroll
   for (int e = 0; e < LPT; ++e) {
     float val = gv[e] * mu;
-    if (ADD1) val += a1[e];
-    if (ADD2) val += A2M ? (a2q[e] > 0.f ? (A2P ? a2v : a2[e]) : 0.f) : a2[e];
+    if (ADD1 == 1) val += a1[e];
+    if (ADD1 == 2) val = plain_add(val, a1[e]);
+    if (ADD2 && A2S) {
+      if (!((tid / V + e * GR) & 1)) val = plain_add(val, a2[e]);
+    } else if (ADD2) {
+      val += A2Q ? (a2q[e] > 0.f ? (A2P ? a2v : a2[e]) : 0.f) : a2[e];
+    }
     bstore(dxr, (xq[e] > 0.f || !mdx) ? val : 0.f, vo + e * vstep, 0);
     acc = fmaf(gv[e], xq[e], acc);
     if (PART) {
@@ -902,19 +921,20 @@
   }
 }
 
-template <bool ADD1, bool ADD2, bool PART, bool A2M = false>
+template <int ADD1, int ADD2, bool PART, bool A2M = false>
 __global__ __launch_bounds__(kThreads) void gcn_dx_finish_kernel(
     const float* __restrict__ dxt, const float* __restrict__ x0, const float* __restrict__ m,
     const float* __restrict__ add1, const float* __restrict__ add2, float* __restrict__ dx,
     float* __restrict__ dmask_part, const float* __restrict__ ps,
     const float* __restrict__ pmean, const float* __restrict__ pinvstd,
     float2* __restrict__ bn_part, int C, int T, int V, const float* __restrict__ add2m,
-    int flags) {
+    int flags, int T2) {
   SGCN_CRIT_PRIO();
   const bool mdx = flags & SGCN_DXF_MASK_DX, a2p = flags & SGCN_DXF_ADD2_PLANE;
+  constexpr bool a2s = ADD2 == 2;
   __shared__ float s0[kThreads];
   const int plane = blockIdx.x, c = plane % C;
-  const size_t off = (size_t)plane * T * V;
+  const size_t off = (size_t)plane * T * V, off2 = (size_t)plane * T2 * V;
   const int rc = c % V;
   const int i = threadIdx.x;
   const int G = kThreads / V;
@@ -930,11 +950,12 @@
       float gv[kU], xq[kU], a1[kU], a2[kU], sv[kU], a2q[kU];
 #pragma unroll
       for (int k = 0; k < kU; ++k) {
-        const int row = min(t0 + k * G, T - 1) * V;
+        const int tc = min(t0 + k * G, T - 1), row = tc * V;
         gv[k] = dxt[off + row + us];
         xq[k] = x0[off + row + vd];
         if (ADD1) a1[k] = add1[off + row + vd];
-        if (ADD2) a2[k] = a2p ? add2[plane] : add2[off + row + vd];
+        if (ADD2) a2[k] = a2p ? add2[plane]
+                              : (a2s ? add2[off2 + (tc >> 1) * V + vd] : add2[off + row + vd]);
         if (A2M) a2q[k] = add2m[off + row + vd];
         if (PART) sv[k] = ps[off + row + vd];
       }
@@ -942,8 +963,13 @@
       for (int k = 0; k < kU; ++k) {
         const int t = t0 + k * G;
         float val = gv[k] * mu;
-        if (ADD1) val += a1[k];
-        if (ADD2) val += A2M ? (a2q[k] > 0.f ? a2[k] : 0.f) : a2[k];
+        if (ADD1 == 1) val += a1[k];
+        if (ADD1 == 2) val = plain_add(val, a1[k]);
+        if (a2s) {
+          if (!(t & 1)) val = plain_add(val, a2[k]);
+        } else if (ADD2) {
+          val += A2M ? (a2q[k] > 0.f ? a2[k] : 0.f) : a2[k];
+        }
         if (t < T) dx[off + t * V + vd] = (xq[k] > 0.f || !mdx) ? val : 0.f;
         acc += (t < T) ? gv[k] * xq[k] : 0.f;
         if (PART) {
@@ -1431,11 +1457,15 @@
                        const float* add2, const float* add2_mask, float* dx, float* dmask_part,
                        const float* prev_s, const float* prev_mean, const float* prev_invstd,
                        float* prev_part, int B,
-                       int C, int T, int V, int flags, void* stream) {
+                       int C, int T, int V, int flags, int add2_stride, void* stream) {
   SGCN_PLANE_CHECK();
   if (B == 0 || T == 0) return 0;
   SGCN_REQUIRE(dxt && x0 && m && dx && dmask_part);
-  SGCN_REQUIRE((flags & ~(SGCN_DXF_MASK_DX | SGCN_DXF_ADD2_PLANE)) == 0);
+  SGCN_REQUIRE((flags & ~(SGCN_DXF_MASK_DX | SGCN_DXF_ADD2_PLANE | SGCN_DXF_ADD1_PLAIN)) == 0);
+  const bool a1p = flags & SGCN_DXF_ADD1_PLAIN;
+  SGCN_REQUIRE(!a1p || (add1 && !add2_mask));
+  SGCN_REQUIRE(add2_stride == 1 || (add2_stride == 2 && add2 && !add2_mask));
+  const int T2 = add2_stride == 2 ? (T + 1) / 2 : 0;
   SGCN_REQUIRE(!(flags & SGCN_DXF_ADD2_PLANE) || add2_mask);
   SGCN_REQUIRE(!prev_part || (prev_s && prev_mean && prev_invstd));
   SGCN_REQUIRE(!add2_mask || add2);
@@ -1449,7 +1479,7 @@
 #define SGCN_FJ(NT, L, A1, A2, PT, AM)                                                         \
   gcn_dx_finish_ja_kernel<NT, L, A1, A2, PT, AM><<<B * C, NT, 0, st>>>(                        \
       dxt, x0, m, add1, add2, dx, dmask_part, prev_s, prev_mean, prev_invstd, pp, C, T, V,     \
-      add2_mask, flags)
+      add2_mask, flags, T2)
 #define SGCN_FJ_L(NT, A1, A2, PT, AM)                                                          \
   do {                                                                                         \
     if (lpt == 8) SGCN_FJ(NT, 8, A1, A2, PT, AM);                                              \
@@ -1462,6 +1492,11 @@
 #define SGCN_FJ_P(A1, A2, AM)                                                                  \
   do { if (pp) SGCN_FJ_T(A1, A2, true, AM); else SGCN_FJ_T(A1, A2, false, AM); } while (0)
       if (add2_mask) { if (flags & SGCN_DXF_ADD2_PLANE) SGCN_FJ_P(true, true, 2); else SGCN_FJ_P(true, true, 1); }
+      else if (T2) {
+        if (a1p) SGCN_FJ_P(2, true, 3); else if (add1) SGCN_FJ_P(1, true, 3);
+        else SGCN_FJ_P(0, true, 3);
+      }
+      else if (a1p) { if (add2) SGCN_FJ_P(2, true, 0); else SGCN_FJ_P(2, false, 0); }
       else if (add1) { if (add2) SGCN_FJ_P(true, true, 0); else SGCN_FJ_P(true, false, 0); }
       else { if (add2) SGCN_FJ_P(false, true, 0); else SGCN_FJ_P(false, false, 0); }
 #undef SGCN_FJ_P
@@ -1476,24 +1511,28 @@
     if (pp)
       gcn_dx_finish_kernel<true, true, true, true><<<B * C, kThreads, 0, st>>>(
           dxt, x0, m, add1, add2, dx, dmask_part, prev_s, prev_mean, prev_invstd, pp, C, T, V,
-          add2_mask, flags);
+          add2_mask, flags, 0);
     else
       gcn_dx_finish_kernel<true, true, false, true><<<B * C, kThreads, 0, st>>>(
           dxt, x0, m, add1, add2, dx, dmask_part, prev_s, prev_mean, prev_invstd, pp, C, T, V,
-          add2_mask, flags);
+          add2_mask, flags, 0);
     SGCN_LAUNCH_CHECK();
     return 0;
   }
 #define SGCN_FIN(A1, A2, PT)                                                                \
   gcn_dx_finish_kernel<A1, A2, PT><<<B * C, kThreads, 0, st>>>(                           \
       dxt, x0, m, add1, add2, dx, dmask_part, prev_s, prev_mean, prev_invstd, pp, C, T, V,  \
-      nullptr, flags)
+      nullptr, flags, T2)
 #define SGCN_FIN_P(A1, A2)                                                                  \
   do {                                                                                      \
     if (pp) SGCN_FIN(A1, A2, true);                                                         \
     else SGCN_FIN(A1, A2, false);                                                           \
   } while (0)
-  if (add1) { if (add2) SGCN_FIN_P(true, true); else SGCN_FIN_P(true, false); }
+  if (T2) {
+    if (a1p) SGCN_FIN_P(2, 2); else if (add1) SGCN_FIN_P(1, 2); else SGCN_FIN_P(0, 2);
+  }
+  else if (a1p) { if (add2) SGCN_FIN_P(2, 1); else SGCN_FIN_P(2, 0); }
+  else if (add1) { if (add2) SGCN_FIN_P(true, true); else SGCN_FIN_P(true, false); }
   else { if (add2) SGCN_FIN_P(false, true); else SGCN_FIN_P(false, false); }
 #undef SGCN_FIN_P
 #undef SGCN_FIN
diff --git a/shift-gcn_amd/csrc/tshift.hip b/shift-gcn_amd/csrc/tshift.hip
--- a/shift-gcn_amd/csrc/tshift.hip
+++ b/shift-gcn_amd/csrc/tshift.hip
@@ -605,14 +605,19 @@
   }
 }
 
-template <int NT, int LPT, bool AFFINE, bool RELU_MASK, bool BNP, bool JA>
+template <int NT, int LPT, bool AFFINE, bool RELU_MASK, bool BNP, bool JA, int GP = 0,
+          bool RES = false>
 __global__ __launch_bounds__(NT) void tshift_bwd_s2_kernel(
     const float* __restrict__ gout, const float* __restrict__ in,
     const float* __restrict__ xpos, const float* __restrict__ ypos,
     const float* __restrict__ scale, const float* __restrict__ shift,
     const float* __restrict__ bn_mean, const float* __restrict__ bn_invstd,
     float* __restrict__ gin, float2* __restrict__ pgrad, float2* __restrict__ bn_part, int C,
-    int Hb, int W, int Ho, int add_half) {
+    int Hb, int W, int Ho, int add_half, const float* __restrict__ gdy = nullptr,
+    const float* __restrict__ gy = nullptr, const float* __restrict__ gx = nullptr,
+    const float* __restrict__ gcoef = nullptr, const float* __restrict__ gr = nullptr,
+    const float* __restrict__ grcoef = nullptr, float* __restrict__ gres = nullptr) {
+  static_assert(GP || !RES, "RES: the residual gradient of the GP form");
   SGCN_CRIT_PRIO();
   constexpr int STRIDE = 2;
   extern __shared__ float lds[];
@@ -628,7 +633,47 @@
   const float y = add_half ? ypos[c] + 0.5f : ypos[c];
   float a = 1.f, b = 0.f;
   if (AFFINE) { a = scale[c]; b = shift[c]; }
-  {
+  if (GP) {
+    constexpr int LG = LPT / 2;
+    const unsigned gb = (unsigned)nt * 4u, tb = threadIdx.x * 4u;
+    const size_t goff = (size_t)plane * nt;
+    float t[LG], u1[GP == 1 ? LG : 1], u2[LG], rv[RES ? LG : 1], xi[LPT];
+    const auto dyr = make_rsrc(gdy + goff, gb), sr = make_rsrc(gx + goff, gb);
+#pragma unroll
+    for (int e = 0; e < LG; ++e) {
+      t[e] = bload(dyr, tb + e * (NT * 4u), 0);
+      u2[e] = bload(sr, tb + e * (NT * 4u), 0);
+    }
+    if (GP == 1) {
+      const auto yr = make_rsrc(gy + goff, gb);
+#pragma unroll
+      for (int e = 0; e < LG; ++e) u1[e] = bload(yr, tb + e * (NT * 4u), 0);
+    }
+    if (RES) {
+      const auto rr = make_rsrc(gr + goff, gb);
+#pragma unroll
+      for (int e = 0; e < LG; ++e) rv[e] = bload(rr, tb + e * (NT * 4u), 0);
+    }
+    const auto inr = make_rsrc(in + (size_t)plane * nb, (unsigned)nb * 4u);
+#pragma unroll
+    for (int e = 0; e < LPT; ++e) xi[e] = bload(inr, tb + e * (NT * 4u), 0);
+    const float k1 = gcoef[c], k2 = gcoef[C + c], k3 = gcoef[2 * C + c];
+    float q1 = 0.f, q2 = 0.f, q3 = 0.f;
+    if (RES) { q1 = grcoef[c]; q2 = grcoef[C + c]; q3 = grcoef[2 * C + c]; }
+    const auto drr = make_rsrc(RES ? gres + goff : gin, RES ? gb : 0u);
+#pragma unroll
+    for (int e = 0; e < LG; ++e) {
+      const int i = e * NT + threadIdx.x;
+      const float gm = GP == 1 ? (u1[e] > 0.f ? t[e] : 0.f) : t[e];
+      if (i < nt) gs[i] = k1 * gm + k2 * u2[e] + k3;
+      if (RES) bstore(drr, q1 * gm + q2 * rv[e] + q3, tb + e * (NT * 4u), 0);
+    }
+#pragma unroll
+    for (int e = 0; e < LPT; ++e) {
+      const int i = e * NT + threadIdx.x;
+      if (i < nb) xs[i] = xi[e];
+    }
+  } else {
     const float* __restrict__ go = gout + (size_t)plane * nt;
     const float* __restrict__ src = in + (size_t)plane * nb;
     const int ntot = nt + nb;
@@ -1209,6 +1254,22 @@
 #undef SGCN_BWDL
 }
 
+template <int LPT, bool JA>
+void launch_bwd_s2_gp(const float* dy, const float* y, const float* s, const float* coef,
+                      const float* r, const float* rcoef, float* dres, const float* in,
+                      const float* xpos, const float* ypos, float* gin, float2* pg, int B, int C,
+                      int H, int W, int Ho, int add_half, hipStream_t st) {
+  constexpr int NT = kBwdThreads;
+  const size_t lds = (size_t)(H + Ho) * W * sizeof(float);
+#define SGCN_BWDG(G, R)                                                                       \
+  tshift_bwd_s2_kernel<NT, LPT, false, true, false, JA, G, R><<<B * C, NT, lds, st>>>(         \
+      nullptr, in, xpos, ypos, nullptr, nullptr, nullptr, nullptr, gin, pg, nullptr, C, H, W,  \
+      Ho, add_half, dy, y, s, coef, r, rcoef, dres)
+  if (y) { if (r) SGCN_BWDG(1, true); else SGCN_BWDG(1, false); }
+  else { if (r) SGCN_BWDG(2, true); else SGCN_BWDG(2, false); }
+#undef SGCN_BWDG
+}
+
 int pick_lpt(int n, int nt) {
   const int per = (n + nt - 1) / nt;
   return per <= 8 ? 8 : (per <= 16 ? 16 : 32);
@@ -1476,6 +1537,40 @@
   return 0;
 }
 
+int sgcn_tshift_bwd_s2_bnin(const float* dy, const float* y, const float* s, const float* coef,
+                            const float* r, const float* rcoef, float* dres, const float* in,
+                            const float* xpos, const float* ypos, float* gin, float* gx,
+                            float* gy, void* ws, size_t ws_bytes, int B, int C, int H, int W,
+                            int ypos_is_raw, void* stream) {
+  SGCN_REQUIRE(B > 0 && C > 0 && H > 0 && W > 0);
+  const int Ho = H / 2;
+  SGCN_REQUIRE((long long)(H + Ho) * W <= kBwdLdsMax);
+  SGCN_REQUIRE(dy && s && coef && in && xpos && ypos && gin && ws);
+  SGCN_REQUIRE((r == nullptr) == (rcoef == nullptr) && (r == nullptr) == (dres == nullptr));
+  SGCN_REQUIRE((gx == nullptr) == (gy == nullptr));
+  SGCN_REQUIRE(ws_bytes >= sgcn_tshift_bwd_ws_bytes(B, C));
+  SGCN_REQUIRE((long long)B * C < (1LL << 31));
+  hipStream_t st = (hipStream_t)stream;
+  float2* pg = (float2*)ws;
+  const int ah = ypos_is_raw ? 1 : 0;
+  const int lpt = pick_lpt(H * W, kBwdThreads);
+#define SGCN_S2G(L, J)                                                                       \
+  launch_bwd_s2_gp<L, J>(dy, y, s, coef, r, rcoef, dres, in, xpos, ypos, gin, pg, B, C, H, W, \
+                         Ho, ah, st)
+  if (W <= 64) {
+    if (lpt == 8) SGCN_S2G(8, true); else if (lpt == 16) SGCN_S2G(16, true);
+    else SGCN_S2G(32, true);
+  } else {
+    if (lpt == 8) SGCN_S2G(8, false); else if (lpt == 16) SGCN_S2G(16, false);
+    else SGCN_S2G(32, false);
+  }
+#undef SGCN_S2G
+  SGCN_LAUNCH_CHECK();
+  if (gx) tshift_pos_finalize_kernel<<<(C + 3) / 4, 256, 0, st>>>(pg, B, C, gx, gy);
+  SGCN_LAUNCH_CHECK();
+  return 0;
+}
+
 size_t sgcn_tshift_bwd_ws_bytes(int B, int C) { return (size_t)B * C * sizeof(float2); }
 
 int sgcn_tshift_pos_finalize_many(const void* const* partials, float* const* gx,
diff --git a/shift-gcn_amd/shiftgcn/_lib.py b/shift-gcn_amd/shiftgcn/_lib.py
--- a/shift-gcn_amd/shiftgcn/_lib.py
+++ b/shift-gcn_amd/shiftgcn/_lib.py
@@ -8,7 +8,7 @@
 LIB_NAME = "libshiftgcn_hip.so"
 LIB_PATH = os.path.join(os.path.dirname(os.path.abspath(__file__)), LIB_NAME)
 LIB_PATH = os.environ.get("SGCN_LIB_PATH", LIB_PATH)
-ABI_VERSION = 24
+ABI_VERSION = 25
 BATCH_MAX = 32
 ABI_DIAG_FLAG = 0x10000
 EINVAL = -22
@@ -61,7 +61,9 @@
     "sgcn_mask_prep": (_I, [_P, _P, _I, _P]),
     "sgcn_gcn_gather": (_I, [_P, _P, _P, _I, _I, _I, _I, _P]),
     "sgcn_gcn_dx_finish": (_I, [_P, _P, _P, _P, _P, _P, _P, _P, _P, _P, _P, _P, _I, _I, _I, _I,
-                                _I, _P]),
+                                _I, _I, _P]),
+    "sgcn_tshift_bwd_s2_bnin": (_I, [_P, _P, _P, _P, _P, _P, _P, _P, _P, _P, _P, _P, _P, _P, _Z,
+                                     _I, _I, _I, _I, _I, _P]),
     "sgcn_tshift_bwd_bnin": (_I, [_P, _P, _P, _P, _P, _P, _P, _P, _P, _P, _P, _Z, _I, _I, _I,
                                   _I, _I, _I, _P]),
     "sgcn_mask_grad_finalize": (_I, [_P, _P, _I, _I, _I, _P, _I, _P]),
diff --git a/shift-gcn_amd/shiftgcn/fused.py b/shift-gcn_amd/shiftgcn/fused.py
--- a/shift-gcn_amd/shiftgcn/fused.py
+++ b/shift-gcn_amd/shiftgcn/fused.py
@@ -218,7 +218,7 @@
 
 
 def gcn_backward(mod, s: GcnSaved, dH, extra_dx=None, dy_coef=None, prev=None, pre6=None,
-                 off=False, mask_dx=False):
+                 off=False, mask_dx=False, extra_stride=1):
     x0 = s.x0
     assert not (mask_dx and mod.has_down)
     B, Cin, T, V = x0.shape
@@ -262,8 +262,12 @@
         ops.pw_dw(PV(dZ), PV(s.xg), dLW, Cout, Cin, T, V, transpose=True, dbias=dLb)
     g["Linear_weight"], g["Linear_bias"] = _late(dLW, off), _late(dLb, off)
     a2, a2m = extra_dx or (None, None)
+    down_first = CONV_UNITS and mod.has_down and a2m is None
+    if down_first:
+        g_id = _empty(B, Cin, T, V, like=x0)
+        g.update(_down_dx_and_dw(mod, dD0, x0, g_id, False, off))
     res = ops.gcn_dx_finish(dXt, x0, s.m, add1=g_id, add2=a2, prev=prev, add2_mask=a2m,
-                            mask_dx=mask_dx)
+                            mask_dx=mask_dx, add2_stride=extra_stride, add1_plain=down_first)
     dx, mpart, prev_part = res if prev is not None else (*res, None)
     dmask = ops.grad_like(mod.Feature_Mask)
     fm = mod.Feature_Mask
@@ -274,14 +278,21 @@
         with _OffPath(off, mpart):
             ops.mask_grad_finalize(mpart, fm, B, Cin, V, out=dmask)
         g["Feature_Mask"] = _late(dmask, off)
-    if mod.has_down:
-        dWd = ops.grad_like(conv.weight)
-        dbd = ops.grad_like(conv.bias)
-        ops.pw_fwd(conv.weight, True, None, PV(dD0), PV(dx), Cin, Cout, T, V, accumulate=True)
-        with _OffPath(off, dD0, x0):
-            ops.pw_dw(PV(dD0), PV(x0), dWd, Cout, Cin, T, V, dbias=dbd)
-        g["down.0.weight"], g["down.0.bias"] = _late(dWd, off), _late(dbd, off)
+    if mod.has_down and not down_first:
+        g.update(_down_dx_and_dw(mod, dD0, x0, dx, True, off))
     return dx, g, prev_part
+
+
+def _down_dx_and_dw(mod, dD0, x0, dx, accumulate, off):
+    B, Cin, T, V = x0.shape
+    conv = mod.down[0]
+    Cout = mod.out_channels
+    dWd = ops.grad_like(conv.weight)
+    dbd = ops.grad_like(conv.bias)
+    ops.pw_fwd(conv.weight, True, None, PV(dD0), PV(dx), Cin, Cout, T, V, accumulate=accumulate)
+    with _OffPath(off, dD0, x0):
+        ops.pw_dw(PV(dD0), PV(x0), dWd, Cout, Cin, T, V, dbias=dbd)
+    return {"down.0.weight": _late(dWd, off), "down.0.bias": _late(dbd, off)}
 
 
 class TcnSaved:
@@ -383,13 +394,18 @@
 
 
 def tcn_core_backward(mod, s: TcnSaved, dS, materialize_dx=True, gpre=None, gcn_z=None,
-                      off=False):
+                      off=False, dres_out=None):
     H = s.H
     B, C, T, V = H.shape
     Cout = mod.out_channels
     si, so = mod.shift_in, mod.shift_out
     g, pre6 = {}, None
-    if gpre is not None:
+    if gpre is not None and so.stride == 2:
+        dRp, gx, gy, dres = ops.tshift_bwd_s2_bnin(
+            gpre[0], gpre[1], s.S, gpre[2], s.R, so.xpos.detach(), so.ypos.detach(), r=gpre[3],
+            rcoef=gpre[4], defer_pos=off, pos_out=_pos_alloc(so, off))
+        dres_out.append(dres)
+    elif gpre is not None:
         dRp, gx, gy = ops.tshift_bwd_bnin(gpre[0], gpre[1], s.S, gpre[2], s.R,
                                           so.xpos.detach(), so.ypos.detach(), defer_pos=off,
                                           pos_out=_pos_alloc(so, off))
@@ -448,14 +464,14 @@
     return Rc, rst, s
 
 
-def convbn_dx_and_dw(mod, s: ConvBnSaved, dRc, dx, accumulate, off=False):
+def convbn_dx_and_dw(mod, s: ConvBnSaved, dRc, dx, accumulate, off=False, compact=False):
     B, Cin, T, V = s.x.shape
     conv = mod.conv
     Cout = conv.out_channels
     dW = ops.grad_like(conv.weight)
     db = ops.grad_like(conv.bias)
-    ops.pw_fwd(conv.weight, True, None, PV(dRc), PV(dx, mod.stride), Cin, Cout, s.To, V,
-               accumulate=accumulate)
+    ops.pw_fwd(conv.weight, True, None, PV(dRc), PV(dx, 1 if compact else mod.stride), Cin,
+               Cout, s.To, V, accumulate=accumulate)
     with _OffPath(off, dRc, s.x):
         ops.pw_dw(PV(dRc), PV(s.x, mod.stride), dW, Cout, Cin, s.To, V, dbias=db)
     return {"conv.weight": _late(dW, off), "conv.bias": _late(db, off)}
@@ -606,7 +622,13 @@
     coef2, g["tcn1.bn2.weight"], g["tcn1.bn2.bias"] = ops.bn_bwd_finalize(
         part, B, Cout, B * To * V, ts.sst, unit.tcn1.bn2)
     dS = gpre = dres = extra = None
-    if _fused_tail(unit, To, V):
+    s2 = (CONV_UNITS and kind == "conv" and unit.tcn1.shift_out.stride == 2 and
+          ops.s2_bnin_fits(ts.R.shape[2], V))
+    if s2:
+        coefR, g["residual.bn.weight"], g["residual.bn.bias"] = ops.bn_bwd_finalize(
+            rpart, B, Cout, B * To * V, s.rs.rst, unit.residual.bn)
+        gpre = (dout, y, coef2, s.rs.Rc, coefR)
+    elif _fused_tail(unit, To, V):
         gpre = (dout, y, coef2)
         if kind == "identity":
             extra = (dout, y)
@@ -623,16 +645,29 @@
                 dres = torch.empty_like(s.x)
                 extra = (dres, None)
             ops.bn_bwd_apply(dout, y, relu, S, coef2, False, dr=dres, dx=dS)
+    dres_out = []
     (dA, coefA), gt, pre6 = tcn_core_backward(unit.tcn1, ts, dS, materialize_dx=False,
-                                              gpre=gpre, gcn_z=_gcn_z(unit, s), off=off)
+                                              gpre=gpre, gcn_z=_gcn_z(unit, s), off=off,
+                                              dres_out=dres_out)
+    if s2:
+        dres = dres_out[0]
+    gr, xs = None, 1
+    if CONV_UNITS and kind == "conv":
+        xs = unit.residual.stride
+        dxr = _empty(*s.x.shape[:2], s.rs.To, V, like=s.x)
+        gr = convbn_dx_and_dw(unit.residual, s.rs, dres, dxr, accumulate=False, off=off,
+                              compact=True)
+        extra = (dxr, None)
     dx, gg, prev_part = gcn_backward(unit.gcn1, s.gs, dA, extra_dx=extra, dy_coef=coefA,
-                                     prev=s.prev, pre6=pre6, off=off, mask_dx=mask_dx)
+                                     prev=s.prev, pre6=pre6, off=off, mask_dx=mask_dx,
+                                     extra_stride=xs)
     if s.prev is not None or mask_dx:
         li.dx, li.prev_part, li.masked = dx, prev_part, mask_dx
     g.update({"tcn1." + k: v for k, v in gt.items()})
     g.update({"gcn1." + k: v for k, v in gg.items()})
     if kind == "conv":
-        gr = convbn_dx_and_dw(unit.residual, s.rs, dres, dx, accumulate=True, off=off)
+        if gr is None:
+            gr = convbn_dx_and_dw(unit.residual, s.rs, dres, dx, accumulate=True, off=off)
         g.update({"residual." + k: v for k, v in gr.items()})
     return dx, g
 
@@ -643,6 +678,7 @@
 GBN_FUSION = int(os.environ.get("SGCN_GBN_FUSION", "2"))
 ASYNC_DW = int(os.environ.get("SGCN_ASYNC_DW", "1"))
 PREMASK = int(os.environ.get("SGCN_PREMASK", "1"))
+CONV_UNITS = int(os.environ.get("SGCN_CONV_UNITS", "1"))
 
 
 def trainable(module):
diff --git a/shift-gcn_amd/shiftgcn/ops.py b/shift-gcn_amd/shiftgcn/ops.py
--- a/shift-gcn_amd/shiftgcn/ops.py
+++ b/shift-gcn_amd/shiftgcn/ops.py
@@ -440,6 +440,39 @@
     return gin, (pp if pp is not None else gx), gy
 
 
+def s2_bnin_fits(H, W):
+    return H > 0 and (H + H // 2) * W <= BNIN_MAX_PLANE
+
+
+def tshift_bwd_s2_bnin(dy, y, s, coef, inp, xpos, ypos, r=None, rcoef=None, defer_pos=False,
+                       pos_out=None):
+    for t, n in ((dy, "dy"), (y, "y"), (s, "s"), (inp, "input"), (coef, "coef"), (r, "r"),
+                 (rcoef, "rcoef")):
+        if t is not None:
+            check_input(t, n)
+    B, C, H, W = inp.shape
+    if tuple(s.shape) != (B, C, H // 2, W) or dy.shape != s.shape:
+        raise ValueError(f"stride-2 gradient {tuple(dy.shape)} / {tuple(s.shape)} of planes "
+                         f"{tuple(inp.shape)}")
+    if (r is None) != (rcoef is None) or (r is not None and r.shape != s.shape):
+        raise ValueError("r and rcoef go together, r laid out like s")
+    lib = _lib.load()
+    dev = inp.device
+    gin = torch.empty_like(inp)
+    dres = torch.empty_like(s) if r is not None else None
+    nbytes = lib.sgcn_tshift_bwd_ws_bytes(B, C)
+    ws = torch.empty((max(nbytes, 4) + 3) // 4, device=dev, dtype=_F32)
+    gx, gy, pp = _pos_out(defer_pos, ws, B, C, dev, pos_out)
+    nb = 4 * ((2 + (y is not None) + 2 * (r is not None)) * s.numel() + 2 * inp.numel())
+    with _timed("tshift_bwd", 0, nb, inp, "S2BN " + _shp(inp)):
+        rc = lib.sgcn_tshift_bwd_s2_bnin(
+            _ptr(dy), _ptr(y), _ptr(s), _ptr(coef), _ptr(r), _ptr(rcoef), _ptr(dres), _ptr(inp),
+            _ptr(xpos), _ptr(ypos), _ptr(gin), _ptr(gx), _ptr(gy), _ptr(ws), nbytes, B, C, H, W,
+            1, _stream(inp))
+    _lib.check(rc, "sgcn_tshift_bwd_s2_bnin")
+    return gin, (pp if pp is not None else gx), gy, dres
+
+
 class PlaneView:
 
     __slots__ = ("t", "bstride", "cstride", "tstride", "rsign")
@@ -778,9 +811,15 @@
 
 
 def gcn_dx_finish(dxt, x0, m, add1=None, add2=None, prev=None, add2_mask=None,
-                  mask_dx=False):
+                  mask_dx=False, add2_stride=1, add1_plain=False):
     B, C, T, V = dxt.shape
+    if add2_stride != 1 and (add2 is None or
+                             tuple(add2.shape) != (B, C, (T + add2_stride - 1) // add2_stride, V)):
+        raise ValueError(f"compact add2 of stride {add2_stride} for {tuple(dxt.shape)}")
+    if add2_stride != 1:
+        check_input(add2, "add2")
     flags = int(bool(mask_dx)) | (2 if add2 is not None and _plane_dy(add2, dxt) else 0)
+    flags |= 4 if add1_plain else 0
     dx = torch.empty_like(dxt)
     part = torch.empty((B * C * V,), device=dxt.device, dtype=_F32)
     pp = torch.empty((B * C * 2,), device=dxt.device, dtype=_F32) if prev is not None else None
@@ -792,7 +831,7 @@
                                             _ptr(add2), _ptr(add2_mask), _ptr(dx), _ptr(part),
                                             _ptr(ps), _ptr(pst.mean) if pst else None,
                                             _ptr(pst.invstd) if pst else None, _ptr(pp), B, C,
-                                            T, V, flags, _stream(dxt))
+                                            T, V, flags, int(add2_stride), _stream(dxt))
     _lib.check(rc, "sgcn_gcn_dx_finish")
     return (dx, part) if prev is None else (dx, part, pp)
 
```

After: 2073 clips/s, median of 6. Within noise of the previous version (+1.0%).
